# hawkn/emqx

Measured on AMD Instinct MI355X. Metric: topic matches/sec at 10M filters, higher is better.
Workload: dtype u8/u32; 1 GPU; c3: 10M mixed-wildcard filters incl. $share groups and '$SYS' exclusion; filters=10000002, topics_per_gpu_step=1000000, global_batch=1000000, parallelism=topic-sharded x1 (trie replicated), streams=3, distinct_batches=4, table_copies=1, outputs=pairs

## Files before the change

### emqx_amd/_native.py

```python
from __future__ import annotations

import ctypes as C
from pathlib import Path

import numpy as np

from .build import LIB_TMATCH

TM_OK, TM_EINVAL, TM_ENOMEM, TM_EDEVICE, TM_ECAP = 0, -1, -2, -3, -4
TM_OP_DELETE, TM_OP_INSERT = 0, 1
TM_KEY_BINARY, TM_KEY_WORDS, TM_KEY_EMPTY_LIST, TM_KEY_ESCAPED = 0, 1, 2, 4
TM_ORDER_TRAVERSAL, TM_ORDER_SORTED, TM_ORDER_UNIQUE = 0, 1, 2

EXPORTS = ("tm_create", "tm_destroy", "tm_apply_deltas", "tm_sync", "tm_match_batch",
           "tm_match_batch_dev", "tm_first_batch", "tm_stats", "tm_profile_enable", "tm_profile_read",
           "tm_last_error", "tm_abi_version", "tm_merge_shards", "tm_host_alloc", "tm_host_free",
           "tm_stream_release", "tm_match_batch_ex", "tm_match_batch_dev_ex", "tm_sort_segments",
           "tm_matches_filter", "tm_apply_deltas_ex", "tm_read_begin", "tm_read_end", "tm_epoch",
           "tm_create_replicas", "tm_replica_stats", "tm_debug_set", "tm_debug_get", "tm_match_batch32_ex",
           "tm_match_batch32_dev", "tm_matches_filter_ex", "tm_host_alloc_ex", "tm_commit",
           "tm_match_batch32_pairs", "tm_match_batch_dev_pairs", "tm_set_dests", "tm_fanout_dev", "tm_route_batch",
           "tm_fanout_dev_pairs", "tm_route_batch32", "tm_set_route_filters", "tm_aggre_dev", "tm_route_batch_ex",
           "tm_route_batch32_ex")
TM_ALLOC_VRAM = 1
TM_ROUTE_AGGRE = 1
NO_FILTER = 0xFFFFFFFF
TM_DEBUG_LB_SPINS, TM_DEBUG_LB_FAIL_BLOCK, TM_DEBUG_LB_LAUNCHES, TM_DEBUG_PHASES = 1, 2, 3, 4
TM_DEBUG_FAILED_BATCHES, TM_DEBUG_RETRIED_BATCHES = 5, 6
TM_DEBUG_PATH_PHASES, TM_DEBUG_PATH_SMALL, TM_DEBUG_PATH_LANE = 7, 8, 9
TM_DEBUG_SMALL_KERNEL = 10
SMALL_AUTO, SMALL_WAVE, SMALL_WAVE8 = 0, 1, 3
TM_DEBUG_COMBINE, TM_DEBUG_COMBINED_LAUNCHES, TM_DEBUG_COMBINED_BATCHES = 12, 13, 14
TM_DEBUG_WIDE_NODES, TM_DEBUG_DENSE_WIDE = 15, 16
TM_DEBUG_CMB_GATHER, TM_DEBUG_CMB_LAND = 17, 18
TM_DEBUG_COMMITS, TM_DEBUG_COMMIT_WAITS, TM_DEBUG_COMMIT_FORCED = 19, 20, 21
TM_DEBUG_SMALL_TICKET = 22
TM_DEBUG_CMB_SPIN = 23
TM_DEBUG_PATCH_ZC = 24
TM_DEBUG_FANOUT_GRID = 25
TM_DEBUG_ROUTE_ONE, TM_DEBUG_ROUTE_GRID = 26, 27
MAX_DESTS = 65536


class NativeUnavailable(RuntimeError):
    pass


class TmError(RuntimeError):
    def __init__(self, code, msg):
        super().__init__(f"tmatch error {code}: {msg}")
        self.code = code


class DeviceError(TmError):
    """TM_EDEVICE: the GPU failed the call (e.g. a batch whose look-back wait
    expired twice, include/tmatch.h err flag 4).  Never a client error: the
    reference raises badarg only for a '+'/'#' topic level
    (emqx_trie_search.erl:374-375)."""


class tm_options(C.Structure):
    _fields_ = [("device", C.c_int32), ("copies", C.c_uint32), ("hint_keys", C.c_uint64)]


class tm_stats_t(C.Structure):
    _fields_ = [(n, C.c_uint64) for n in ("n_keys", "n_wild_keys", "n_exact_keys", "n_dead_keys",
                                          "n_nodes", "n_edges", "n_words", "device_bytes",
                                          "uploads", "patch_bytes")]


_lib = None


def load_library(path: Path | None = None):
    global _lib
    if _lib is not None and path is None:
        return _lib
    import os
    p = Path(path) if path else Path(os.environ.get("TM_LIB", LIB_TMATCH))
    if not p.exists():
        raise NativeUnavailable(f"{p} is not built (run emqx_amd.build.build_all())")
    lib = C.CDLL(str(p))
    vp, u64, u32, i32 = C.c_void_p, C.c_uint64, C.c_uint32, C.c_int
    sig = {
        "tm_create": (i32, [C.POINTER(tm_options), C.POINTER(vp)]),
        "tm_destroy": (i32, [vp]),
        "tm_apply_deltas": (i32, [vp, u64, vp, vp, vp, vp, vp]),
        "tm_sync": (i32, [vp, vp]),
        "tm_match_batch": (i32, [vp, u64, vp, vp, vp, vp, u64, vp]),
        "tm_match_batch_dev": (i32, [vp, u64, vp, vp, vp, vp, u64, vp, vp]),
        "tm_first_batch": (i32, [vp, u64, vp, vp, vp, vp]),
        "tm_matches_filter": (i32, [vp, u64, vp, vp, vp, vp, u64, vp]),
        "tm_matches_filter_ex": (i32, [vp, u64, vp, vp, vp, vp, vp, u64, vp]),
        "tm_stats": (i32, [vp, C.POINTER(tm_stats_t)]),
        "tm_profile_enable": (i32, [vp, i32]),
        "tm_profile_read": (i32, [vp, C.POINTER(C.c_double), C.POINTER(C.c_double), C.POINTER(u64), i32]),
        "tm_last_error": (C.c_char_p, [vp]),
        "tm_abi_version": (u32, []),
        "tm_merge_shards": (i32, [u32, u64, vp, vp, u64, vp, vp, u64, vp]),
        "tm_host_alloc": (i32, [vp, u64, C.POINTER(vp)]),
        "tm_host_free": (i32, [vp, vp]),
        "tm_host_alloc_ex": (i32, [vp, u64, u32, C.POINTER(vp)]),
        "tm_stream_release": (i32, [vp, vp]),
        "tm_match_batch_ex": (i32, [vp, u64, vp, vp, vp, vp, u64, vp, u32, vp]),
        "tm_match_batch_dev_ex": (i32, [vp, u64, vp, vp, vp, vp, u64, vp, u32, vp, vp]),
        "tm_match_batch_dev_pairs": (i32, [vp, u64, vp, vp, vp, vp, u64, vp, vp]),
        "tm_sort_segments": (i32, [vp, u64, vp, vp, u64, u32, vp, vp]),
        "tm_apply_deltas_ex": (i32, [vp, u64, vp, vp, vp, vp, vp, C.POINTER(u64)]),
        "tm_commit": (i32, [vp, u64, vp, vp, vp, vp, vp, C.POINTER(u64)]),
        "tm_read_begin": (i32, [vp, C.POINTER(u64)]),
        "tm_read_end": (i32, [vp, u64]),
        "tm_epoch": (i32, [vp, C.POINTER(u64), C.POINTER(u64)]),
        "tm_create_replicas": (i32, [C.POINTER(tm_options), C.POINTER(C.c_int32), u32, C.POINTER(vp)]),
        "tm_replica_stats": (i32, [vp, u32, C.POINTER(u64), C.POINTER(C.c_int32)]),
        "tm_match_batch32_ex": (i32, [vp, u64, vp, vp, vp, vp, u64, vp, u32, vp]),
        "tm_match_batch32_dev": (i32, [vp, u64, vp, vp, vp, vp, u64, vp, vp]),
        "tm_match_batch32_pairs": (i32, [vp, u64, vp, vp, vp, vp, u64, vp]),
        "tm_set_dests": (i32, [vp, u64, vp, vp]),
        "tm_fanout_dev": (i32, [vp, u64, vp, vp, u64, vp, u64, u32, vp, vp, vp, vp]),
        "tm_fanout_dev_pairs": (i32, [vp, u64, vp, vp, u64, vp, u64, u32, vp, vp, vp, vp]),
        "tm_route_batch": (i32, [vp, u64, vp, vp, u32, vp, vp, vp, u64, vp]),
        "tm_route_batch32": (i32, [vp, u64, vp, vp, u32, vp, vp, vp, u64, vp]),
        "tm_set_route_filters": (i32, [vp, u64, vp, vp]),
        "tm_aggre_dev": (i32, [vp, u32, vp, vp, vp, u64, vp, u64, vp, vp, vp, vp]),
        "tm_route_batch_ex": (i32, [vp, u64, vp, vp, u32, vp, vp, vp, u64, vp, u32]),
        "tm_route_batch32_ex": (i32, [vp, u64, vp, vp, u32, vp, vp, vp, u64, vp, u32]),
        "tm_debug_set": (i32, [vp, u32, u64]),
        "tm_debug_get": (i32, [vp, u32, C.POINTER(u64)]),
    }
    for name, (res, args) in sig.items():
        try:
            f = getattr(lib, name)
        except AttributeError:
            if p == LIB_TMATCH:
                raise
            continue
        f.restype, f.argtypes = res, args
    if path is None:
        _lib = lib
    return lib


def _ptr(a: np.ndarray | None):
    return None if a is None else a.ctypes.data_as(C.c_void_p)


def _gpu_present() -> bool:
    try:
        import torch
        return torch.cuda.is_available()
    except Exception:
        return False


def merge_shards(world: int, n: int, d_shard_hit: int, d_shard_vals: int, stride: int, d_out_hit: int,
                 d_out_vals: int, cap: int, stream: int | None = None):
    if not _gpu_present():
        raise NativeUnavailable("no HIP device visible: the shard merge runs on the GPU only")
    lib = load_library()
    rc = lib.tm_merge_shards(world, n, d_shard_hit, d_shard_vals, stride, d_out_hit, d_out_vals, cap, stream)
    if rc != TM_OK:
        raise TmError(rc, lib.tm_last_error(None).decode())


def pack_strings(items) -> tuple[np.ndarray, np.ndarray]:
    items = [bytes(x) for x in items]
    offs = np.zeros(len(items) + 1, dtype=np.uint64)
    if items:
        offs[1:] = np.cumsum([len(x) for x in items], dtype=np.uint64)
    blob = np.frombuffer(b"".join(items) + b"\0" * 16, dtype=np.uint8)
    return blob, offs


class Index:

    def __init__(self, device: int = -1, hint_keys: int = 0, devices=None, copies: int = 1):
        if not _gpu_present():
            raise NativeUnavailable("no HIP device visible: the topic index runs on the GPU only")
        self._lib = load_library()
        opts = tm_options(device, copies, hint_keys)
        h = C.c_void_p()
        if devices is not None:
            devs = (C.c_int32 * len(devices))(*devices)
            rc = self._lib.tm_create_replicas(C.byref(opts), devs, len(devices), C.byref(h))
        else:
            rc = self._lib.tm_create(C.byref(opts), C.byref(h))
        if rc != TM_OK:
            raise TmError(rc, self._lib.tm_last_error(None).decode())
        self._h = h

    def _check(self, rc):
        if rc != TM_OK:
            cls = DeviceError if rc == TM_EDEVICE else TmError
# ... 260 lines not shown
```

### emqx_amd/csrc/tm_dev.h

```cpp
#pragma once
#include <stdint.h>
#include <hip/hip_runtime.h>
#include "tm_layout.h"

namespace tmx {

struct DevIndex {
    const VocabEntry *vocab; uint32_t vmask;
    const uint8_t *wpool;
    const Node *nodes;
    const CSlot *ctab;
    const uint32_t *vals;
    const ExactEntry *exact; uint32_t xmask;
    const uint16_t *xfp;
    const uint32_t *wseq;
    const uint32_t *wbits; uint32_t wcap;
    uint32_t depth, xlen_max;
    uint64_t xlen_mask;
    uint32_t hdesc;
};

constexpr int FAST_L = 8;

__host__ __device__ __forceinline__ uint32_t need_levels(const DevIndex &ix, uint32_t L) {
    const bool exact = L < 64 ? ((ix.xlen_mask >> L) & 1u) != 0 : L <= ix.xlen_max;
    return exact || L < ix.depth ? L : ix.depth;
}
constexpr int MID_L = 32;
constexpr int MAX_LEVELS = 65536;
constexpr int RCAP = 8;
constexpr int DEEP_LANES = 64;

enum { L_MID = 0, L_DEEP = 1, L_OVF_MID = 2, L_OVF_DEEP = 3, L_COUNT = 4 };

enum : uint32_t { LB_AGG = 1, LB_INCL = 2, LB_FAIL = 3 };
constexpr uint32_t LB_TAG_BITS = 19, LB_TAG_MASK = (1u << LB_TAG_BITS) - 1;
constexpr uint64_t LB_VAL_MASK = (1ull << 42) - 1;
__host__ __device__ constexpr uint64_t lb_word(uint32_t tag, uint32_t st, uint64_t v) {
    return (uint64_t)tag << 45 | (uint64_t)st << 42 | (v & LB_VAL_MASK);
}
__host__ __device__ constexpr uint32_t lb_tag(uint64_t w) { return (uint32_t)(w >> 45); }
__host__ __device__ constexpr uint32_t lb_state(uint64_t w) { return (uint32_t)(w >> 42) & 7u; }

constexpr uint32_t LB_SPINS = 1u << 22;
constexpr uint32_t LB_SLEEP = 1;
constexpr uint32_t LB_STRIDE = 1;
struct LbCtl {
    uint32_t spins;
    uint32_t fail_block;
    uint32_t ticket;
};

constexpr int SMALL_SEGS = 16;

struct Workspace {
    uint32_t *cnt;
    uint32_t *nr;
    uint2 *rng;
    uint32_t *lists;
    uint32_t *list_n;
    uint64_t *blk;
    uint64_t *sup;
    uint32_t *deep_wid;
    uint2 *deep_stk;
    uint8_t *deep_plus;
    uint64_t *look;
    uint32_t *pairs;
    uint64_t *vres;
    uint32_t *hint_h, *hint_d;
    uint64_t cap_n;
};

constexpr int TILE = 256;
constexpr int SUP = 64;
constexpr int SM_TICK = L_COUNT + 4;
constexpr int LIST_SLOTS = SM_TICK + SMALL_SEGS;
constexpr int HINT_FAIL = L_COUNT + 1;
constexpr int HINT_WORDS = L_COUNT + 2;
constexpr int VRES_K = 64;
constexpr int VRES_STRIDE = 16;
constexpr int VRES_POOL = VRES_K * VRES_STRIDE;
constexpr int VRES_WORDS = VRES_POOL + VRES_STRIDE;
constexpr int SM_TOPICS = 16;
constexpr int SM_TB = 256;
constexpr int SM_VSTAGE = 1024;


hipError_t launch_match_phase1(const DevIndex &ix, const Workspace &ws, uint64_t n, const uint8_t *bytes,
                               const uint64_t *offs, uint64_t *hit_offs, uint8_t *err, hipStream_t s,
                               hipEvent_t ev_walk0 = nullptr, hipEvent_t ev_walk1 = nullptr);
hipError_t launch_match_phase2(const DevIndex &ix, const Workspace &ws, uint64_t n, const uint8_t *bytes,
                               const uint64_t *offs, uint64_t *hit_offs, uint32_t *out, uint64_t cap,
                               hipStream_t s);
hipError_t launch_match_pairs(const DevIndex &ix, const Workspace &ws, uint64_t n, const uint8_t *bytes,
                              const uint64_t *offs, uint8_t *err, uint32_t *pairs, uint32_t *out, uint64_t cap,
                              hipStream_t s, hipEvent_t ev_walk0 = nullptr, hipEvent_t ev_walk1 = nullptr);
bool small_path_ok(const DevIndex &ix, uint64_t n);
bool one_launch_ok(const DevIndex &ix);
bool lite_path_ok(const DevIndex &ix);
enum { SMALL_AUTO = 0, SMALL_WAVE = 1, SMALL_WAVE8 = 3 };
enum { PATH_PHASES = 0, PATH_SMALL = 1, PATH_LANE = 2, PATH_COUNT = 3 };
hipError_t launch_match(const DevIndex &ix, const Workspace &ws, uint64_t n, const uint8_t *bytes,
                        const uint64_t *offs, uint64_t *hit_offs, uint8_t *err, uint32_t *out, uint64_t cap,
                        uint32_t tag, LbCtl lb, bool phases, int small_kind, hipStream_t s,
                        hipEvent_t ev_walk0 = nullptr, hipEvent_t ev_walk1 = nullptr, int *path = nullptr);
struct SmallSeg {
    const uint8_t *blob; const void *offs; void *hit; uint8_t *err; uint32_t *out;
    uint64_t cap; uint32_t n, block0;
};
struct SmallSegs { uint32_t count, pairs; SmallSeg s[SMALL_SEGS]; };
hipError_t launch_small_segs(const DevIndex &ix, const Workspace &ws, const SmallSegs &sg, bool u32, uint32_t tag,
                             LbCtl lb, int small_kind, hipStream_t s, int *path = nullptr);
hipError_t launch_match32(const DevIndex &ix, const Workspace &ws, uint64_t n, const uint8_t *bytes,
                          const uint32_t *offs, uint32_t *hit_offs, uint8_t *err, uint32_t *out, uint64_t cap,
                          uint32_t tag, LbCtl lb, int small_kind, hipStream_t s, int *path = nullptr);
hipError_t launch_offs_widen(const uint32_t *in, uint64_t *out, uint64_t m, hipStream_t s);
hipError_t launch_offs_narrow(const uint64_t *in, uint32_t *out, uint64_t m, hipStream_t s);
hipError_t launch_first(const DevIndex &ix, const Workspace &ws, uint64_t n, const uint8_t *bytes,
                        const uint64_t *offs, uint32_t *out_value, uint8_t *out_found, hipStream_t s);
hipError_t launch_merge_shards(uint32_t world, uint64_t n, const uint64_t *shard_hit, const uint32_t *shard_vals,
                               uint64_t stride, uint64_t *out_hit, uint32_t *out, uint64_t cap, hipStream_t s);
hipError_t launch_sort_segments(const Workspace &ws, uint64_t n, const uint64_t *hit_offs, uint32_t *out, uint64_t cap,
                                int unique, uint32_t *ucnt, hipStream_t s);
hipError_t launch_copy_values(const uint64_t *hit_offs, uint64_t n, const uint32_t *src, uint32_t *dst, uint64_t cap,
                              hipStream_t s);
constexpr int FO_GRID = 4096;
constexpr int FO_MAX_BITS = 9;
constexpr int FO_BINS = 1 << FO_MAX_BITS;
constexpr uint32_t FO_MAX_DESTS = 65536;
struct FanoutScratch {
    uint32_t *tab;
    uint32_t *tot;
    uint32_t *t, *v, *b;
    uint64_t cap;
    uint64_t *voff;
    uint64_t voff_cap;
    uint64_t *sums;
    uint32_t *b2;
    uint64_t *ag_bits;
    uint32_t *ag_pre, *ag_cnt;
    uint64_t ag_cap;
};
constexpr uint32_t FP_TILES = 1024;
bool fanout_two_pass(uint32_t n_dests);
hipError_t launch_fanout(const FanoutScratch &fs, uint64_t n, const uint64_t *hit, const uint32_t *values,
                         uint64_t cap, const uint32_t *dest_of, uint64_t dest_len, uint32_t n_dests,
                         uint64_t *dest_offsets, uint32_t *out_topic, uint32_t *out_value, hipStream_t s);
hipError_t launch_fanout_pairs(const FanoutScratch &fs, uint64_t n, const uint32_t *pairs, const uint32_t *values,
                               uint64_t cap, const uint32_t *dest_of, uint64_t dest_len, uint32_t n_dests,
                               uint64_t *dest_offsets, uint32_t *out_topic, uint32_t *out_value, hipStream_t s);
constexpr uint32_t FO1_TOPICS = 8192;
constexpr uint32_t FO1_ENTRIES = 16384;
constexpr uint32_t FO1_BLOCK = 1024;
constexpr uint32_t FO1_MAX_DESTS = 255;
enum { FO1_ST_STATE = 0, FO1_ST_TOTAL = 1, FO1_ST_WORDS = 2 };
enum : uint32_t { FO1_DONE = 1, FO1_TOO_LARGE = 2 };
hipError_t launch_fanout_one(uint64_t n, const uint32_t *pairs, const uint32_t *values, uint64_t vcap,
                             const uint32_t *dest_of, uint64_t dest_len, uint32_t n_dests, uint32_t *dest_offsets,
                             uint32_t *out_topic, uint32_t *out_value, uint64_t cap, uint32_t *status, hipStream_t s);
hipError_t launch_aggre(const FanoutScratch &fs, uint32_t n_dests, const uint64_t *dest_offsets, const uint32_t *in_topic,
                        const uint32_t *in_value, uint64_t cap, const uint32_t *filter_of, uint64_t filter_len,
                        uint64_t *out_dest_offsets, uint32_t *out_topic, uint32_t *out_value, hipStream_t s);
hipError_t launch_aggre_one(const uint32_t *status_in, const uint32_t *dest_offsets, uint32_t n_dests,
                            const uint32_t *in_topic, const uint32_t *in_value, const uint32_t *filter_of,
                            uint64_t filter_len, uint32_t *out_dest_offsets, uint32_t *out_topic, uint32_t *out_value,
                            uint64_t cap, uint32_t *status, hipStream_t s);
constexpr int N_TABLES = 9;
constexpr uint64_t PATCH_OFF = (1ull << 48) - 1;
struct PatchRun { uint64_t dst; uint32_t src, n; };
struct PatchBases { uint64_t b[N_TABLES]; };
hipError_t launch_patch(const PatchRun *d_runs, const uint32_t *d_data, uint64_t n_runs, PatchBases bases,
                        hipStream_t s);
// ... 7 lines not shown
```

### emqx_amd/csrc/tm_host.cpp

```cpp
#include <hip/hip_runtime.h>

#include <algorithm>
#include <atomic>
#include <chrono>
#include <cstdlib>
#include <cstdio>
#include <cstring>
#include <condition_variable>
#include <deque>
#include <memory>
#include <mutex>
#include <string>
#include <thread>
#include <map>
#include <unordered_map>
#include <unordered_set>
#include <set>
#include <vector>

#include "../../include/tmatch.h"
#include "tm_dev.h"
#include "tm_layout.h"

using namespace tmx;

namespace {

thread_local std::string g_last_error;


struct Dirty {
    std::vector<std::pair<uint64_t, uint64_t>> r;
    bool all = true;
    void add(uint64_t lo, uint64_t hi) {
        if (all || lo >= hi) return;
        if (!r.empty() && lo >= r.back().first && lo <= r.back().second) {
            r.back().second = std::max(r.back().second, hi);
            return;
        }
        r.push_back({lo, hi});
    }
    void set_all() { all = true; r.clear(); }
    void clear() { all = false; r.clear(); }
};

constexpr int MAX_REPLICAS = 16;

template <class T>
struct Mirror {
    std::vector<T> h;
    T *d[MAX_REPLICAS] = {};
    uint64_t dcap = 0;
    Dirty dirty;
    void touch(uint64_t i, uint64_t n = 1) {
        uint64_t lo = i * sizeof(T), hi = (i + n) * sizeof(T);
        dirty.add(lo / 4, (hi + 3) / 4);
    }
    uint64_t bytes() const { return h.size() * sizeof(T); }
};

struct NodeAux {
    uint32_t parent = NONE, wid = NONE, hash_cap = 0, exact_cap = 0;
    uint32_t depth = 0;
    uint32_t hash_roff = 0, exact_roff = 0;
    uint8_t is_plus = 0;
    uint32_t bm = NONE;
    uint32_t hdesc = 0;
};

struct WordRef { const uint8_t *p; uint32_t n; int kind; };

inline uint32_t nlit_of(const Node &n) { return n.nlit & NLIT_MASK; }

}

struct Lane {
    int r = 0;
    hipStream_t s = nullptr;
    bool owned = false;
    bool busy = false;
    bool used = false;
    bool drained = false;
    hipEvent_t done = nullptr;
    uint64_t tick = 0;
    uint32_t tag = 0;
    uint64_t waited = 0;
    Workspace w{};
    uint8_t *pin_in = nullptr, *pin_in_dev = nullptr; uint64_t pin_in_cap = 0;
    uint8_t *pin_out = nullptr, *pin_out_dev = nullptr; uint64_t pin_out_cap = 0;
    uint8_t *d_in = nullptr; uint64_t d_in_cap = 0;
    uint8_t *d_res = nullptr; uint64_t d_res_cap = 0;
    uint32_t *pin_vals = nullptr, *pin_vals_dev = nullptr; uint64_t pin_vals_cap = 0;
    uint32_t *d_vals = nullptr; uint64_t d_vals_cap = 0;
    uint64_t *d_o64 = nullptr, *d_h64 = nullptr; uint64_t d_o64_cap = 0, d_h64_cap = 0;
    FanoutScratch f{};
    uint32_t *d_ft = nullptr, *d_fv = nullptr; uint64_t d_ft_cap = 0, d_fv_cap = 0;
    uint64_t *d_fo = nullptr; uint64_t d_fo_cap = 0;
    uint32_t *d_pr = nullptr; uint64_t d_pr_cap = 0;
    uint32_t *fo1_h = nullptr, *fo1_d = nullptr;
    uint32_t *d_at = nullptr, *d_av = nullptr; uint64_t d_at_cap = 0, d_av_cap = 0;
    uint64_t *d_ao = nullptr; uint64_t d_ao_cap = 0;
    uint32_t *fo1_s = nullptr;
};

constexpr int PATCH_RING = 128;
constexpr uint64_t PATCH_ZC_MAX = 64 << 10;
struct PatchSlot {
    uint8_t *pin = nullptr; uint64_t pin_cap = 0;
    uint8_t *pin_dev = nullptr;
    uint64_t bytes = 0, nr = 0, seq = 0;
};

struct Replica {
    int device = 0, group = 0;
    hipStream_t ps = nullptr;
    hipEvent_t last_patch = nullptr;
    uint8_t *pdev[PATCH_RING] = {}; uint64_t pdev_cap[PATCH_RING] = {};
    hipEvent_t pdone[PATCH_RING] = {}; bool ppending[PATCH_RING] = {};
    uint64_t applied = 0;
    uint64_t last_use = 0;
    uint64_t batches = 0;
};


constexpr int MAX_HOST_LANES = 16;
constexpr int MAX_DEV_LANES = 16;

constexpr int CMB_LEADERS = 4;

struct tm_index {
    std::mutex mu;
    std::mutex img;
    std::atomic<bool> img_dirty{true};
    bool view_ok = false;
    std::condition_variable cv;
    int nrep = 1, ngroups = 1;
    Replica rep[MAX_REPLICAS];
    uint64_t rr = 0;

    Mirror<VocabEntry> vocab; uint64_t vcount = 0; uint32_t wid_next = 0;
    std::vector<uint32_t> wref, wslot, free_wids;
    Mirror<uint8_t> wpool; uint64_t wpool_dead = 0;
    Mirror<Node> nodes; std::vector<NodeAux> aux; std::vector<uint32_t> free_nodes; uint64_t live_nodes = 0;
    Mirror<CSlot> ctab; std::vector<uint32_t> free_ctab[33]; uint64_t nlinks = 0, ntables = 0;
    Mirror<uint32_t> vals; std::vector<uint32_t> free_blocks[33];
    Mirror<ExactEntry> exact; std::vector<uint32_t> xcap, xroff; uint64_t xcount = 0;
    Mirror<uint16_t> xfp;
    Mirror<uint32_t> wseq; uint64_t wseq_dead = 0;
    Mirror<uint32_t> wbits; uint32_t wb_words = 0;
    std::vector<uint32_t> free_wbits; std::set<uint32_t> wide;
    std::unordered_map<uint64_t, uint32_t> lvl_edges;
    std::vector<uint32_t> lvl_distinct;
    bool dense_dirty = false;

    std::vector<uint64_t> depth_cnt, xlen_cnt;

    std::unordered_set<std::string> dead;
    struct MfState {
        std::mutex mu;
        bool log_on = false, log_lost = false;
        std::vector<std::pair<bool, std::string>> log;
        std::unordered_set<std::string> keys;
        bool have_keys = false, dev_stale = true;
        std::atomic<size_t> nkeys{0};
        std::vector<std::string> words;
        uint32_t *pool = nullptr, *val = nullptr; uint64_t *koff = nullptr, K = 0;
        uint64_t pcap = 0, vcap = 0, kcap = 0;
        uint32_t *q = nullptr; uint64_t qcap = 0;
        uint8_t *err = nullptr; uint64_t *hit = nullptr; uint32_t *out = nullptr;
        uint64_t ecap = 0, ocap = 0, hcap = 0;
        hipStream_t s = nullptr;
        uint64_t snapshots = 0, slices = 0;
    } mf;
    uint64_t n_wild = 0, n_exact = 0;
    uint64_t n_hdesc_keys = 0;
    uint64_t uploads = 0, patch_bytes = 0;

    PatchSlot patch[PATCH_RING]; uint64_t patch_seq = 0;
    uint64_t pub_seq = 0;
    int serving[MAX_REPLICAS];
    std::atomic<int> img_hold{0};
    std::atomic<uint64_t> commits{0}, commit_waits{0}, commit_forced{0};
    DevIndex view[MAX_REPLICAS];

    std::vector<std::unique_ptr<Lane>> lanes;
    uint64_t tick = 0;

    std::mutex dst_mu;
    std::vector<uint32_t> dest_h;
    struct DestDev {
        uint32_t *d = nullptr; uint64_t cap = 0, len = 0;
        uint64_t lo = 0, hi = 0;
        uint32_t *pin = nullptr; uint64_t pin_cap = 0;
        hipEvent_t ev = nullptr; bool ev_set = false;
        hipStream_t ev_s = nullptr;
    } dest[MAX_REPLICAS];
    std::vector<uint32_t> filt_h;
    DestDev filt[MAX_REPLICAS];

    struct Pinned { uint8_t *host, *dev; uint64_t size; bool vram; };
    std::vector<Pinned> pinned;

    std::atomic<uint64_t> epoch{1};
    std::mutex ep_mu;
    uint64_t next_ticket = 1;
    std::map<uint64_t, uint64_t> readers;
    std::multiset<uint64_t> reader_epochs;

    bool prof = false;
    struct ProfEv { hipEvent_t b0, w0, w1, b1; int device; };
    std::vector<ProfEv> prof_pending, prof_free;
    double prof_walk_ms = 0, prof_batch_ms = 0;
    uint64_t prof_batches = 0;

    LbCtl dbg_lb{LB_SPINS, NONE, 0};
    uint32_t small_ticket = 1;
    bool patch_zc = true;
    uint64_t dbg_lb_launches = 0;
    bool dbg_phases = false;
    int small_kind = SMALL_AUTO;
    std::atomic<uint64_t> failed_batches{0}, retried_batches{0};
    std::atomic<uint64_t> path_batches[PATH_COUNT] = {};
    std::atomic<uint64_t> route_one{0}, route_grid{0};
    std::mutex cmb_mu;
    std::condition_variable cmb_gcv;
    std::deque<struct SmallReq *> cmb_q;
    int cmb_running = 0;
    int cmb_inflight = 0;
    int cmb_gathering = 0;
    int cmb_hw = 0;
    uint64_t cmb_hw_ns = 0;
    std::atomic<int> cmb_leaders{CMB_LEADERS};
    std::atomic<int> cmb_gather_us{0};
    std::atomic<int> cmb_spin_us{0};
    std::atomic<uint64_t> cmb_launches{0}, cmb_batches{0};
};

namespace {

int fail(tm_index *, int code, const std::string &msg) {
    g_last_error = msg;
    return code;
}

#define HIPCHK(h, x)                                                                    \
    do {                                                                                \
        hipError_t e_ = (x);                                                            \
        if (e_ != hipSuccess)                                                           \
            return fail(h, TM_EDEVICE, std::string(#x ": ") + hipGetErrorString(e_));   \
    } while (0)


void pack8(const uint8_t *p, uint32_t n, uint32_t &b0, uint32_t &b1);

uint64_t word_hash(const uint8_t *p, uint32_t n) {
    if (n <= VINL) {
        uint32_t b0, b1;
        pack8(p, n, b0, b1);
        return word_hash_short(b0, b1, n);
    }
    uint64_t x = FNV_OFF;
    for (uint32_t i = 0; i < n; i++) x = (x ^ p[i]) * FNV_PRIME;
    return word_hash_finish(x, n);
}

uint32_t pow2_at_least(uint64_t x) {
    uint64_t c = 16;
    while (c < x) c <<= 1;
    return (uint32_t)c;
}


void pack8(const uint8_t *p, uint32_t n, uint32_t &b0, uint32_t &b1) {
    b0 = b1 = 0;
    for (uint32_t i = 0; i < n && i < 8; i++) (i < 4 ? b0 : b1) |= (uint32_t)p[i] << (8 * (i % 4));
}

bool vocab_eq(tm_index *ix, const VocabEntry &e, uint64_t h, const uint8_t *p, uint32_t n) {
    if (e.tag != vocab_tag(h, n)) return false;
    if (n <= VINL) {
        uint32_t b0, b1;
        pack8(p, n, b0, b1);
        return e.b0 == b0 && e.b1 == b1;
    }
    return e.b1 == n && !memcmp(ix->wpool.h.data() + e.b0, p, n);
}

uint32_t vocab_find(tm_index *ix, const uint8_t *p, uint32_t n) {
    const uint64_t h = word_hash(p, n);
    const uint32_t mask = (uint32_t)ix->vocab.h.size() - 1;
    for (uint32_t s = (uint32_t)h & mask;; s = (s + 1) & mask) {
        const VocabEntry &e = ix->vocab.h[s];
        if (e.wid == NONE) return NONE;
        if (vocab_eq(ix, e, h, p, n)) return e.wid;
    }
}

VocabEntry empty_vocab() { VocabEntry e; memset(&e, 0, sizeof e); e.wid = NONE; return e; }

void vocab_bytes(tm_index *ix, const VocabEntry &e, std::string &out) {
    uint32_t n = e.tag & 0xFF;
    if (n < VINL + 1) {
        out.resize(n);
        for (uint32_t i = 0; i < n; i++) out[i] = (char)(((i < 4 ? e.b0 : e.b1) >> (8 * (i % 4))) & 0xFF);
    } else {
        out.assign(reinterpret_cast<const char *>(ix->wpool.h.data() + e.b0), e.b1);
    }
}

constexpr uint32_t VOCAB_LOAD_SHIFT = 2;
uint64_t vocab_entry_hash(tm_index *ix, const VocabEntry &e) {
    std::string w;
    vocab_bytes(ix, e, w);
    return word_hash(reinterpret_cast<const uint8_t *>(w.data()), (uint32_t)w.size());
}

void vocab_rehash(tm_index *ix, uint64_t cap) {
    std::vector<VocabEntry> nt(cap, empty_vocab());
    const uint32_t mask = (uint32_t)nt.size() - 1;
    for (const VocabEntry &e : ix->vocab.h) {
        if (e.wid == NONE) continue;
        const uint64_t h = vocab_entry_hash(ix, e);
        for (uint32_t s = (uint32_t)h & mask;; s = (s + 1) & mask)
            if (nt[s].wid == NONE) { nt[s] = e; ix->wslot[e.wid] = s; break; }
    }
    ix->vocab.h.swap(nt);
    ix->vocab.dirty.set_all();
}

void wide_cover(tm_index *ix);

void vocab_grow(tm_index *ix, uint64_t need) {
    if ((need << VOCAB_LOAD_SHIFT) <= ix->vocab.h.size()) return;
    vocab_rehash(ix, pow2_at_least(need << VOCAB_LOAD_SHIFT));
}

uint32_t vocab_intern(tm_index *ix, const uint8_t *p, uint32_t n) {
    uint32_t w = vocab_find(ix, p, n);
    if (w != NONE) return w;
    vocab_grow(ix, ix->vcount + 1);
    VocabEntry e = empty_vocab();
    const uint64_t h = word_hash(p, n);
    e.tag = vocab_tag(h, n);
    if (!ix->free_wids.empty()) { e.wid = ix->free_wids.back(); ix->free_wids.pop_back(); }
    else {
        e.wid = ix->wid_next++;
        ix->wref.push_back(0);
        ix->wslot.push_back(NONE);
        wide_cover(ix);
    }
    if (n <= VINL) {
        pack8(p, n, e.b0, e.b1);
    } else {
        uint64_t off = ix->wpool.h.size();
        ix->wpool.h.resize(off + ((n + 3) & ~3u), 0);
        memcpy(ix->wpool.h.data() + off, p, n);
        ix->wpool.touch(off, (n + 3) & ~3u);
        e.b0 = (uint32_t)off;
        e.b1 = n;
    }
    const uint32_t mask = (uint32_t)ix->vocab.h.size() - 1;
    for (uint32_t s = (uint32_t)h & mask;; s = (s + 1) & mask)
        if (ix->vocab.h[s].wid == NONE) { ix->vocab.h[s] = e; ix->vocab.touch(s); ix->wslot[e.wid] = s; break; }
    ix->vcount++;
    return e.wid;
}

void vocab_erase(tm_index *ix, uint32_t wid) {
    auto &t = ix->vocab.h;
    const uint32_t mask = (uint32_t)t.size() - 1;
    uint32_t i = ix->wslot[wid];
    if (t[i].wid != wid) return;
    if ((t[i].tag & 0xFF) > VINL) ix->wpool_dead += (t[i].b1 + 3) & ~3u;
    for (uint32_t j = (i + 1) & mask; t[j].wid != NONE; j = (j + 1) & mask) {
        const uint32_t k = (uint32_t)vocab_entry_hash(ix, t[j]) & mask;
        const bool stays = (i <= j) ? (i < k && k <= j) : (i < k || k <= j);
        if (!stays) { t[i] = t[j]; ix->wslot[t[i].wid] = i; ix->vocab.touch(i); i = j; }
    }
    t[i] = empty_vocab();
    ix->vocab.touch(i);
    ix->wslot[wid] = NONE;
    ix->free_wids.push_back(wid);
    ix->vcount--;
}

void word_ref(tm_index *ix, uint32_t wid) { ix->wref[wid]++; }
void word_unref(tm_index *ix, uint32_t wid) {
    if (--ix->wref[wid] == 0) vocab_erase(ix, wid);
}


uint32_t cls_of(uint32_t cap);

uint32_t ctab_alloc(tm_index *ix, uint32_t cap) {
    auto &fl = ix->free_ctab[cls_of(cap)];
    uint32_t o;
    if (!fl.empty()) { o = fl.back(); fl.pop_back(); }
    else { o = (uint32_t)ix->ctab.h.size(); ix->ctab.h.resize(o + cap); }
    for (uint32_t i = 0; i < cap; i++) ix->ctab.h[o + i] = CSlot{NONE, NONE, 0, 0};
    ix->ctab.touch(o, cap);
    ix->ntables++;
    return o;
}

void ctab_free(tm_index *ix, uint32_t off, uint32_t cap) {
    ix->free_ctab[cls_of(cap)].push_back(off);
    ix->ntables--;
}

void ctab_put(tm_index *ix, uint32_t off, uint32_t mask, uint32_t wid, uint32_t child, uint64_t sum) {
    for (uint32_t s = child_hash(wid) & mask;; s = (s + 1) & mask)
        if (ix->ctab.h[off + s].wid == NONE) {
            ix->ctab.h[off + s] = CSlot{wid, child, (uint32_t)sum, (uint32_t)(sum >> 32)};
            ix->ctab.touch(off + s);
            return;
        }
}

uint32_t ctab_find(tm_index *ix, uint32_t off, uint32_t mask, uint32_t wid) {
    for (uint32_t s = child_hash(wid) & mask;; s = (s + 1) & mask) {
        const CSlot &c = ix->ctab.h[off + s];
        if (c.wid == NONE) return NONE;
        if (c.wid == wid) return s;
    }
}

void ctab_erase(tm_index *ix, uint32_t off, uint32_t mask, uint32_t wid) {
    uint32_t i = ctab_find(ix, off, mask, wid);
    if (i == NONE) return;
    CSlot *t = ix->ctab.h.data() + off;
    for (uint32_t j = (i + 1) & mask; t[j].wid != NONE; j = (j + 1) & mask) {
        uint32_t k = child_hash(t[j].wid) & mask;
        bool stays = (i <= j) ? (i < k && k <= j) : (i < k || k <= j);
        if (!stays) { t[i] = t[j]; ix->ctab.touch(off + i); i = j; }
    }
    t[i] = CSlot{NONE, NONE, 0, 0};
    ix->ctab.touch(off + i);
}


uint32_t cls_of(uint32_t cap) { uint32_t c = 0; while ((1u << c) < cap) c++; return c; }

uint32_t val_alloc(tm_index *ix, uint32_t cap) {
    auto &fl = ix->free_blocks[cls_of(cap)];
    if (!fl.empty()) { uint32_t o = fl.back(); fl.pop_back(); return o; }
    uint64_t o = ix->vals.h.size();
    ix->vals.h.resize(o + cap, 0);
    return (uint32_t)o;
}

void val_free(tm_index *ix, uint32_t off, uint32_t cap) {
    if (cap) ix->free_blocks[cls_of(cap)].push_back(off);
}

bool run_insert(tm_index *ix, uint32_t &off, uint32_t &cnt, uint32_t &cap, uint32_t v) {
    uint32_t *b = ix->vals.h.data() + off;
    uint32_t pos = (uint32_t)(std::lower_bound(b, b + cnt, v) - b);
    if (pos < cnt && b[pos] == v) return false;
    if (cnt == cap) {
        uint32_t ncap = cap ? cap * 2 : 1;
        uint32_t noff = val_alloc(ix, ncap);
        memmove(ix->vals.h.data() + noff, ix->vals.h.data() + off, sizeof(uint32_t) * cnt);
        val_free(ix, off, cap);
        off = noff; cap = ncap;
        ix->vals.touch(off, cnt);
    }
    uint32_t *r = ix->vals.h.data() + off;
    memmove(r + pos + 1, r + pos, sizeof(uint32_t) * (cnt - pos));
    r[pos] = v;
    cnt++;
    ix->vals.touch(off + pos, cnt - pos);
    return true;
}

bool run_erase(tm_index *ix, uint32_t &off, uint32_t &cnt, uint32_t &cap, uint32_t v) {
    uint32_t *b = ix->vals.h.data() + off;
    uint32_t pos = (uint32_t)(std::lower_bound(b, b + cnt, v) - b);
    if (pos >= cnt || b[pos] != v) return false;
    memmove(b + pos, b + pos + 1, sizeof(uint32_t) * (cnt - pos - 1));
    cnt--;
    if (pos < cnt) ix->vals.touch(off + pos, cnt - pos);
    if (!cnt) { val_free(ix, off, cap); off = 0; cap = 0; }
    return true;
}

bool run_op(tm_index *ix, bool ins, uint32_t &roff, uint32_t &cap, uint32_t &doff, uint32_t &dcnt, uint32_t v) {
    uint32_t off = roff, cnt = dcnt & RUN_CNT;
    const bool changed = ins ? run_insert(ix, off, cnt, cap, v) : run_erase(ix, off, cnt, cap, v);
    roff = off;
    if (cnt == 1) { doff = ix->vals.h[off]; dcnt = 1u | RUN_INLINE; }
    else { doff = off; dcnt = cnt; }
    return changed;
}


uint32_t node_new(tm_index *ix, uint32_t parent, uint32_t wid, bool is_plus) {
    uint32_t id;
    if (!ix->free_nodes.empty()) { id = ix->free_nodes.back(); ix->free_nodes.pop_back(); }
    else { id = (uint32_t)ix->nodes.h.size(); ix->nodes.h.emplace_back(); ix->aux.emplace_back(); }
    Node nd; memset(&nd, 0, sizeof nd); nd.plus = NONE;
    for (uint32_t k = 0; k < KINL; k++) { nd.kw[k] = NONE; nd.kc[k] = NONE; }
    ix->nodes.h[id] = nd;
    ix->nodes.touch(id);
    NodeAux a; a.parent = parent; a.wid = wid; a.is_plus = is_plus;
    a.depth = parent == NONE ? 0 : ix->aux[parent].depth + 1;
    ix->aux[id] = a;
    ix->live_nodes++;
    if (ix->depth_cnt.size() <= a.depth) ix->depth_cnt.resize(a.depth + 1, 0);
    ix->depth_cnt[a.depth]++;
    if (!is_plus && wid != NONE) word_ref(ix, wid);
    return id;
}

uint32_t child_find(tm_index *ix, uint32_t node, uint32_t wid) {
    const Node &n = ix->nodes.h[node];
    if (nlit_of(n) <= KINL) {
        for (uint32_t k = 0; k < KINL; k++) if (n.kw[k] == wid) return n.kc[k];
        return NONE;
    }
    uint32_t s = ctab_find(ix, n.kw[0], n.kw[1], wid);
    return s == NONE ? NONE : ix->ctab.h[n.kw[0] + s].child;
}

void set_bloom(Node &n, uint32_t wid) {
    const uint32_t b = child_bit(child_hash(wid));
    bloom_word(n, b >> 5) |= 1u << (b & 31);
}


void wide_bit(tm_index *ix, uint32_t node, uint32_t wid, bool on) {
    const uint32_t bm = ix->aux[node].bm;
    if (bm == NONE) return;
    uint32_t &w = ix->wbits.h[bm + (wid >> 5)];
    if (on) w |= 1u << (wid & 31); else w &= ~(1u << (wid & 31));
    ix->wbits.touch(bm + (wid >> 5));
}

void wide_fill(tm_index *ix, uint32_t node) {
    const uint32_t bm = ix->aux[node].bm;
    std::fill(ix->wbits.h.begin() + bm, ix->wbits.h.begin() + bm + ix->wb_words, 0u);
    Node &n = ix->nodes.h[node];
    for (uint32_t i = 0; i <= n.kw[1]; i++) {
        const uint32_t w = ix->ctab.h[n.kw[0] + i].wid;
        if (w != NONE) ix->wbits.h[bm + (w >> 5)] |= 1u << (w & 31);
    }
    ix->wbits.touch(bm, ix->wb_words);
    n.kw[2] = bm;
    ix->nodes.touch(node);
    ix->dense_dirty = true;
}

uint32_t wide_alloc(tm_index *ix) {
    if (!ix->free_wbits.empty()) { uint32_t o = ix->free_wbits.back(); ix->free_wbits.pop_back(); return o; }
    const uint32_t o = (uint32_t)ix->wbits.h.size();
    ix->wbits.h.resize(o + ix->wb_words, 0u);
    return o;
}

void wide_cover(tm_index *ix) {
    if (ix->wide.empty() || (uint64_t)ix->wb_words * 32 >= ix->wid_next) return;
    uint32_t words = std::max<uint32_t>(ix->wb_words, 1024);
    while ((uint64_t)words * 32 < ix->wid_next) words *= 2;
    ix->wb_words = words;
    ix->wbits.h.clear();
    ix->free_wbits.clear();
    for (uint32_t node : ix->wide) {
        ix->aux[node].bm = wide_alloc(ix);
        wide_fill(ix, node);
    }
    ix->wbits.dirty.set_all();
}

void to_wide(tm_index *ix, uint32_t node) {
    if (ix->wide.empty()) ix->wb_words = 0;
    ix->wide.insert(node);
    if ((uint64_t)ix->wb_words * 32 < ix->wid_next) {
        ix->aux[node].bm = NONE;
        wide_cover(ix);
        return;
    }
    ix->aux[node].bm = wide_alloc(ix);
    wide_fill(ix, node);
}

void from_wide(tm_index *ix, uint32_t node) {
    ix->free_wbits.push_back(ix->aux[node].bm);
    ix->aux[node].bm = NONE;
    ix->wide.erase(node);
    Node &n = ix->nodes.h[node];
    for (uint32_t j = 0; j < 6; j++) bloom_word(n, j) = 0;
    for (uint32_t i = 0; i <= n.kw[1]; i++) {
        const uint32_t w = ix->ctab.h[n.kw[0] + i].wid;
        if (w != NONE) set_bloom(n, w);
    }
    ix->nodes.touch(node);
}

uint64_t lit_bloom(tm_index *ix, uint32_t q) {
    const Node &n = ix->nodes.h[q];
    uint64_t m = 0;
    auto add = [&](uint32_t wid) { m |= 1ull << psum_bit(child_hash(wid)); };
    if (nlit_of(n) <= KINL) {
        for (uint32_t k = 0; k < KINL; k++) if (n.kw[k] != NONE) add(n.kw[k]);
    } else if (nlit_of(n) > PSUM_BLOOM) {
        m = (1ull << PSUM_BLOOM) - 1;
    } else {
        for (uint32_t i = 0; i <= n.kw[1]; i++) if (ix->ctab.h[n.kw[0] + i].wid != NONE) add(ix->ctab.h[n.kw[0] + i].wid);
    }
    return m;
}

uint64_t node_flags(const Node &n) {
    return (n.hash_cnt ? PSUM_HASH : 0) | (n.exact_cnt ? PSUM_EXACT : 0) | (n.plus != NONE ? PSUM_PLUS : 0) |
           ((n.nlit & NLIT_HDESC) ? PSUM_HDESC : 0);
}

uint64_t node_psum(tm_index *ix, uint32_t q) {
    const Node &n = ix->nodes.h[q];
    uint64_t m = node_flags(n) | lit_bloom(ix, q) << PSUM_BQ;
    if (n.plus != NONE) m |= node_flags(ix->nodes.h[n.plus]) << PSUM_QQ | lit_bloom(ix, n.plus) << PSUM_BQQ;
    return m;
}

void summary_refresh1(tm_index *ix, uint32_t x);
void summary_refresh(tm_index *ix, uint32_t x) {
    summary_refresh1(ix, x);
    if (x != ROOT && ix->aux[x].is_plus) summary_refresh1(ix, ix->aux[x].parent);
}

void summary_refresh1(tm_index *ix, uint32_t x) {
    if (x == ROOT) return;
    const NodeAux &a = ix->aux[x];
    const uint32_t p = a.parent;
    Node &pn = ix->nodes.h[p];
    if (a.is_plus) {
        if (pn.plus != x) return;
        const uint64_t m = node_psum(ix, x);
        if (pn.psum_lo != (uint32_t)m || pn.psum_hi != (uint32_t)(m >> 32)) {
            pn.psum_lo = (uint32_t)m; pn.psum_hi = (uint32_t)(m >> 32);
            ix->nodes.touch(p);
        }
        return;
    }
    if (nlit_of(pn) <= KINL) return;
    const uint32_t sl = ctab_find(ix, pn.kw[0], pn.kw[1], a.wid);
    if (sl == NONE) return;
    CSlot &c = ix->ctab.h[pn.kw[0] + sl];
    if (c.child != x) return;
    const uint64_t m = node_psum(ix, x);
    if (c.sum_lo != (uint32_t)m || c.sum_hi != (uint32_t)(m >> 32)) {
        c.sum_lo = (uint32_t)m; c.sum_hi = (uint32_t)(m >> 32);
        ix->ctab.touch(pn.kw[0] + sl);
    }
}

void to_table(tm_index *ix, uint32_t node, uint32_t cap) {
    Node &n = ix->nodes.h[node];
    std::vector<CSlot> kids;
    if (nlit_of(n) <= KINL) {
        for (uint32_t k = 0; k < KINL; k++)
            if (n.kw[k] != NONE) {
                const uint64_t m = node_psum(ix, n.kc[k]);
                kids.push_back({n.kw[k], n.kc[k], (uint32_t)m, (uint32_t)(m >> 32)});
            }
    } else {
        for (uint32_t i = 0; i <= n.kw[1]; i++) if (ix->ctab.h[n.kw[0] + i].wid != NONE) kids.push_back(ix->ctab.h[n.kw[0] + i]);
        ctab_free(ix, n.kw[0], n.kw[1] + 1);
    }
    uint32_t off = ctab_alloc(ix, cap);
    Node &m = ix->nodes.h[node];
    for (uint32_t j = 0; j < 6; j++) bloom_word(m, j) = 0;
    for (auto &c : kids) {
        ctab_put(ix, off, cap - 1, c.wid, c.child, (uint64_t)c.sum_hi << 32 | c.sum_lo);
        set_bloom(m, c.wid);
    }
    m.kw[0] = off; m.kw[1] = cap - 1;
    if (ix->aux[node].bm != NONE) {
        m.kw[2] = ix->aux[node].bm;
        ix->dense_dirty = true;
    }
}

void lvl_edge(tm_index *ix, uint32_t lvl, uint32_t wid, bool add) {
    const uint64_t k = (uint64_t)lvl << 32 | wid;
    if (ix->lvl_distinct.size() <= lvl) ix->lvl_distinct.resize(lvl + 1, 0);
    if (add) {
        if (ix->lvl_edges[k]++ == 0) { ix->lvl_distinct[lvl]++; ix->dense_dirty |= !ix->wide.empty(); }
    } else {
        auto it = ix->lvl_edges.find(k);
        if (it != ix->lvl_edges.end() && --it->second == 0) {
            ix->lvl_edges.erase(it);
            ix->lvl_distinct[lvl]--;
            ix->dense_dirty |= !ix->wide.empty();
        }
    }
}

constexpr uint64_t DENSE_NUM = 3, DENSE_DEN = 5;
void wide_dense(tm_index *ix) {
    if (!ix->dense_dirty) return;
    ix->dense_dirty = false;
    for (uint32_t node : ix->wide) {
        Node &n = ix->nodes.h[node];
        const uint32_t lvl = ix->aux[node].depth;
        const uint64_t distinct = lvl < ix->lvl_distinct.size() ? ix->lvl_distinct[lvl] : 0;
        const bool dense = (uint64_t)nlit_of(n) * DENSE_DEN >= distinct * DENSE_NUM;
        const uint32_t want = dense ? NONE : ix->aux[node].bm;
        if (n.kw[2] != want) { n.kw[2] = want; ix->nodes.touch(node); }
    }
}

void child_add(tm_index *ix, uint32_t node, uint32_t wid, uint32_t child) {
    ix->nlinks++;
    lvl_edge(ix, ix->aux[node].depth, wid, true);
    if (ix->aux[node].bm != NONE) ix->dense_dirty = true;
    Node *n = &ix->nodes.h[node];
    if (nlit_of(*n) < KINL) {
        for (uint32_t k = 0; k < KINL; k++)
            if (n->kw[k] == NONE) { n->kw[k] = wid; n->kc[k] = child; break; }
    } else {
        if (nlit_of(*n) == KINL) to_table(ix, node, 16);
        else if ((nlit_of(*n) + 1) * 2 > n->kw[1] + 1) to_table(ix, node, (n->kw[1] + 1) * 2);
        n = &ix->nodes.h[node];
        ctab_put(ix, n->kw[0], n->kw[1], wid, child, node_psum(ix, child));
        if (ix->aux[node].bm != NONE) wide_bit(ix, node, wid, true);
        else set_bloom(*n, wid);
    }
    n->nlit++;
    if (nlit_of(*n) == WIDE_LIT && ix->aux[node].bm == NONE) { to_wide(ix, node); n = &ix->nodes.h[node]; }
    ix->nodes.touch(node);
    summary_refresh(ix, node);
}

void child_remove(tm_index *ix, uint32_t node, uint32_t wid) {
    ix->nlinks--;
    lvl_edge(ix, ix->aux[node].depth, wid, false);
    if (ix->aux[node].bm != NONE) ix->dense_dirty = true;
    Node &n = ix->nodes.h[node];
    if (nlit_of(n) <= KINL) {
        for (uint32_t k = 0; k < KINL; k++)
            if (n.kw[k] == wid) { n.kw[k] = NONE; n.kc[k] = NONE; break; }
        n.nlit--;
    } else {
        ctab_erase(ix, n.kw[0], n.kw[1], wid);
        wide_bit(ix, node, wid, false);
        n.nlit--;
        if (ix->aux[node].bm != NONE && nlit_of(n) < WIDE_LIT) from_wide(ix, node);
        if (nlit_of(n) == KINL) {
            std::vector<CSlot> kids;
            for (uint32_t i = 0; i <= n.kw[1]; i++) if (ix->ctab.h[n.kw[0] + i].wid != NONE) kids.push_back(ix->ctab.h[n.kw[0] + i]);
            ctab_free(ix, n.kw[0], n.kw[1] + 1);
            for (uint32_t k = 0; k < KINL; k++) { n.kw[k] = kids[k].wid; n.kc[k] = kids[k].child; }
        }
    }
    ix->nodes.touch(node);
    summary_refresh(ix, node);
}

bool node_empty(tm_index *ix, uint32_t id) {
    const Node &n = ix->nodes.h[id];
    return n.plus == NONE && n.nlit == 0 && n.hash_cnt == 0 && n.exact_cnt == 0 && ix->aux[id].hdesc == 0;
}

void node_prune(tm_index *ix, uint32_t id) {
    while (id != ROOT && node_empty(ix, id)) {
        NodeAux a = ix->aux[id];
        if (a.is_plus) {
            Node &pn = ix->nodes.h[a.parent];
            pn.plus = NONE; pn.psum_lo = pn.psum_hi = 0;
            ix->nodes.touch(a.parent);
            summary_refresh(ix, a.parent);
        } else {
            child_remove(ix, a.parent, a.wid);
            word_unref(ix, a.wid);
        }
        ix->free_nodes.push_back(id);
        ix->live_nodes--;
        ix->depth_cnt[a.depth]--;
        id = a.parent;
    }
}


ExactEntry empty_exact() { ExactEntry e; memset(&e, 0, sizeof e); e.nlev = NONE; return e; }

uint64_t seq_hash(const std::vector<uint32_t> &w) {
    uint64_t x = FNV_OFF;
    for (uint32_t v : w) x = seq_hash_step(x, v);
    return seq_hash_finish(x, (uint32_t)w.size());
}

bool exact_eq(tm_index *ix, const ExactEntry &e, uint64_t h, const std::vector<uint32_t> &w) {
    if (e.h_lo != (uint32_t)h || e.h_hi != (uint32_t)(h >> 32) || e.nlev != w.size()) return false;
    const uint32_t *s = w.size() <= XINL ? e.wids : ix->wseq.h.data() + e.seq_off;
    return !memcmp(s, w.data(), sizeof(uint32_t) * w.size());
}

uint32_t exact_find_slot(tm_index *ix, uint64_t h, const std::vector<uint32_t> &w) {
    const uint32_t mask = (uint32_t)ix->exact.h.size() - 1;
    for (uint32_t s = (uint32_t)h & mask;; s = (s + 1) & mask) {
        const ExactEntry &e = ix->exact.h[s];
        if (e.nlev == NONE) return NONE;
        if (exact_eq(ix, e, h, w)) return s;
    }
}

void exact_rehash(tm_index *ix, uint32_t ncap);
void exact_grow(tm_index *ix, uint64_t need) {
    if (need * 2 <= ix->exact.h.size()) return;
    exact_rehash(ix, pow2_at_least(need * 2));
}

void exact_rehash(tm_index *ix, uint32_t ncap) {
    std::vector<ExactEntry> nt(ncap, empty_exact());
    std::vector<uint32_t> nc(ncap, 0), nr(ncap, 0);
    std::vector<uint16_t> nf(ncap, 0);
    const uint32_t mask = ncap - 1;
    for (size_t i = 0; i < ix->exact.h.size(); i++) {
        const ExactEntry &e = ix->exact.h[i];
        if (e.nlev == NONE) continue;
        for (uint32_t s = e.h_lo & mask;; s = (s + 1) & mask)
            if (nt[s].nlev == NONE) { nt[s] = e; nc[s] = ix->xcap[i]; nr[s] = ix->xroff[i]; nf[s] = ix->xfp.h[i]; break; }
    }
    ix->exact.h.swap(nt);
    ix->xcap.swap(nc);
    ix->xroff.swap(nr);
    ix->xfp.h.swap(nf);
    ix->exact.dirty.set_all();
    ix->xfp.dirty.set_all();
}

void exact_erase_slot(tm_index *ix, uint32_t i) {
    auto &t = ix->exact.h;
    const uint32_t mask = (uint32_t)t.size() - 1;
    {
        const uint32_t nl = t[i].nlev;
        const uint32_t *ws = nl <= XINL ? t[i].wids : ix->wseq.h.data() + t[i].seq_off;
        std::vector<uint32_t> used(ws, ws + nl);
        if (nl > XINL) ix->wseq_dead += nl;
        for (uint32_t w : used) word_unref(ix, w);
        ix->xlen_cnt[nl]--;
    }
    for (uint32_t j = (i + 1) & mask; t[j].nlev != NONE; j = (j + 1) & mask) {
        uint32_t k = t[j].h_lo & mask;
        bool stays = (i <= j) ? (i < k && k <= j) : (i < k || k <= j);
        if (!stays) {
            t[i] = t[j]; ix->xcap[i] = ix->xcap[j]; ix->xroff[i] = ix->xroff[j]; ix->xfp.h[i] = ix->xfp.h[j];
            ix->exact.touch(i); ix->xfp.touch(i);
            i = j;
        }
    }
    t[i] = empty_exact();
    ix->xcap[i] = 0;
    ix->xroff[i] = 0;
    ix->xfp.h[i] = 0;
    ix->exact.touch(i);
    ix->xfp.touch(i);
    ix->xcount--;
}

void reclaim(tm_index *ix) {
    if (ix->wpool_dead * 2 > ix->wpool.h.size() && ix->wpool.h.size() >= (64u << 10)) {
        std::vector<uint8_t> np;
        np.reserve(ix->wpool.h.size() - ix->wpool_dead);
        for (VocabEntry &e : ix->vocab.h) {
            if (e.wid == NONE || (e.tag & 0xFF) <= VINL) continue;
            const uint64_t off = np.size(), padded = (e.b1 + 3) & ~3u;
            np.insert(np.end(), ix->wpool.h.begin() + e.b0, ix->wpool.h.begin() + e.b0 + padded);
            e.b0 = (uint32_t)off;
        }
        ix->wpool.h.swap(np);
        ix->wpool_dead = 0;
        ix->wpool.dirty.set_all();
        ix->vocab.dirty.set_all();
    }
    if (ix->wseq_dead * 2 > ix->wseq.h.size() && ix->wseq.h.size() >= (16u << 10)) {
        std::vector<uint32_t> nq;
        nq.reserve(ix->wseq.h.size() - ix->wseq_dead);
        for (ExactEntry &e : ix->exact.h) {
            if (e.nlev == NONE || e.nlev <= XINL) continue;
            const uint64_t off = nq.size();
            nq.insert(nq.end(), ix->wseq.h.begin() + e.seq_off, ix->wseq.h.begin() + e.seq_off + e.nlev);
            e.seq_off = (uint32_t)off;
        }
        ix->wseq.h.swap(nq);
        ix->wseq_dead = 0;
        ix->wseq.dirty.set_all();
        ix->exact.dirty.set_all();
    }
    const uint64_t vmin = 1024;
    if (ix->vocab.h.size() > vmin && (ix->vcount << (VOCAB_LOAD_SHIFT + 2)) < ix->vocab.h.size())
        vocab_rehash(ix, std::max<uint64_t>(vmin, pow2_at_least(std::max<uint64_t>(ix->vcount, 1) << VOCAB_LOAD_SHIFT)));
    if (ix->exact.h.size() > 1024 && ix->xcount * 8 < ix->exact.h.size())
        exact_rehash(ix, std::max<uint32_t>(1024, pow2_at_least(ix->xcount * 2)));
}


void split_words(const uint8_t *f, uint32_t len, std::vector<WordRef> &out) {
    out.clear();
    uint32_t s = 0;
    for (uint32_t i = 0; i <= len; i++) {
        if (i == len || f[i] == '/') {
            uint32_t n = i - s;
            int kind = (n == 1 && f[s] == '+') ? 1 : (n == 1 && f[s] == '#') ? 2 : 0;
            out.push_back({f + s, n, kind});
            s = i + 1;
        }
    }
}

std::string dead_key(const uint8_t *f, uint32_t len, uint32_t v, uint8_t flags) {
    std::string k;
    k.reserve(len + 5);
    k.push_back((char)flags);
// ... 34 lines not shown
std::string esc_join(const std::vector<std::pair<std::string, bool>> &w) {
    std::string o;
    for (size_t i = 0; i < w.size(); i++) {
        if (i) o.push_back('/');
        if (w[i].second) { o += w[i].first; continue; }
        if (w[i].first == "+" || w[i].first == "#") { o.push_back('\\'); o += w[i].first; continue; }
        for (char c : w[i].first) {
            if (c == '/' || c == '\\') o.push_back('\\');
            o.push_back(c);
        }
    }
    return o;
}

bool word_never(const std::pair<std::string, bool> &w) {
    return !w.second && (w.first == "+" || w.first == "#" || w.first.find('/') != std::string::npos);
}

void word_key_op(tm_index *ix, bool ins, const std::vector<WordRef> &w, uint32_t v, const std::string &dk,
                 bool dead_done);

void key_op(tm_index *ix, bool ins, const uint8_t *f, uint32_t len, uint32_t v, uint8_t flags,
            std::vector<WordRef> &w, std::vector<uint32_t> &wids) {
    if ((flags & TM_KEY_ESCAPED) && !(flags & TM_KEY_EMPTY_LIST)) {
        std::vector<std::pair<std::string, bool>> ew;
        esc_words(f, len, ew);
        bool never = false;
        for (auto &x : ew) never |= word_never(x);
        if (!never) {
            std::string plain;
            for (size_t i = 0; i < ew.size(); i++) { if (i) plain.push_back('/'); plain += ew[i].first; }
            key_op(ix, ins, reinterpret_cast<const uint8_t *>(plain.data()), (uint32_t)plain.size(), v,
                   TM_KEY_WORDS, w, wids);
            return;
        }
        const std::string canon = esc_join(ew);
        const std::string dk = dead_key(reinterpret_cast<const uint8_t *>(canon.data()), (uint32_t)canon.size(), v,
                                        TM_KEY_WORDS | TM_KEY_ESCAPED);
        if (ix->mf.log_on) mf_log(ix, ins, dk);
        if (ins ? !ix->dead.insert(dk).second : !ix->dead.erase(dk)) return;
        size_t hpos = ew.size();
        for (size_t i = 0; i + 1 < ew.size(); i++)
            if (ew[i].second && ew[i].first == "#") { hpos = i; break; }
        bool plain_prefix = hpos < ew.size();
        for (size_t i = 0; i < hpos && plain_prefix; i++) plain_prefix = !word_never(ew[i]);
        if (!plain_prefix) return;
        std::vector<WordRef> pw;
        for (size_t i = 0; i <= hpos; i++)
            pw.push_back({reinterpret_cast<const uint8_t *>(ew[i].first.data()), (uint32_t)ew[i].first.size(),
                          ew[i].second ? (ew[i].first == "+" ? 1 : 2) : 0});
        pw.push_back({nullptr, 0, 0});
        word_key_op(ix, ins, pw, v, dk, true);
        return;
    }
    if (flags & TM_KEY_EMPTY_LIST) {
        auto k = dead_key(nullptr, 0, v, TM_KEY_EMPTY_LIST);
        if (ins) ix->dead.insert(k); else ix->dead.erase(k);
        mf_log(ix, ins, k);
        return;
    }
    split_words(f, len, w);
    bool wild = false;
    for (auto &x : w) wild |= x.kind != 0;
    if (!wild && !(flags & TM_KEY_WORDS)) {
        wids.clear();
        if (ins) {
            for (auto &x : w) wids.push_back(vocab_intern(ix, x.p, x.n));
            exact_grow(ix, ix->xcount + 1);
        } else {
            for (auto &x : w) {
                uint32_t id = vocab_find(ix, x.p, x.n);
                if (id == NONE) return;
                wids.push_back(id);
            }
        }
        const uint64_t h = seq_hash(wids);
        uint32_t s = exact_find_slot(ix, h, wids);
        if (s == NONE) {
            if (!ins) return;
            ExactEntry e = empty_exact();
            e.h_lo = (uint32_t)h; e.h_hi = (uint32_t)(h >> 32); e.nlev = (uint32_t)wids.size();
            if (wids.size() <= XINL) {
                std::copy(wids.begin(), wids.end(), e.wids);
            } else {
                e.seq_off = (uint32_t)ix->wseq.h.size();
                ix->wseq.h.insert(ix->wseq.h.end(), wids.begin(), wids.end());
                ix->wseq.touch(e.seq_off, wids.size());
            }
            const uint32_t mask = (uint32_t)ix->exact.h.size() - 1;
            for (s = (uint32_t)h & mask; ix->exact.h[s].nlev != NONE; s = (s + 1) & mask) {}
            ix->exact.h[s] = e;
            ix->xcap[s] = 0;
            ix->xroff[s] = 0;
            ix->xfp.h[s] = exact_fp(h);
            ix->xfp.touch(s);
            ix->xcount++;
            for (uint32_t wd : wids) word_ref(ix, wd);
            if (ix->xlen_cnt.size() <= wids.size()) ix->xlen_cnt.resize(wids.size() + 1, 0);
            ix->xlen_cnt[wids.size()]++;
        }
        ExactEntry &e = ix->exact.h[s];
        if (ins) { if (run_op(ix, true, ix->xroff[s], ix->xcap[s], e.val_off, e.val_cnt, v)) ix->n_exact++; }
        else if (run_op(ix, false, ix->xroff[s], ix->xcap[s], e.val_off, e.val_cnt, v)) {
            ix->n_exact--;
            if (!(e.val_cnt & RUN_CNT)) { exact_erase_slot(ix, s); return; }
        }
        ix->exact.touch(s);
        return;
    }
    word_key_op(ix, ins, w, v, dead_key(f, len, v, TM_KEY_WORDS), false);
}

void word_key_op(tm_index *ix, bool ins, const std::vector<WordRef> &w, uint32_t v, const std::string &dk,
                 bool dead_done) {
    if (ix->mf.log_on && !dead_done) mf_log(ix, ins, dk);
    size_t hpos = w.size();
    for (size_t i = 0; i + 1 < w.size(); i++)
        if (w[i].kind == 2) { hpos = i; break; }
    if (hpos < w.size() && !dead_done) {
        if (ins ? !ix->dead.insert(dk).second : !ix->dead.erase(dk)) return;
    }
    const bool hash_term = hpos == w.size() && w.back().kind == 2;
    const size_t end = hpos < w.size() ? hpos : hash_term ? w.size() - 1 : w.size();
    uint32_t node = ROOT;
    for (size_t i = 0; i < end; i++) {
        if (w[i].kind == 1) {
            uint32_t c = ix->nodes.h[node].plus;
            if (c == NONE) {
                if (!ins) return;
                c = node_new(ix, node, NONE, true);
                ix->nodes.h[node].plus = c;
                ix->nodes.touch(node);
                summary_refresh(ix, node);
                summary_refresh(ix, c);
            }
            node = c;
        } else {
            uint32_t wid = ins ? vocab_intern(ix, w[i].p, w[i].n) : vocab_find(ix, w[i].p, w[i].n);
            if (wid == NONE) return;
            uint32_t c = child_find(ix, node, wid);
            if (c == NONE) {
                if (!ins) return;
                c = node_new(ix, node, wid, false);
                child_add(ix, node, wid, c);
            }
            node = c;
        }
    }
    Node &nd = ix->nodes.h[node];
    NodeAux &a = ix->aux[node];
    if (hpos < w.size()) {
        a.hdesc += ins ? 1 : -1;
        ix->n_hdesc_keys += ins ? 1 : -1;
        nd.nlit = nlit_of(nd) | (a.hdesc ? NLIT_HDESC : 0);
        ix->nodes.touch(node);
        summary_refresh(ix, node);
        if (!ins) node_prune(ix, node);
        return;
    }
    bool changed;
    changed = hash_term ? run_op(ix, ins, a.hash_roff, a.hash_cap, nd.hash_off, nd.hash_cnt, v)
                        : run_op(ix, ins, a.exact_roff, a.exact_cap, nd.exact_off, nd.exact_cnt, v);
    if (!changed) return;
    ix->nodes.touch(node);
    summary_refresh(ix, node);
    if (ins) ix->n_wild++;
    else { ix->n_wild--; node_prune(ix, node); }
}


constexpr uint64_t DEV_GUARD = 16;

int bring_up(tm_index *ix, int r, uint64_t upto, hipStream_t st, bool idle = false);
int collect_patch_locked(tm_index *ix);

template <class T>
int upload_full(tm_index *ix, Mirror<T> &m) {
    for (int r = 0; r < ix->nrep; r++)
        if (int rc = bring_up(ix, r, ix->patch_seq, ix->rep[r].ps)) return rc;
    uint64_t need = std::max<uint64_t>(m.h.size(), 1);
    const bool grow = need > m.dcap;
    const uint64_t cap = grow ? need + need / 2 + DEV_GUARD : m.dcap;
    auto ship = [&]() -> int {
        for (int r = 0; r < ix->nrep; r++) {
            HIPCHK(ix, hipSetDevice(ix->rep[r].device));
            HIPCHK(ix, hipDeviceSynchronize());
            if (grow) {
                if (m.d[r]) HIPCHK(ix, hipFree(m.d[r]));
                m.d[r] = nullptr;
                HIPCHK(ix, hipMalloc(&m.d[r], cap * sizeof(T)));
            }
            if (m.bytes()) HIPCHK(ix, hipMemcpy(m.d[r], m.h.data(), m.bytes(), hipMemcpyHostToDevice));
        }
        return TM_OK;
    };
    if (int rc = ship()) {
        m.dcap = 0;
        return rc;
    }
    m.dcap = cap;
    if (getenv("TM_DEBUG_UPLOADS"))
        fprintf(stderr, "tm upload_full: %zu-byte elements x %zu (%.1f MB), dcap %lu, %d replicas\n", sizeof(T),
                m.h.size(), m.bytes() / 1e6, (unsigned long)m.dcap, ix->nrep);
    m.dirty.clear();
    ix->uploads++;
    return TM_OK;
}

constexpr uint32_t PATCH_RUN = 64;

template <class T>
int collect(tm_index *ix, Mirror<T> &m, uint32_t table, std::vector<PatchRun> &runs, std::vector<uint32_t> &data) {
    if (m.h.size() + DEV_GUARD > m.dcap) m.dirty.set_all();
    if (!m.dirty.all) {
        uint64_t words = 0;
        for (auto &r : m.dirty.r) words += r.second - r.first;
        if (words * 4 > m.bytes() / 2) m.dirty.set_all();
    }
    if (m.dirty.all) return upload_full(ix, m);
    const uint8_t *src = reinterpret_cast<const uint8_t *>(m.h.data());
    const uint64_t limit = (m.bytes() + 3) / 4;
    for (auto &r : m.dirty.r) {
        const uint64_t hi = std::min<uint64_t>(r.second, limit);
        for (uint64_t lo = r.first; lo < hi; lo += PATCH_RUN) {
            const uint32_t n = (uint32_t)std::min<uint64_t>(PATCH_RUN, hi - lo);
            const uint64_t at = data.size();
            runs.push_back(PatchRun{(uint64_t)table << 48 | lo, (uint32_t)at, n});
            data.resize(at + n, 0);
            memcpy(data.data() + at, src + 4 * lo, std::min<uint64_t>(4ull * n, m.bytes() - 4 * lo));
        }
    }
    m.dirty.clear();
    return TM_OK;
}

PatchBases patch_bases(tm_index *ix, int r) {
    PatchBases b;
    const void *t[N_TABLES] = {ix->vocab.d[r], ix->wpool.d[r], ix->nodes.d[r], ix->ctab.d[r], ix->vals.d[r],
                               ix->exact.d[r], ix->xfp.d[r], ix->wseq.d[r], ix->wbits.d[r]};
    for (int i = 0; i < N_TABLES; i++) b.b[i] = reinterpret_cast<uint64_t>(t[i]);
    return b;
}

int next_tag(tm_index *ix, Lane &ln, hipStream_t s, uint32_t &tag) {
    ln.tag = (ln.tag + 1) & LB_TAG_MASK;
    if (!ln.tag) {
        ln.tag = 1;
        HIPCHK(ix, hipMemsetAsync(ln.w.look, 0, (ln.w.cap_n / SM_TOPICS + 4) * 8 * LB_STRIDE, s));
    }
    tag = ln.tag;
    return TM_OK;
}

LbCtl next_lb(tm_index *ix) {
    LbCtl c{LB_SPINS, NONE, 0};
    if (ix->dbg_lb_launches) {
        ix->dbg_lb_launches--;
        c = ix->dbg_lb;
    }
    c.ticket = ix->small_ticket;
    return c;
}

bool batch_failed(tm_index *ix, Lane &ln) {
    volatile uint32_t *f = ln.w.hint_h + HINT_FAIL;
    if (!*f) return false;
    *f = 0;
    ix->failed_batches++;
    return true;
}

int batch_done(tm_index *ix, Lane &ln) {
    HIPCHK(ix, hipEventRecord(ln.done, ln.s));
    ln.used = true;
    ln.drained = false;
    return TM_OK;
}

bool lane_busy(Lane &l) {
    if (!l.used || l.drained) return false;
    if (hipEventQuery(l.done) == hipErrorNotReady) return true;
    l.drained = true;
    return false;
}

int apply_patch(tm_index *ix, int r, uint64_t q, hipStream_t st, bool wait_readers = true) {
    Replica &R = ix->rep[r];
    const uint32_t k = (uint32_t)((q - 1) % PATCH_RING);
    const PatchSlot &p = ix->patch[k];
    HIPCHK(ix, hipSetDevice(R.device));
    const bool zc = ix->patch_zc && p.pin_dev && p.bytes <= PATCH_ZC_MAX;
    if (!zc && (p.bytes > R.pdev_cap[k] || !R.pdev[k])) {
        if (R.ppending[k]) { HIPCHK(ix, hipEventSynchronize(R.pdone[k])); R.ppending[k] = false; }
        if (R.pdev[k]) HIPCHK(ix, hipFree(R.pdev[k]));
        R.pdev[k] = nullptr;
        R.pdev_cap[k] = 0;
        const uint64_t want = std::max<uint64_t>(p.bytes * 2, 1u << 20);
        uint8_t *np = nullptr;
        HIPCHK(ix, hipMalloc(&np, want));
        R.pdev[k] = np;
        R.pdev_cap[k] = want;
    }
    if (wait_readers)
        for (auto &l : ix->lanes)
            if (l->r == r && l->s != st && lane_busy(*l)) HIPCHK(ix, hipStreamWaitEvent(st, l->done, 0));
    if (R.last_patch) HIPCHK(ix, hipStreamWaitEvent(st, R.last_patch, 0));
    const uint8_t *src = R.pdev[k];
// ... 25 lines not shown
    if (ix->view_ok && !commit &&
        (!ix->img_dirty.load(std::memory_order_acquire) || ix->img_hold.load(std::memory_order_acquire) > 0))
        return TM_OK;
    std::lock_guard<std::mutex> gi(ix->img);
    ix->img_dirty.store(false, std::memory_order_relaxed);
    int rc = collect_patch_locked(ix);
    for (int r = 0; r < ix->nrep; r++) ix->view[r] = dev_view_build(ix, r);
    ix->view_ok = rc == TM_OK;
    if (!commit) ix->pub_seq = ix->patch_seq;
    return rc;
}

int collect_patch_locked2(tm_index *ix);

int collect_patch_locked(tm_index *ix) {
    const int rc = collect_patch_locked2(ix);
    if (rc) {
        ix->vocab.dirty.set_all(); ix->wpool.dirty.set_all(); ix->nodes.dirty.set_all();
        ix->ctab.dirty.set_all(); ix->vals.dirty.set_all(); ix->exact.dirty.set_all();
        ix->xfp.dirty.set_all(); ix->wseq.dirty.set_all(); ix->wbits.dirty.set_all();
    }
    return rc;
}

std::atomic<uint64_t> g_col_n{0}, g_col_runs_ns{0}, g_col_slot_ns{0}, g_col_copy_ns{0};
const bool g_col_timing = getenv("TM_HOST_TIMING") != nullptr;
uint64_t col_now() {
    return (uint64_t)std::chrono::duration_cast<std::chrono::nanoseconds>(
        std::chrono::steady_clock::now().time_since_epoch()).count();
}

int collect_patch_locked2(tm_index *ix) {
    const uint64_t t0 = g_col_timing ? col_now() : 0;
    std::vector<PatchRun> runs;
    std::vector<uint32_t> data;
    int rc;
    if ((rc = collect(ix, ix->vocab, 0, runs, data))) return rc;
    if ((rc = collect(ix, ix->wpool, 1, runs, data))) return rc;
    if ((rc = collect(ix, ix->nodes, 2, runs, data))) return rc;
    if ((rc = collect(ix, ix->ctab, 3, runs, data))) return rc;
    if ((rc = collect(ix, ix->vals, 4, runs, data))) return rc;
    if ((rc = collect(ix, ix->exact, 5, runs, data))) return rc;
    if ((rc = collect(ix, ix->xfp, 6, runs, data))) return rc;
    if ((rc = collect(ix, ix->wseq, 7, runs, data))) return rc;
    if ((rc = collect(ix, ix->wbits, 8, runs, data))) return rc;
    const uint64_t nr = runs.size(), nw = data.size();
    if (!nr) return TM_OK;
    const uint64_t t1 = g_col_timing ? col_now() : 0;
    const uint64_t q = ix->patch_seq + 1;
    const uint32_t k = (uint32_t)((q - 1) % PATCH_RING);
    PatchSlot &p = ix->patch[k];
    if (p.seq) {
        for (int r = 0; r < ix->nrep; r++) {
            Replica &R = ix->rep[r];
            if (R.applied < p.seq && (rc = bring_up(ix, r, p.seq, R.ps))) return rc;
            if (R.ppending[k]) {
                HIPCHK(ix, hipSetDevice(R.device));
                HIPCHK(ix, hipEventSynchronize(R.pdone[k]));
                R.ppending[k] = false;
            }
        }
    }
    const uint64_t t2 = g_col_timing ? col_now() : 0;
    const uint64_t bytes = nr * sizeof(PatchRun) + nw * 4;
    if (bytes > p.pin_cap || !p.pin) {
        if (p.pin) HIPCHK(ix, hipHostFree(p.pin));
        p.pin = nullptr;
        p.pin_cap = 0;
        const uint64_t want = std::max<uint64_t>(bytes * 2, 64u << 10);
        uint8_t *np = nullptr;
        HIPCHK(ix, hipHostMalloc(&np, want, hipHostMallocPortable | hipHostMallocMapped));
        p.pin = np;
        p.pin_cap = want;
        void *dp = nullptr;
        p.pin_dev = hipHostGetDevicePointer(&dp, np, 0) == hipSuccess ? static_cast<uint8_t *>(dp) : nullptr;
    }
    memcpy(p.pin, runs.data(), nr * sizeof(PatchRun));
    memcpy(p.pin + nr * sizeof(PatchRun), data.data(), nw * 4);
    p.bytes = bytes; p.nr = nr; p.seq = q;
    if (g_col_timing) {
        g_col_n++;
        g_col_runs_ns += t1 - t0; g_col_slot_ns += t2 - t1; g_col_copy_ns += col_now() - t2;
    }
    ix->patch_seq = q;
    ix->patch_bytes += nw * 4;
    ix->uploads++;
    return TM_OK;
}

int sync_locked(tm_index *ix, int r0, hipStream_t s) {
    int rc;
    if ((rc = collect_patch(ix))) return rc;
    if ((rc = bring_up(ix, r0, ix->pub_seq, s))) return rc;
    HIPCHK(ix, hipSetDevice(ix->rep[r0].device));
    return TM_OK;
}

int pick_copy(tm_index *ix, int g, const int *busy, hipStream_t s = nullptr, bool by_stream = false) {
    auto ok = [&](int r) { return ix->rep[r].group == g && (!busy || busy[r] < MAX_HOST_LANES); };
    const int sv = ix->serving[g];
    if (sv >= 0 && ok(sv) && ix->rep[sv].applied >= ix->pub_seq) return sv;
    for (int r = 0; r < ix->nrep; r++)
        if (ok(r) && ix->rep[r].applied >= ix->pub_seq) return r;
    if (by_stream) {
        int pick = -1;
        uint64_t pick_tick = 0;
        for (int r = 0; r < ix->nrep; r++) {
            if (!ok(r)) continue;
            bool free_here = true;
            uint64_t mine = 0;
            for (auto &l : ix->lanes) {
                if (l->r != r || !l->used) continue;
                if (l->s == s) { mine = std::max<uint64_t>(mine, l->tick); continue; }
                if (lane_busy(*l)) { free_here = false; break; }
            }
            if (free_here && (pick < 0 || mine > pick_tick)) { pick = r; pick_tick = mine; }
        }
        if (pick >= 0) return pick;
    }
    for (int r = 0; r < ix->nrep; r++) {
        if (!ok(r)) continue;
        bool idle = true;
        for (auto &l : ix->lanes)
            if (l->r == r && lane_busy(*l)) { idle = false; break; }
        if (idle) return r;
    }
    int best = -1;
    for (int r = 0; r < ix->nrep; r++)
        if (ok(r) && (best < 0 || ix->rep[r].last_use < ix->rep[best].last_use)) best = r;
    return best;
}

DevIndex dev_view(tm_index *ix, int r) { return ix->view[r]; }

DevIndex dev_view_build(tm_index *ix, int r) {
    DevIndex d;
    d.vocab = ix->vocab.d[r]; d.vmask = (uint32_t)ix->vocab.h.size() - 1;
    d.wpool = ix->wpool.d[r];
    d.nodes = ix->nodes.d[r];
    d.ctab = ix->ctab.d[r];
    d.vals = ix->vals.d[r];
    d.exact = ix->exact.d[r]; d.xmask = (uint32_t)ix->exact.h.size() - 1;
    d.xfp = ix->xfp.d[r];
    d.wseq = ix->wseq.d[r];
    d.wbits = ix->wbits.d[r]; d.wcap = ix->wide.empty() ? 0 : ix->wb_words * 32;
    auto &dc = ix->depth_cnt, &xc = ix->xlen_cnt;
    while (dc.size() > 1 && dc.back() == 0) dc.pop_back();
    while (!xc.empty() && xc.back() == 0) xc.pop_back();
    d.depth = dc.empty() ? 0 : (uint32_t)dc.size() - 1;
    d.xlen_max = xc.empty() ? 0 : (uint32_t)xc.size() - 1;
    d.xlen_mask = 0;
    for (size_t k = 0; k < xc.size() && k < 64; k++) if (xc[k]) d.xlen_mask |= 1ull << k;
    d.hdesc = ix->n_hdesc_keys != 0;
    return d;
}


void free_workspace(Workspace &w) {
    void *wb[] = {w.cnt, w.nr, w.rng, w.lists, w.list_n, w.blk, w.deep_wid, w.deep_stk, w.deep_plus, w.look, w.pairs,
                  w.vres};
    for (void *p : wb) if (p) (void)hipFree(p);
    if (w.hint_h) (void)hipHostFree(w.hint_h);
    w = Workspace{};
}

void free_lane(Lane &l) {
    free_workspace(l.w);
    void *dv[] = {l.d_in, l.d_res, l.d_vals, l.d_o64, l.d_h64, l.f.tab, l.f.tot, l.f.t, l.f.v, l.f.b, l.f.voff, l.f.sums, l.f.b2,
                  l.d_ft, l.d_fv, l.d_fo, l.d_pr, l.f.ag_bits, l.f.ag_pre, l.f.ag_cnt, l.d_at, l.d_av, l.d_ao, l.fo1_s};
    for (void *p : dv) if (p) (void)hipFree(p);
    void *pins[] = {l.pin_in, l.pin_out, l.pin_vals, l.fo1_h};
    for (void *p : pins) if (p) (void)hipHostFree(p);
    if (l.done) (void)hipEventDestroy(l.done);
    if (l.owned && l.s) (void)hipStreamDestroy(l.s);
}

int make_lane(tm_index *ix, int r, hipStream_t s, bool owned, Lane *&out) {
    auto l = std::make_unique<Lane>();
    l->r = r;
    l->owned = owned;
    if (owned) HIPCHK(ix, hipStreamCreateWithFlags(&l->s, hipStreamNonBlocking));
    else l->s = s;
    HIPCHK(ix, hipEventCreateWithFlags(&l->done, hipEventDisableTiming));
    out = l.get();
    ix->lanes.push_back(std::move(l));
    return TM_OK;
}

int host_lane(tm_index *ix, std::unique_lock<std::mutex> &g, Lane *&out) {
    for (;;) {
        if (int rc = collect_patch(ix)) return rc;
        int busy[MAX_REPLICAS] = {}, gbusy[MAX_REPLICAS] = {};
        bool gfree[MAX_REPLICAS] = {};
        for (auto &l : ix->lanes)
            if (l->owned) busy[l->r] += l->busy;
        for (int r = 0; r < ix->nrep; r++) {
            gbusy[ix->rep[r].group] += busy[r];
            gfree[ix->rep[r].group] |= busy[r] < MAX_HOST_LANES;
        }
        int bg = -1;
        for (int k = 0; k < ix->ngroups; k++) {
            const int gi = (int)((ix->rr + k) % ix->ngroups);
            if (gfree[gi] && (bg < 0 || gbusy[gi] < gbusy[bg])) bg = gi;
        }
        if (bg >= 0) {
            ix->rr++;
            const int best = pick_copy(ix, bg, busy);
            ix->rep[best].last_use = ++ix->tick;
            HIPCHK(ix, hipSetDevice(ix->rep[best].device));
            for (auto &l : ix->lanes)
                if (l->owned && l->r == best && !l->busy) { l->busy = true; out = l.get(); return TM_OK; }
            int rc = make_lane(ix, best, nullptr, true, out);
            if (rc) return rc;
            out->busy = true;
            return TM_OK;
        }
        ix->cv.wait(g);
    }
}

struct LaneLease {
    tm_index *ix;
    std::unique_lock<std::mutex> &g;
    Lane *ln = nullptr;
    ~LaneLease() {
        if (!ln) return;
        if (!g.owns_lock()) g.lock();
        ln->busy = false;
        ix->cv.notify_one();
    }
};

int dev_group(tm_index *ix, int &g) {
    int dev = 0;
    HIPCHK(ix, hipGetDevice(&dev));
    for (int r = 0; r < ix->nrep; r++)
        if (ix->rep[r].device == dev) { g = ix->rep[r].group; return TM_OK; }
    return fail(ix, TM_EINVAL, "device API: the current HIP device holds no replica of this index");
}

int dev_lane(tm_index *ix, hipStream_t s, int r, Lane *&out) {
    int n = 0;
    size_t lru = SIZE_MAX;
    for (size_t i = 0; i < ix->lanes.size(); i++) {
        Lane &l = *ix->lanes[i];
        if (l.owned) continue;
        if (l.s == s && l.r == r) { l.tick = ++ix->tick; out = &l; return TM_OK; }
        n++;
        if (lru == SIZE_MAX || l.tick < ix->lanes[lru]->tick) lru = i;
    }
    if (n >= MAX_DEV_LANES && lru != SIZE_MAX) {
        Lane &l = *ix->lanes[lru];
        HIPCHK(ix, hipSetDevice(ix->rep[l.r].device));
        if (l.used) HIPCHK(ix, hipEventSynchronize(l.done));
        free_lane(l);
        ix->lanes.erase(ix->lanes.begin() + lru);
    }
    HIPCHK(ix, hipSetDevice(ix->rep[r].device));
    int rc = make_lane(ix, r, s, false, out);
    if (rc) return rc;
    out->tick = ++ix->tick;
    return TM_OK;
}

template <class T>
int grow_dev(tm_index *ix, hipStream_t s, T *&p, uint64_t &cap, uint64_t need) {
    if (need <= cap && p) return TM_OK;
    HIPCHK(ix, hipStreamSynchronize(s));
    if (p) HIPCHK(ix, hipFree(p));
    p = nullptr;
    cap = std::max<uint64_t>(need + need / 4, 64);
    HIPCHK(ix, hipMalloc(&p, cap * sizeof(T)));
    return TM_OK;
}

int ensure_ws(tm_index *ix, uint64_t n, Lane &ln) {
    Workspace &w = ln.w;
    if (!w.deep_wid) {
        HIPCHK(ix, hipMalloc(&w.deep_wid, (uint64_t)DEEP_LANES * MAX_LEVELS * 4));
        HIPCHK(ix, hipMalloc(&w.deep_stk, (uint64_t)DEEP_LANES * (MAX_LEVELS + 1) * 8));
        HIPCHK(ix, hipMalloc(&w.deep_plus, (uint64_t)DEEP_LANES * MAX_LEVELS));
        HIPCHK(ix, hipMalloc(&w.list_n, LIST_SLOTS * 4));
        HIPCHK(ix, hipMemsetAsync(w.list_n, 0, LIST_SLOTS * 4, ln.s));
        HIPCHK(ix, hipMalloc(&w.pairs, 2 * SMALL_SEGS * 4));
        HIPCHK(ix, hipMemsetAsync(w.pairs, 0, 2 * SMALL_SEGS * 4, ln.s));
        HIPCHK(ix, hipMalloc(&w.vres, VRES_WORDS * 8));
        HIPCHK(ix, hipMemsetAsync(w.vres, 0, VRES_WORDS * 8, ln.s));
        HIPCHK(ix, hipHostMalloc(&w.hint_h, HINT_WORDS * 4, hipHostMallocMapped));
        std::memset(w.hint_h, 0, HINT_WORDS * 4);
        HIPCHK(ix, hipHostGetDevicePointer(reinterpret_cast<void **>(&w.hint_d), w.hint_h, 0));
    }
    if (ix->rep[ln.r].last_patch && ln.waited != ix->rep[ln.r].applied) {
        HIPCHK(ix, hipStreamWaitEvent(ln.s, ix->rep[ln.r].last_patch, 0));
        ln.waited = ix->rep[ln.r].applied;
    }
    if (n <= w.cap_n && w.cnt) return TM_OK;
    HIPCHK(ix, hipStreamSynchronize(ln.s));
    if (w.cnt) {
        void *old[] = {w.cnt, w.nr, w.rng, w.lists, w.blk, w.look};
        for (void *p : old) (void)hipFree(p);
    }
    uint64_t c = std::max<uint64_t>(n + n / 4, 1024);
    HIPCHK(ix, hipMalloc(&w.cnt, c * 4));
    HIPCHK(ix, hipMalloc(&w.nr, c * 4));
    HIPCHK(ix, hipMalloc(&w.rng, c * RCAP * 8));
    HIPCHK(ix, hipMalloc(&w.lists, c * (L_COUNT + 1) * 4));
    const uint64_t nblk = c / TILE + 4, nsup = c / ((uint64_t)TILE * SUP) + 4;
    HIPCHK(ix, hipMalloc(&w.blk, (nblk + nsup) * 8));
    HIPCHK(ix, hipMemsetAsync(w.blk, 0, (nblk + nsup) * 8, ln.s));
    w.sup = w.blk + nblk;
    HIPCHK(ix, hipMalloc(&w.look, (c / SM_TOPICS + 4) * 8 * LB_STRIDE));
    HIPCHK(ix, hipMemsetAsync(w.look, 0, (c / SM_TOPICS + 4) * 8 * LB_STRIDE, ln.s));
    w.cap_n = c;
    return TM_OK;
}

void init_tables(tm_index *ix, uint64_t hint) {
    ix->vocab.h.assign(1024, empty_vocab());
    ix->exact.h.assign(1024, empty_exact());
    ix->xfp.h.assign(1024, 0);
    ix->xcap.assign(ix->exact.h.size(), 0);
    ix->xroff.assign(ix->exact.h.size(), 0);
    ix->nodes.h.reserve(hint / 2 + 1);
    ix->aux.reserve(hint / 2 + 1);
    node_new(ix, NONE, NONE, false);
    ix->vals.h.reserve(hint + 16);
    ix->vals.h.assign(4, 0);
}

hipStream_t pick_stream(tm_index *, void *s) { return reinterpret_cast<hipStream_t>(s); }

int prof_begin(tm_index *ix, tm_index::ProfEv &ev, hipStream_t s) {
    ev = {nullptr, nullptr, nullptr, nullptr, 0};
    if (!ix->prof) return TM_OK;
    int dev = 0;
    HIPCHK(ix, hipGetDevice(&dev));
    for (size_t i = 0; i < ix->prof_free.size(); i++)
        if (ix->prof_free[i].device == dev) {
            ev = ix->prof_free[i];
            ix->prof_free.erase(ix->prof_free.begin() + i);
            break;
        }
    if (!ev.b0) {
        HIPCHK(ix, hipEventCreate(&ev.b0)); HIPCHK(ix, hipEventCreate(&ev.w0));
        HIPCHK(ix, hipEventCreate(&ev.w1)); HIPCHK(ix, hipEventCreate(&ev.b1));
        ev.device = dev;
    }
    HIPCHK(ix, hipEventRecord(ev.b0, s));
    return TM_OK;
}

int prof_end(tm_index *ix, tm_index::ProfEv &ev, hipStream_t s) {
    if (!ev.b0) return TM_OK;
    HIPCHK(ix, hipEventRecord(ev.b1, s));
    ix->prof_pending.push_back(ev);
    return TM_OK;
}

int drain_lanes(tm_index *ix) {
    for (auto &l : ix->lanes)
        if (l->used) {
            HIPCHK(ix, hipSetDevice(ix->rep[l->r].device));
            HIPCHK(ix, hipEventSynchronize(l->done));
        }
    return TM_OK;
}

}


extern "C" {

uint32_t tm_abi_version(void) { return (1u << 16) | 14u; }

const char *tm_last_error(tm_index *) { return g_last_error.c_str(); }

int tm_create_replicas(const tm_options *opts, const int32_t *devices, uint32_t n, tm_index **out) {
    if (!out) return fail(nullptr, TM_EINVAL, "tm_create: out is NULL");
    *out = nullptr;
    const uint32_t copies = opts && opts->copies ? opts->copies : 1;
    if (!devices || n == 0 || n > 8 || copies > 4 || n * copies > (uint32_t)MAX_REPLICAS)
        return fail(nullptr, TM_EINVAL, "tm_create_replicas: 1 to 8 devices, 1 to 4 copies, at most 16 replicas");
    tm_index *ix = new (std::nothrow) tm_index();
    if (!ix) return fail(nullptr, TM_ENOMEM, "tm_create: out of host memory");
    ix->nrep = (int)(n * copies);
    for (int g = 0; g < MAX_REPLICAS; g++) ix->serving[g] = -1;
    ix->ngroups = (int)n;
    hipError_t e = hipSuccess;
    for (uint32_t r = 0; r < n * copies && e == hipSuccess; r++) {
        Replica &R = ix->rep[r];
        R.device = devices[r / copies];
        R.group = (int)(r / copies);
        e = hipSetDevice(R.device);
        if (e == hipSuccess) e = hipStreamCreateWithFlags(&R.ps, hipStreamNonBlocking);
        for (int i = 0; i < PATCH_RING && e == hipSuccess; i++)
            e = hipEventCreateWithFlags(&R.pdone[i], hipEventDisableTiming);
    }
    if (e != hipSuccess) {
        std::string m = std::string("tm_create: ") + hipGetErrorString(e);
        tm_destroy(ix);
        return fail(nullptr, TM_EDEVICE, m);
    }
    (void)hipSetDevice(ix->rep[0].device);
    init_tables(ix, opts ? opts->hint_keys : 0);
    *out = ix;
    return TM_OK;
}

int tm_create(const tm_options *opts, tm_index **out) {
    int32_t dev = opts ? opts->device : -1;
    if (dev < 0) {
        int d = 0;
        if (hipGetDevice(&d) != hipSuccess) d = 0;
        dev = d;
    }
    return tm_create_replicas(opts, &dev, 1, out);
}

int tm_replica_stats(tm_index *ix, uint32_t r, uint64_t *batches, int32_t *device) {
    if (!ix) return fail(nullptr, TM_EINVAL, "tm_replica_stats: null handle");
    std::lock_guard<std::mutex> g(ix->mu);
    if (r >= (uint32_t)ix->nrep) return fail(ix, TM_EINVAL, "tm_replica_stats: no such replica");
    if (batches) *batches = ix->rep[r].batches;
    if (device) *device = ix->rep[r].device;
    return TM_OK;
}

namespace { void mf_free_keys(tm_index::MfState &m); }

struct CmbTiming {
    std::atomic<uint64_t> groups{0}, reqs{0};
    std::atomic<uint64_t> lock_ns{0}, setup_ns{0}, launch_ns{0}, sync_ns{0}, release_ns{0}, done_ns{0}, req_ns{0};
};
static CmbTiming g_cmbt;
struct CommitTiming {
    std::atomic<uint64_t> n{0}, apply_ns{0}, lock_ns{0}, collect_ns{0}, idle_ns{0}, ship_ns{0};
};
static CommitTiming g_cmt;
static const bool g_cmb_timing = getenv("TM_HOST_TIMING") != nullptr;
static inline uint64_t ns_now() {
    return (uint64_t)std::chrono::duration_cast<std::chrono::nanoseconds>(
        std::chrono::steady_clock::now().time_since_epoch()).count();
}

int tm_destroy(tm_index *ix) {
    if (!ix) return TM_EINVAL;
    if (g_cmb_timing && g_cmbt.groups) {
        const double g = (double)g_cmbt.groups, us = 1e-3;
        fprintf(stderr, "tm combiner: %lu launches, %lu requests (%.2f per launch); per launch us: lock %.1f "
                        "setup %.1f launch %.1f sync %.1f lane-release %.1f mark-done %.1f; per request %.1f us\n",
                (unsigned long)g_cmbt.groups.load(), (unsigned long)g_cmbt.reqs.load(), g_cmbt.reqs / g,
                g_cmbt.lock_ns * us / g, g_cmbt.setup_ns * us / g, g_cmbt.launch_ns * us / g, g_cmbt.sync_ns * us / g,
                g_cmbt.release_ns * us / g, g_cmbt.done_ns * us / g,
                g_cmbt.req_ns * us / std::max<double>(1.0, (double)g_cmbt.reqs));
    }
    if (g_cmb_timing && g_col_n) {
        const double c = (double)g_col_n, us = 1e-3;
        fprintf(stderr, "tm collect: %lu patches; per patch us: runs %.1f slot-reuse %.1f pinned-copy %.1f\n",
                (unsigned long)g_col_n.load(), g_col_runs_ns * us / c, g_col_slot_ns * us / c, g_col_copy_ns * us / c);
    }
    if (g_cmb_timing && g_cmt.n) {
        const double c = (double)g_cmt.n, us = 1e-3;
        fprintf(stderr, "tm commit: %lu commits; per commit us: image %.1f lock %.1f collect %.1f wait-idle %.1f "
                        "ship %.1f\n", (unsigned long)g_cmt.n.load(), g_cmt.apply_ns * us / c, g_cmt.lock_ns * us / c,
                g_cmt.collect_ns * us / c, g_cmt.idle_ns * us / c, g_cmt.ship_ns * us / c);
    }
    for (int r = 0; r < ix->nrep; r++) {
        (void)hipSetDevice(ix->rep[r].device);
        (void)hipDeviceSynchronize();
    }
    for (auto &l : ix->lanes) {
        (void)hipSetDevice(ix->rep[l->r].device);
        free_lane(*l);
    }
    for (int r = 0; r < ix->nrep; r++) {
        Replica &R = ix->rep[r];
        (void)hipSetDevice(R.device);
        void *bufs[] = {ix->vocab.d[r], ix->wpool.d[r], ix->nodes.d[r], ix->ctab.d[r], ix->vals.d[r], ix->exact.d[r],
                        ix->xfp.d[r], ix->wseq.d[r], ix->wbits.d[r]};
        for (void *p : bufs) if (p) (void)hipFree(p);
        for (int i = 0; i < PATCH_RING; i++) {
            if (R.pdev[i]) (void)hipFree(R.pdev[i]);
            if (R.pdone[i]) (void)hipEventDestroy(R.pdone[i]);
        }
        if (R.ps) (void)hipStreamDestroy(R.ps);
    }
    for (int g = 0; g < ix->ngroups; g++) {
        for (int r = 0; r < ix->nrep; r++)
            if (ix->rep[r].group == g) { (void)hipSetDevice(ix->rep[r].device); break; }
        for (auto *D : {&ix->dest[g], &ix->filt[g]}) {
            if (D->d) (void)hipFree(D->d);
            if (D->pin) (void)hipHostFree(D->pin);
            if (D->ev) (void)hipEventDestroy(D->ev);
        }
    }
    (void)hipSetDevice(ix->rep[0].device);
    mf_free_keys(ix->mf);
    for (void *p : {(void *)ix->mf.q, (void *)ix->mf.err, (void *)ix->mf.hit, (void *)ix->mf.out}) if (p) (void)hipFree(p);
    if (ix->mf.s) (void)hipStreamDestroy(ix->mf.s);
    for (auto &p : ix->patch) if (p.pin) (void)hipHostFree(p.pin);
    for (auto &b : ix->pinned) (void)(b.vram ? hipFree(b.host) : hipHostFree(b.host));
    for (auto *v : {&ix->prof_pending, &ix->prof_free})
        for (auto &ev : *v) {
            (void)hipSetDevice(ev.device);
            for (hipEvent_t x : {ev.b0, ev.w0, ev.w1, ev.b1}) (void)hipEventDestroy(x);
        }
    delete ix;
    return TM_OK;
}

int tm_apply_deltas_ex(tm_index *ix, uint64_t n, const uint8_t *ops, const uint8_t *fb, const uint64_t *fo,
                       const uint32_t *values, const uint8_t *key_flags, uint64_t *out_epoch) {
    if (!ix) return fail(nullptr, TM_EINVAL, "tm_apply_deltas: null handle");
    if (n && (!ops || !fo || !values || (!fb && fo[n] != fo[0])))
        return fail(ix, TM_EINVAL, "tm_apply_deltas: null buffer");
    for (uint64_t i = 0; i < n; i++)
        if (ops[i] > TM_OP_INSERT || fo[i + 1] < fo[i] || fo[i + 1] - fo[i] > 0xFFFFFFFFull)
            return fail(ix, TM_EINVAL, "tm_apply_deltas: bad op or offsets at " + std::to_string(i));
    std::lock_guard<std::mutex> g(ix->img);
    std::vector<WordRef> w;
    std::vector<uint32_t> wids;
    try {
        for (uint64_t i = 0; i < n; i++)
            key_op(ix, ops[i] == TM_OP_INSERT, fb + fo[i], (uint32_t)(fo[i + 1] - fo[i]), values[i],
                   key_flags ? key_flags[i] : 0, w, wids);
        reclaim(ix);
        wide_dense(ix);
    } catch (const std::bad_alloc &) {
        return fail(ix, TM_ENOMEM, "tm_apply_deltas: out of host memory");
    }
    if (n) ix->img_dirty.store(true, std::memory_order_release);
    const uint64_t e = n ? ix->epoch.fetch_add(1, std::memory_order_acq_rel) + 1 : ix->epoch.load();
    if (out_epoch) *out_epoch = e;
    return TM_OK;
}

int tm_apply_deltas(tm_index *ix, uint64_t n, const uint8_t *ops, const uint8_t *fb, const uint64_t *fo,
                    const uint32_t *values, const uint8_t *key_flags) {
    return tm_apply_deltas_ex(ix, n, ops, fb, fo, values, key_flags, nullptr);
}

constexpr auto COMMIT_WAIT = std::chrono::milliseconds(20);

static_assert(sizeof(DevIndex) == 120, "DevIndex changed: compare the new field in same_view");
static bool same_view(const DevIndex &a, const DevIndex &b) {
    return a.vocab == b.vocab && a.vmask == b.vmask && a.wpool == b.wpool && a.nodes == b.nodes && a.ctab == b.ctab &&
           a.vals == b.vals && a.exact == b.exact && a.xmask == b.xmask && a.xfp == b.xfp && a.wseq == b.wseq &&
           a.wbits == b.wbits && a.wcap == b.wcap && a.depth == b.depth && a.xlen_max == b.xlen_max &&
           a.xlen_mask == b.xlen_mask && a.hdesc == b.hdesc;
}

int tm_commit(tm_index *ix, uint64_t n, const uint8_t *ops, const uint8_t *fb, const uint64_t *fo,
              const uint32_t *values, const uint8_t *key_flags, uint64_t *out_epoch) {
    if (!ix) return fail(nullptr, TM_EINVAL, "tm_commit: null handle");
    ix->img_hold.fetch_add(1, std::memory_order_acq_rel);
    struct Unhold {
        tm_index *ix;
        ~Unhold() { ix->img_hold.fetch_sub(1, std::memory_order_acq_rel); }
    } unhold{ix};
    const uint64_t ta = g_cmb_timing ? ns_now() : 0;
    int rc = tm_apply_deltas_ex(ix, n, ops, fb, fo, values, key_flags, out_epoch);
    if (rc || !n) return rc;
    const uint64_t tb = g_cmb_timing ? ns_now() : 0;
    std::unique_lock<std::mutex> g(ix->mu);
    const uint64_t tc = g_cmb_timing ? ns_now() : 0;
    const bool had_view = ix->view_ok;
    const uint64_t uploads0 = ix->uploads;
    DevIndex view0[MAX_REPLICAS];
    for (int r = 0; r < ix->nrep; r++) view0[r] = ix->view[r];
    if ((rc = collect_patch(ix, true))) return rc;
    const uint64_t q = ix->patch_seq;
    if (ix->pub_seq >= q) return TM_OK;
    ix->commits++;
    bool no_wait = !had_view || ix->uploads - uploads0 > 1;
    for (int r = 0; r < ix->nrep && !no_wait; r++) no_wait = !same_view(view0[r], ix->view[r]);
    const uint64_t td = g_cmb_timing ? ns_now() : 0;
    uint64_t t_idle = 0, t_ship = 0;
    const auto t0 = std::chrono::steady_clock::now();
    bool done[MAX_REPLICAS] = {}, waited = false;
    int left = ix->ngroups;
    for (;;) {
        const bool late = no_wait || std::chrono::steady_clock::now() - t0 > COMMIT_WAIT;
        bool busy[MAX_REPLICAS] = {};
        for (auto &l : ix->lanes)
            if (!busy[l->r] && lane_busy(*l)) busy[l->r] = true;
        for (int gi = 0; gi < ix->ngroups; gi++) {
            if (done[gi]) continue;
            int pick = -1, copies = 0;
            for (int r = 0; r < ix->nrep; r++) {
                if (ix->rep[r].group != gi) continue;
                copies++;
                if (!busy[r] && (pick < 0 || ix->rep[r].applied < ix->rep[pick].applied)) pick = r;
            }
            if (pick < 0 && copies > 1 && !late) continue;
            if (pick >= 0 && copies > 1) {
                const uint64_t t0s = g_cmb_timing ? ns_now() : 0;
                if ((rc = bring_up(ix, pick, q, ix->rep[pick].ps, true))) return rc;
                if (g_cmb_timing) t_ship += ns_now() - t0s;
                ix->serving[gi] = pick;
            } else {
                ix->commit_forced++;
            }
            done[gi] = true;
            left--;
        }
        if (!left) break;
        waited = true;
        const uint64_t tw = g_cmb_timing ? ns_now() : 0;
        g.unlock();
        std::this_thread::sleep_for(std::chrono::microseconds(2));
        g.lock();
        if (g_cmb_timing) t_idle += ns_now() - tw;
    }
    if (waited) ix->commit_waits++;
    if (ix->pub_seq < q) ix->pub_seq = q;
    if (g_cmb_timing) {
        g_cmt.n++;
        g_cmt.apply_ns += tb - ta; g_cmt.lock_ns += tc - tb; g_cmt.collect_ns += td - tc;
        g_cmt.idle_ns += t_idle; g_cmt.ship_ns += t_ship;
    }
    return TM_OK;
}

int tm_read_begin(tm_index *ix, uint64_t *ticket) {
    if (!ix || !ticket) return fail(ix, TM_EINVAL, "tm_read_begin: null argument");
    std::lock_guard<std::mutex> g(ix->ep_mu);
    const uint64_t e = ix->epoch.load(std::memory_order_acquire);
    *ticket = ix->next_ticket++;
    ix->readers.emplace(*ticket, e);
    ix->reader_epochs.insert(e);
    return TM_OK;
}

int tm_read_end(tm_index *ix, uint64_t ticket) {
    if (!ix) return fail(nullptr, TM_EINVAL, "tm_read_end: null handle");
    std::lock_guard<std::mutex> g(ix->ep_mu);
    auto it = ix->readers.find(ticket);
    if (it == ix->readers.end()) return fail(ix, TM_EINVAL, "tm_read_end: unknown ticket");
    ix->reader_epochs.erase(ix->reader_epochs.find(it->second));
    ix->readers.erase(it);
    return TM_OK;
}

int tm_epoch(tm_index *ix, uint64_t *current, uint64_t *safe) {
    if (!ix) return fail(nullptr, TM_EINVAL, "tm_epoch: null handle");
    std::lock_guard<std::mutex> g(ix->ep_mu);
    const uint64_t e = ix->epoch.load(std::memory_order_acquire);
    if (current) *current = e;
    if (safe) *safe = ix->reader_epochs.empty() ? e : *ix->reader_epochs.begin();
    return TM_OK;
}

int tm_sync(tm_index *ix, void *stream) {
    if (!ix) return fail(nullptr, TM_EINVAL, "tm_sync: null handle");
    std::lock_guard<std::mutex> g(ix->mu);
    int dev = 0, r0 = 0;
    HIPCHK(ix, hipGetDevice(&dev));
    hipStream_t s = pick_stream(ix, stream);
    bool found = false;
    for (int r = 0; r < ix->nrep && !found; r++) if (ix->rep[r].device == dev) { r0 = r; found = true; }
    if (!found) s = ix->rep[0].ps;
    return sync_locked(ix, r0, s);
}

int tm_match_batch_dev_ex(tm_index *ix, uint64_t n, const uint8_t *bytes, const uint64_t *offs, uint64_t *hit_offs,
                          uint32_t *out, uint64_t cap, uint8_t *err, uint32_t order, uint32_t *ucnt, void *stream) {
    if (!ix) return fail(nullptr, TM_EINVAL, "tm_match_batch_dev: null handle");
    if (!hit_offs || (n && (!offs || !bytes || !err))) return fail(ix, TM_EINVAL, "tm_match_batch_dev: null buffer");
    if (n >= 0xFFFFFFFFull) return fail(ix, TM_EINVAL, "tm_match_batch_dev: batch too large");
    if (order > TM_ORDER_UNIQUE) return fail(ix, TM_EINVAL, "tm_match_batch_dev: bad order");
    std::lock_guard<std::mutex> g(ix->mu);
    hipStream_t s = pick_stream(ix, stream);
    int rc, grp = 0;
    Lane *ln;
    if ((rc = dev_group(ix, grp))) return rc;
    if ((rc = collect_patch(ix))) return rc;
    const int r = pick_copy(ix, grp, nullptr, s, true);
    ix->rep[r].last_use = ++ix->tick;
    ix->rep[r].batches++;
    if ((rc = dev_lane(ix, s, r, ln))) return rc;
    if ((rc = sync_locked(ix, ln->r, s))) return rc;
    if ((rc = ensure_ws(ix, n, *ln))) return rc;
    const DevIndex d = dev_view(ix, ln->r);
    tm_index::ProfEv ev;
    if ((rc = prof_begin(ix, ev, s))) return rc;
    uint32_t tag;
    if ((rc = next_tag(ix, *ln, s, tag))) return rc;
    int path = PATH_PHASES;
    HIPCHK(ix, launch_match(d, ln->w, n, bytes, offs, hit_offs, err, out, out ? cap : 0, tag, next_lb(ix),
                            ix->dbg_phases, ix->small_kind, s, ev.w0, ev.w1, &path));
    ix->path_batches[path]++;
    if (order != TM_ORDER_TRAVERSAL && out)
        HIPCHK(ix, launch_sort_segments(ln->w, n, hit_offs, out, cap, order == TM_ORDER_UNIQUE, ucnt, s));
    if ((rc = batch_done(ix, *ln))) return rc;
    return prof_end(ix, ev, s);
}

int tm_match_batch_dev_pairs(tm_index *ix, uint64_t n, const uint8_t *bytes, const uint64_t *offs, uint32_t *pairs,
                             uint32_t *out, uint64_t cap, uint8_t *err, void *stream) {
    if (!ix) return fail(nullptr, TM_EINVAL, "tm_match_batch_dev_pairs: null handle");
    if (!pairs || (n && (!offs || !bytes || !err))) return fail(ix, TM_EINVAL, "tm_match_batch_dev_pairs: null buffer");
    if (reinterpret_cast<uintptr_t>(pairs) & 7) return fail(ix, TM_EINVAL, "tm_match_batch_dev_pairs: pairs not 8-byte aligned");
// ... 1208 lines not shown
        if (ev.w1) HIPCHK(ix, hipEventRecord(ev.w1, s));
        ix->path_batches[path]++;
    } else {
        if ((rc = grow_dev(ix, s, ln->d_o64, ln->d_o64_cap, n + 1))) return rc;
        if ((rc = grow_dev(ix, s, ln->d_h64, ln->d_h64_cap, n + 1))) return rc;
        HIPCHK(ix, launch_offs_widen(offs, ln->d_o64, n + 1, s));
        int path = PATH_PHASES;
        HIPCHK(ix, launch_match(d, ln->w, n, bytes, ln->d_o64, ln->d_h64, err, out, out ? cap : 0, tag, next_lb(ix),
                                ix->dbg_phases, ix->small_kind, s, ev.w0, ev.w1, &path));
        ix->path_batches[path]++;
        HIPCHK(ix, launch_offs_narrow(ln->d_h64, hit_offs, n + 1, s));
    }
    if ((rc = batch_done(ix, *ln))) return rc;
    return prof_end(ix, ev, s);
}

int tm_first_batch(tm_index *ix, uint64_t n, const uint8_t *tb, const uint64_t *to, uint32_t *out_value,
                   uint8_t *out_found) {
    if (!ix) return fail(nullptr, TM_EINVAL, "tm_first_batch: null handle");
    if (!to || !out_value || !out_found || (n && !tb && to[n] != to[0]))
        return fail(ix, TM_EINVAL, "tm_first_batch: null buffer");
    if (n >= 0xFFFFFFFFull) return fail(ix, TM_EINVAL, "tm_first_batch: batch too large");
    std::unique_lock<std::mutex> g(ix->mu);
    LaneLease lease{ix, g};
    int rc;
    if ((rc = host_lane(ix, g, lease.ln))) return rc;
    Lane &ln = *lease.ln;
    const hipStream_t s = ln.s;
    if ((rc = sync_locked(ix, ln.r, s))) return rc;
    if ((rc = ensure_ws(ix, n, ln))) return rc;
    ix->rep[ln.r].batches++;
    if (n && n <= ZC_TOPICS) {
        const uint64_t nbytes = to[n];
        uint8_t *db = nbytes ? pinned_dev(ix, tb, nbytes) : nullptr;
        uint8_t *dof = pinned_dev(ix, to, (n + 1) * 8);
        uint8_t *dv = pinned_dev(ix, out_value, n * 4), *df = pinned_dev(ix, out_found, n);
        if ((db || !nbytes) && ((uintptr_t)tb & 15) == 0 && dof && dv && df) {
            HIPCHK(ix, launch_first(dev_view(ix, ln.r), ln.w, n, db ? db : dof, reinterpret_cast<const uint64_t *>(dof),
                                    reinterpret_cast<uint32_t *>(dv), df, s));
            if ((rc = batch_done(ix, ln))) return rc;
            g.unlock();
            HIPCHK(ix, hipStreamSynchronize(s));
            return TM_OK;
        }
    }
    const uint8_t *dbytes;
    const uint64_t *doffs;
    if ((rc = stage_in(ix, ln, n, tb, to, nullptr, dbytes, doffs))) return rc;
    const uint64_t rbytes = n * 5;
    uint8_t *dres;
    if ((rc = stage_out(ix, ln, n, rbytes, dres))) return rc;
    HIPCHK(ix, launch_first(dev_view(ix, ln.r), ln.w, n, dbytes, doffs, reinterpret_cast<uint32_t *>(dres), dres + n * 4, s));
    if ((rc = fetch_out(ix, ln, n, rbytes))) return rc;
    if ((rc = batch_done(ix, ln))) return rc;
    g.unlock();
    HIPCHK(ix, hipStreamSynchronize(s));
    if (n) {
        memcpy(out_value, ln.pin_out, n * 4);
        memcpy(out_found, ln.pin_out + n * 4, n);
    }
    return TM_OK;
}

int tm_merge_shards(uint32_t world, uint64_t n, const uint64_t *shard_hit, const uint32_t *shard_vals,
                    uint64_t stride, uint64_t *out_hit, uint32_t *out, uint64_t cap, void *stream) {
    if (!world || !shard_hit || !out_hit || (cap && !out) || (n && !shard_vals))
        return fail(nullptr, TM_EINVAL, "tm_merge_shards: bad argument");
    hipError_t e = launch_merge_shards(world, n, shard_hit, shard_vals, stride, out_hit, out, cap,
                                       reinterpret_cast<hipStream_t>(stream));
    if (e != hipSuccess) return fail(nullptr, TM_EDEVICE, std::string("tm_merge_shards: ") + hipGetErrorString(e));
    return TM_OK;
}

int tm_profile_enable(tm_index *ix, int enable) {
    if (!ix) return fail(nullptr, TM_EINVAL, "tm_profile_enable: null handle");
    std::lock_guard<std::mutex> g(ix->mu);
    ix->prof = enable != 0;
    return TM_OK;
}

int tm_profile_read(tm_index *ix, double *walk_ms, double *batch_ms, uint64_t *batches, int reset) {
    if (!ix) return fail(nullptr, TM_EINVAL, "tm_profile_read: null handle");
    std::lock_guard<std::mutex> g(ix->mu);
    for (auto &ev : ix->prof_pending) {
        HIPCHK(ix, hipEventSynchronize(ev.b1));
        float w = 0, b = 0;
        if (ev.w0) { HIPCHK(ix, hipEventElapsedTime(&w, ev.w0, ev.w1)); }
        HIPCHK(ix, hipEventElapsedTime(&b, ev.b0, ev.b1));
        ix->prof_walk_ms += w; ix->prof_batch_ms += b; ix->prof_batches++;
        ix->prof_free.push_back(ev);
    }
    ix->prof_pending.clear();
    if (walk_ms) *walk_ms = ix->prof_walk_ms;
    if (batch_ms) *batch_ms = ix->prof_batch_ms;
    if (batches) *batches = ix->prof_batches;
    if (reset) { ix->prof_walk_ms = ix->prof_batch_ms = 0; ix->prof_batches = 0; }
    return TM_OK;
}

int tm_debug_set(tm_index *ix, uint32_t key, uint64_t value) {
    if (!ix) return fail(nullptr, TM_EINVAL, "tm_debug_set: null handle");
    std::lock_guard<std::mutex> g(ix->mu);
    switch (key) {
    case TM_DEBUG_LB_SPINS: ix->dbg_lb.spins = value > 0xFFFFFFFFull ? 0xFFFFFFFFu : (uint32_t)value; break;
    case TM_DEBUG_LB_FAIL_BLOCK: ix->dbg_lb.fail_block = value > 0xFFFFFFFFull ? NONE : (uint32_t)value; break;
    case TM_DEBUG_LB_LAUNCHES: ix->dbg_lb_launches = value; break;
    case TM_DEBUG_PHASES: ix->dbg_phases = value != 0; break;
    case TM_DEBUG_COMBINE: ix->cmb_leaders = value > 16 ? 16 : (int)value; break;
    case TM_DEBUG_CMB_GATHER: ix->cmb_gather_us = value > 1000 ? 1000 : (int)value; break;
    case TM_DEBUG_CMB_LAND: if (value) return fail(ix, TM_EINVAL, "tm_debug_set: TM_DEBUG_CMB_LAND was removed"); break;
    case TM_DEBUG_CMB_SPIN: ix->cmb_spin_us = value > 1000 ? 1000 : (int)value; break;
    case TM_DEBUG_SMALL_TICKET: ix->small_ticket = value != 0; break;
    case TM_DEBUG_PATCH_ZC: ix->patch_zc = value != 0; break;
    case TM_DEBUG_SMALL_KERNEL:
        if (value != SMALL_AUTO && value != SMALL_WAVE && value != SMALL_WAVE8)
            return fail(ix, TM_EINVAL, "tm_debug_set: TM_DEBUG_SMALL_KERNEL is 0, 1 or 3 (2, the lane kernel, was removed)");
        ix->small_kind = (int)value;
        break;
    default: return fail(ix, TM_EINVAL, "tm_debug_set: unknown key");
    }
    return TM_OK;
}

int tm_debug_get(tm_index *ix, uint32_t key, uint64_t *value) {
    if (!ix || !value) return fail(ix, TM_EINVAL, "tm_debug_get: null argument");
    switch (key) {
    case TM_DEBUG_FAILED_BATCHES: *value = ix->failed_batches.load(); break;
    case TM_DEBUG_RETRIED_BATCHES: *value = ix->retried_batches.load(); break;
    case TM_DEBUG_PATH_PHASES: *value = ix->path_batches[PATH_PHASES].load(); break;
    case TM_DEBUG_PATH_SMALL: *value = ix->path_batches[PATH_SMALL].load(); break;
    case TM_DEBUG_PATH_LANE: *value = ix->path_batches[PATH_LANE].load(); break;
    case TM_DEBUG_COMBINE: *value = (uint64_t)ix->cmb_leaders.load(); break;
    case TM_DEBUG_CMB_GATHER: *value = (uint64_t)ix->cmb_gather_us.load(); break;
    case TM_DEBUG_CMB_LAND: *value = 0; break;
    case TM_DEBUG_CMB_SPIN: *value = (uint64_t)ix->cmb_spin_us.load(); break;
    case TM_DEBUG_COMMITS: *value = ix->commits.load(); break;
    case TM_DEBUG_SMALL_TICKET: *value = ix->small_ticket; break;
    case TM_DEBUG_PATCH_ZC: *value = ix->patch_zc; break;
    case TM_DEBUG_FANOUT_GRID: *value = FO_GRID; break;
    case TM_DEBUG_ROUTE_ONE: *value = ix->route_one.load(); break;
    case TM_DEBUG_ROUTE_GRID: *value = ix->route_grid.load(); break;
    case TM_DEBUG_COMMIT_WAITS: *value = ix->commit_waits.load(); break;
    case TM_DEBUG_COMMIT_FORCED: *value = ix->commit_forced.load(); break;
    case TM_DEBUG_COMBINED_LAUNCHES: *value = ix->cmb_launches.load(); break;
    case TM_DEBUG_COMBINED_BATCHES: *value = ix->cmb_batches.load(); break;
    case TM_DEBUG_WIDE_NODES:
    case TM_DEBUG_DENSE_WIDE: {
        std::lock_guard<std::mutex> g(ix->img);
        uint64_t v = 0;
        for (uint32_t node : ix->wide) v += key == TM_DEBUG_WIDE_NODES || ix->nodes.h[node].kw[2] == NONE;
        *value = v;
        break;
    }
    default: return fail(ix, TM_EINVAL, "tm_debug_get: unknown key");
    }
    return TM_OK;
}


}

namespace {

void mf_words_of(const uint8_t *p, uint32_t n, std::vector<std::string> &out) {
    out.clear();
    uint32_t s0 = 0;
    for (uint32_t i = 0; i <= n; i++)
        if (i == n || p[i] == '/') { out.emplace_back(reinterpret_cast<const char *>(p) + s0, i - s0); s0 = i + 1; }
}

uint32_t mf_rank(const std::vector<std::string> &words, const std::string &w, bool wild) {
    if (wild) return w == "#" ? 0 : 1;
    const auto it = std::lower_bound(words.begin(), words.end(), w);
    const uint32_t i = (uint32_t)(it - words.begin());
    return it != words.end() && *it == w ? 3 + 2 * i : 2 + 2 * i;
}

void mf_key_words(const uint8_t *p, uint32_t n, uint8_t flags, std::vector<std::pair<std::string, bool>> &out) {
    if (flags & TM_KEY_ESCAPED) { esc_words(p, n, out); return; }
    std::vector<std::string> ws;
    mf_words_of(p, n, ws);
    out.clear();
    for (auto &x : ws) out.emplace_back(x, x == "+" || x == "#");
}

void mf_free_keys(tm_index::MfState &m) {
    for (void *p : {(void *)m.pool, (void *)m.koff, (void *)m.val}) if (p) (void)hipFree(p);
    m.pool = nullptr; m.koff = nullptr; m.val = nullptr; m.K = 0; m.pcap = m.kcap = m.vcap = 0;
}

void mf_path(tm_index *ix, uint32_t node, std::string &out) {
    std::vector<uint32_t> up;
    for (uint32_t x = node; x != ROOT; x = ix->aux[x].parent) up.push_back(x);
    out.clear();
    std::string w;
    for (size_t i = up.size(); i-- > 0;) {
        const NodeAux &a = ix->aux[up[i]];
        if (a.is_plus) w = "+";
        else vocab_bytes(ix, ix->vocab.h[ix->wslot[a.wid]], w);
        if (i + 1 != up.size()) out.push_back('/');
        out += w;
    }
}

constexpr double MF_SLICE_US = 100.0;

void mf_snapshot(tm_index *ix) {
    auto &m = ix->mf;
    m.keys.clear();
    {
        std::lock_guard<std::mutex> g(ix->img);
        m.log.clear();
        m.log_on = true;
        m.log_lost = false;
        for (const std::string &k : ix->dead) m.keys.insert(k);
    }
    std::string path, key;
    for (uint64_t cur = 0;;) {
        std::lock_guard<std::mutex> g(ix->img);
        const auto t0 = std::chrono::steady_clock::now();
        uint64_t end = ix->nodes.h.size(), x = cur;
        for (; x < end; x++) {
            if ((x & 63) == 63 &&
                std::chrono::duration<double, std::micro>(std::chrono::steady_clock::now() - t0).count() > MF_SLICE_US) {
                end = x;
                break;
            }
            const Node &n = ix->nodes.h[x];
            if (!(n.exact_cnt & RUN_CNT) && !(n.hash_cnt & RUN_CNT)) continue;
            mf_path(ix, (uint32_t)x, path);
            const NodeAux &a = ix->aux[x];
            auto add = [&](uint32_t roff, uint32_t cnt, bool hash) {
                for (uint32_t i = 0; i < cnt; i++) {
                    const uint32_t v = ix->vals.h[roff + i];
                    std::string f = hash ? (x == ROOT ? std::string("#") : path + "/#") : path;
                    m.keys.insert(dead_key(reinterpret_cast<const uint8_t *>(f.data()), (uint32_t)f.size(), v,
                                           TM_KEY_WORDS));
                }
            };
            add(a.exact_roff, n.exact_cnt & RUN_CNT, false);
            add(a.hash_roff, n.hash_cnt & RUN_CNT, true);
        }
        m.slices++;
        cur = end;
        if (cur >= ix->nodes.h.size()) break;
    }
    m.snapshots++;
    m.have_keys = true;
}

int mf_upload(tm_index *ix) {
    auto &m = ix->mf;
    std::vector<std::pair<std::string, bool>> dw;
    std::vector<std::string> sorted;
    std::unordered_set<std::string> distinct;
    for (const std::string &k : m.keys) {
        if ((uint8_t)k[0] & TM_KEY_EMPTY_LIST) continue;
        mf_key_words(reinterpret_cast<const uint8_t *>(k.data()) + 5, (uint32_t)k.size() - 5, (uint8_t)k[0], dw);
        for (auto &x : dw) if (!x.second) distinct.insert(x.first);
    }
    sorted.assign(distinct.begin(), distinct.end());
    std::sort(sorted.begin(), sorted.end());
    std::vector<uint32_t> pool;
    struct K { uint64_t off; uint32_t len, val; };
    std::vector<K> keys;
    keys.reserve(m.keys.size());
    for (const std::string &k : m.keys) {
        uint32_t v;
        memcpy(&v, k.data() + 1, 4);
        const uint64_t off = pool.size();
        if (!((uint8_t)k[0] & TM_KEY_EMPTY_LIST)) {
            mf_key_words(reinterpret_cast<const uint8_t *>(k.data()) + 5, (uint32_t)k.size() - 5, (uint8_t)k[0], dw);
            for (auto &x : dw) pool.push_back(mf_rank(sorted, x.first, x.second));
        }
        keys.push_back(K{off, (uint32_t)(pool.size() - off), v});
    }
    std::sort(keys.begin(), keys.end(), [&](const K &x, const K &y) {
        const uint32_t m2 = std::min(x.len, y.len);
        for (uint32_t i = 0; i < m2; i++)
            if (pool[x.off + i] != pool[y.off + i]) return pool[x.off + i] < pool[y.off + i];
        if (x.len != y.len) return x.len < y.len;
        return x.val < y.val;
    });
    std::vector<uint32_t> spool;
    spool.reserve(pool.size());
    std::vector<uint64_t> koff(keys.size() + 1, 0);
    std::vector<uint32_t> kval(keys.size());
    for (size_t i = 0; i < keys.size(); i++) {
        koff[i] = spool.size();
        spool.insert(spool.end(), pool.begin() + keys[i].off, pool.begin() + keys[i].off + keys[i].len);
        kval[i] = keys[i].val;
    }
    koff[keys.size()] = spool.size();
    auto grow = [&](auto *&p, uint64_t &cap, uint64_t need, size_t elt) -> int {
        if (need <= cap && p) return TM_OK;
        if (p) { HIPCHK(ix, hipStreamSynchronize(m.s)); HIPCHK(ix, hipFree(p)); }
        p = nullptr;
        cap = need + need / 4 + 1024;
        HIPCHK(ix, hipMalloc(reinterpret_cast<void **>(&p), cap * elt));
        return TM_OK;
    };
    int rc;
    if ((rc = grow(m.pool, m.pcap, spool.size(), 4))) return rc;
    if ((rc = grow(m.koff, m.kcap, koff.size(), 8))) return rc;
    if ((rc = grow(m.val, m.vcap, kval.size(), 4))) return rc;
    if (!spool.empty()) HIPCHK(ix, hipMemcpyAsync(m.pool, spool.data(), spool.size() * 4, hipMemcpyHostToDevice, m.s));
// ... 123 lines not shown
```

### emqx_amd/csrc/tm_kernels.hip

```cpp
#include "tm_dev.h"
#include "tm_scan.h"

#if defined(__HIP_DEVICE_COMPILE__) && !defined(__gfx950__)
#error "tm_kernels.hip: the tail tickets' ordering is argued for gfx950 only (see above)"
#endif

namespace tmx {


__device__ __forceinline__ uint4 ld4(const void *p) { return *reinterpret_cast<const uint4 *>(p); }
__device__ __forceinline__ uint4 ld4_once(const void *p) {
    typedef unsigned int u32x4 __attribute__((ext_vector_type(4)));
    const u32x4 v = __builtin_nontemporal_load(reinterpret_cast<const u32x4 *>(p));
    return make_uint4(v.x, v.y, v.z, v.w);
}

__device__ __forceinline__ uint32_t bloom_bit(const uint4 &n2, const uint4 &n3, uint32_t b) {
    const uint32_t j = b >> 5;
    const uint32_t w = j == 0 ? n2.z : j == 1 ? n2.w : j == 2 ? n3.x : j == 3 ? n3.y : j == 4 ? n3.z : n3.w;
    return (w >> (b & 31)) & 1u;
}

__device__ __forceinline__ uint32_t child_maybe(const DevIndex &ix, const uint4 &n1, const uint4 &n2, const uint4 &n3,
                                                uint32_t w, uint32_t h) {
    if ((n1.y & NLIT_MASK) >= WIDE_LIT)
        return n2.z == NONE ? 1u : w < ix.wcap ? (ix.wbits[n2.z + (w >> 5)] >> (w & 31)) & 1u : 0u;
    return bloom_bit(n2, n3, child_bit(h));
}

__device__ __forceinline__ bool child_alive(uint32_t lo, uint32_t hi, uint32_t lq, uint32_t L, uint32_t wq,
                                            uint32_t wq2) {
    const uint64_t m = (uint64_t)hi << 32 | lo;
    constexpr uint32_t AT_END = PSUM_HASH | PSUM_EXACT | PSUM_HDESC;
    if (lq == L) return (m & AT_END) != 0;
    if (m & PSUM_HASH) return true;
    if (wq != NONE && ((m >> (PSUM_BQ + psum_bit(child_hash(wq)))) & 1u)) return true;
    if (!(m & PSUM_PLUS)) return false;
    const uint32_t qq = (uint32_t)(m >> PSUM_QQ) & 15u;
    if (lq + 1 == L) return (qq & AT_END) != 0;
    if (qq & (PSUM_HASH | PSUM_PLUS)) return true;
    return wq2 != NONE && ((m >> (PSUM_BQQ + psum_bit(child_hash(wq2)))) & 1u);
}

__device__ __forceinline__ void pin(uint32_t &v) { asm volatile("" : "+v"(v)); }
__device__ __forceinline__ void pin(uint2 &v) { pin(v.x); pin(v.y); }
__device__ __forceinline__ void pin(uint4 &v) { pin(v.x); pin(v.y); pin(v.z); pin(v.w); }

struct WordAcc {
    uint32_t len, b0, b1;
    uint64_t start;
    __device__ __forceinline__ void reset(uint64_t s) {
        len = 0; b0 = b1 = 0; start = s;
    }
    __device__ __forceinline__ void push(uint32_t c) {
        uint32_t v = c << ((len & 3) * 8);
        if (len < 4) b0 |= v; else if (len < 8) b1 |= v;
        len++;
    }
};

struct GlobalSrc {
    const uint8_t *g;
    __device__ __forceinline__ uint4 ld16(uint64_t p) const { return ld4_once(g + p); }
    __device__ __forceinline__ uint32_t byte(uint64_t p) const { return g[p]; }
};
struct StagedSrc {
    const uint8_t *g;
    const uint4 *lds;
    uint64_t b0;
    bool staged;
    __device__ __forceinline__ uint4 ld16(uint64_t p) const {
        return staged ? lds[(uint32_t)(p - b0) >> 4] : ld4_once(g + p);
    }
    __device__ __forceinline__ uint32_t byte(uint64_t p) const {
        return staged ? reinterpret_cast<const uint8_t *>(lds)[(uint32_t)(p - b0)] : g[p];
    }
};

template <class Src>
__device__ bool bytes_eq(const uint8_t *a, const Src &src, uint64_t b, uint32_t n) {
    for (uint32_t i = 0; i < n; i++) if (a[i] != src.byte(b + i)) return false;
    return true;
}

template <class Src>
__device__ __forceinline__ uint64_t word_hash_dev(const WordAcc &w, const Src &src) {
    if (w.len <= VINL) return word_hash_short(w.b0, w.b1, w.len);
    uint64_t h = FNV_OFF;
    for (uint32_t i = 0; i < w.len; i++) h = (h ^ src.byte(w.start + i)) * FNV_PRIME;
    return word_hash_finish(h, w.len);
}

template <class Src>
__device__ uint32_t vocab_probe(const DevIndex &ix, uint32_t slot, uint32_t tag, uint32_t len, uint32_t b0,
                                uint32_t b1, const Src &src, uint64_t start) {
    for (;;) {
        const uint4 e = ld4(ix.vocab + slot);
        if (e.y == NONE) return NONE;
        if (e.x == tag) {
            if (len <= VINL) {
                if (e.z == b0 && e.w == b1) return e.y;
            } else if (e.w == len && bytes_eq(ix.wpool + e.z, src, start, len)) {
                return e.y;
            }
        }
        slot = (slot + 1) & ix.vmask;
    }
}

__device__ uint32_t vocab_probe_short(const DevIndex &ix, uint32_t slot, uint32_t tag, uint32_t b0, uint32_t b1) {
    for (;;) {
        const uint4 e = ld4(ix.vocab + slot);
        if (e.y == NONE) return NONE;
        if (e.x == tag && e.z == b0 && e.w == b1) return e.y;
        slot = (slot + 1) & ix.vmask;
    }
}

template <class Src>
__device__ uint32_t vocab_find(const DevIndex &ix, const WordAcc &w, const Src &src) {
    const uint64_t h = word_hash_dev(w, src);
    return vocab_probe(ix, (uint32_t)h & ix.vmask, vocab_tag(h, w.len), w.len, w.b0, w.b1, src, w.start);
}

__device__ __forceinline__ uint32_t ctab_find(const DevIndex &ix, uint32_t off, uint32_t mask, uint32_t wid,
                                              uint32_t h, uint32_t &slo, uint32_t &shi) {
    for (uint32_t s = h & mask;; s = (s + 1) & mask) {
        uint4 e = ld4(ix.ctab + off + s);
        pin(e);
        if (e.x == wid) { slo = e.z; shi = e.w; return e.y; }
        if (e.x == NONE) return NONE;
    }
}


template <int ML, bool LITE = false>
struct LdsStore {
    static constexpr uint32_t maxl = ML;
    static constexpr bool deferred = true;
    static constexpr bool cuts = ML > FAST_L;
    static constexpr bool need = ML > FAST_L || LITE;
    uint32_t *wid, *pend;
    uint8_t *len8;
    uint32_t stride;
    uint64_t mask;
    uint32_t pm;
    __device__ __forceinline__ void down(uint32_t l, bool via_plus) {
        if constexpr (cuts) pm = via_plus ? pm | (1u << l) : pm & ~(1u << l);
    }
    __device__ __forceinline__ void popped(uint32_t l) {
        if constexpr (cuts) pm &= (1u << (l - 1)) - 1u;
    }
    __device__ __forceinline__ void cut(uint32_t) {
        if constexpr (cuts) mask &= pm ? (1ull << (33u - __clz(pm))) - 1ull : 0ull;
    }
    __device__ __forceinline__ uint32_t get_wid(uint32_t l) const { return wid[l * stride]; }
    __device__ __forceinline__ void set_wid(uint32_t l, uint32_t w) { wid[l * stride] = w; }
    __device__ __forceinline__ void reset() { mask = 0; pm = 0; }
    __device__ __forceinline__ void put_word(uint32_t l, uint32_t b0, uint32_t b1, uint32_t len) {
        wid[l * stride] = b0; pend[l * stride] = b1; len8[l * stride] = (uint8_t)len;
    }
    __device__ __forceinline__ uint32_t word_b0(uint32_t l) const { return wid[l * stride]; }
    __device__ __forceinline__ uint32_t word_b1(uint32_t l) const { return pend[l * stride]; }
    __device__ __forceinline__ uint32_t word_len(uint32_t l) const { return len8[l * stride]; }
    __device__ __forceinline__ void push(uint32_t l, uint32_t node) {
        pend[l * stride] = node; mask |= 1ull << l;
    }
    __device__ __forceinline__ bool pop(uint32_t &l, uint32_t &node) {
        if (!mask) return false;
        l = 63u - (uint32_t)__clzll(mask);
        mask &= ~(1ull << l);
        node = pend[l * stride];
        return true;
    }
};

struct GlobalStore {
    static constexpr uint32_t maxl = MAX_LEVELS;
    static constexpr bool deferred = false;
    static constexpr bool cuts = true;
    static constexpr bool need = true;
    uint32_t *wid;
    uint2 *stk;
    uint8_t *plus_at;
    uint32_t top;
    __device__ __forceinline__ uint32_t get_wid(uint32_t l) const { return wid[l]; }
    __device__ __forceinline__ void set_wid(uint32_t l, uint32_t w) { wid[l] = w; }
    __device__ __forceinline__ void reset() { top = 0; }
    __device__ __forceinline__ void down(uint32_t l, bool via_plus) { plus_at[l] = via_plus; }
    __device__ __forceinline__ void popped(uint32_t l) { plus_at[l - 1] = 0; }
    __device__ void cut(uint32_t L) {
        int64_t q = (int64_t)L - 1;
        while (q >= 0 && !plus_at[q]) q--;
        while (top && (int64_t)stk[top - 1].x > q + 1) top--;
    }
    __device__ __forceinline__ void push(uint32_t l, uint32_t node) { stk[top++] = make_uint2(l, node); }
    __device__ __forceinline__ bool pop(uint32_t &l, uint32_t &node) {
        if (!top) return false;
        uint2 e = stk[--top]; l = e.x; node = e.y;
        return true;
    }
};


enum { RC_OK = 0, RC_BADARG = 1, RC_DEEP = 2 };

constexpr uint32_t VGROUP = 6;

template <class Src>
__device__ __noinline__ uint32_t count_slashes(const Src src, uint64_t p, uint64_t end) {
    uint32_t n = 0;
    for (; p < end; p += 64) {
        uint4 v[4];
#pragma unroll
        for (int c = 0; c < 4; c++) v[c] = p + 16 * c < end ? src.ld16(p + 16 * c) : make_uint4(0, 0, 0, 0);
#pragma unroll
        for (int c = 0; c < 4; c++) {
            const uint32_t w[4] = {v[c].x, v[c].y, v[c].z, v[c].w};
            const uint64_t q = p + 16 * c;
            const int k1 = q >= end ? 0 : end - q < 16 ? (int)(end - q) : 16;
#pragma unroll
            for (int j = 0; j < 4; j++) {
                const uint32_t x = w[j] ^ 0x2F2F2F2Fu;
                uint32_t nz = (((x & 0x7F7F7F7Fu) + 0x7F7F7F7Fu) | x) & 0x80808080u;
                const int valid = k1 - 4 * j;
                if (valid < 4) nz |= valid <= 0 ? 0x80808080u : 0x80808080u << (8 * valid);
                n += 4 - __popc(nz);
            }
        }
    }
    return n;
}

template <class S, class Src>
__device__ int tokenize(const DevIndex &ix, const Src &src, uint64_t beg, uint64_t end, S &st,
                        uint32_t &L, bool &dollar, uint64_t &xh, bool &all_found) {
    uint64_t longmask = 0;
    all_found = true; dollar = false; xh = FNV_OFF;
    if constexpr (S::deferred) {
        constexpr bool NEED = S::need;
        const ScanOut sc = scan_levels<NEED>(src, beg, end, st);
        const uint32_t lev = sc.lev;
        bool bad = sc.bad;
        if (sc.early) {
            const bool any = ix.xlen_max <= S::maxl && ix.depth + 2 <= (uint32_t)MID_L &&
                             end - beg < (uint64_t)MAX_LEVELS;
            L = any ? lev + 1 : lev + 1 + count_slashes(src, sc.p, end);
            return RC_DEEP;
        }
        if (lev > (NEED ? MAX_LEVELS : S::maxl)) { L = lev; return RC_DEEP; }
        L = lev;
        for (uint32_t l = 0; l < L && l < S::maxl; l++) {
            const uint32_t n = st.word_len(l), c = st.word_b0(l) & 0xFFu;
            bad |= n == 1 && (c == '+' || c == '#');
        }
        if (bad) return RC_BADARG;
        if constexpr (NEED) {
            const uint32_t Lw = need_levels(ix, L);
            if (Lw + (Lw < L ? 2 : 0) > S::maxl) return RC_DEEP;
            L |= Lw << 24;
        }
        dollar = st.word_len(0) == 255 ? src.byte(beg) == '$' : st.word_len(0) >= 1 && (st.word_b0(0) & 0xFFu) == '$';
        for (uint32_t l = 0; l < (S::need ? L >> 24 : L); l++) {
            if (st.word_len(l) != 255) continue;
            WordAcc w; w.reset(beg + st.word_b1(l)); w.len = st.word_b0(l);
            st.set_wid(l, vocab_find(ix, w, src));
            longmask |= 1ull << l;
        }
    } else {
        const uint64_t p0 = beg & ~15ull;
        const uint4 z = make_uint4(0, 0, 0, 0);
        const uint4 c0 = p0 < end ? src.ld16(p0) : z;
        const uint4 c1 = p0 + 16 < end ? src.ld16(p0 + 16) : z;
        WordAcc w; w.reset(beg);
        uint32_t lev = 0;
        auto finish = [&]() -> int {
            if (w.len == 1 && (w.b0 == '+' || w.b0 == '#')) return RC_BADARG;
            if (lev >= S::maxl) return RC_DEEP;
            if (lev == 0 && w.len >= 1 && (w.b0 & 0xFF) == '$') dollar = true;
            st.set_wid(lev, vocab_find(ix, w, src));
            lev++;
            return RC_OK;
        };
        uint32_t ci = 0;
        for (uint64_t p = p0; p < end; p += 16, ci++) {
            const uint4 v = ci == 0 ? c0 : ci == 1 ? c1 : src.ld16(p);
            const uint32_t k0 = p < beg ? (uint32_t)(beg - p) : 0;
            const uint32_t k1 = end - p < 16 ? (uint32_t)(end - p) : 16;
            for (uint32_t k = k0; k < k1; k++) {
                const uint32_t word = k < 4 ? v.x : k < 8 ? v.y : k < 12 ? v.z : v.w;
                const uint32_t c = (word >> ((k & 3) * 8)) & 0xFFu;
                if (c == '/') {
                    int rc = finish();
                    if (rc) return rc;
                    w.reset(p + k + 1);
                } else {
                    w.push(c);
                }
            }
        }
        int rc = finish();
        if (rc) return rc;
        L = lev;
    }
    if constexpr (S::deferred) {
        for (uint32_t base = 0; base < (S::need ? L >> 24 : L); base += VGROUP) {
            uint4 e[VGROUP];
            uint32_t tg[VGROUP];
            bool use[VGROUP];
#pragma unroll
            for (uint32_t k = 0; k < VGROUP; k++) {
                const uint32_t l = base + k;
                use[k] = l < (S::need ? L >> 24 : L) && !((longmask >> l) & 1);
                const uint32_t ls = use[k] ? l : 0;
                const uint32_t len = st.word_len(ls);
                const uint64_t h = word_hash_short(st.word_b0(ls), st.word_b1(ls), len);
                tg[k] = vocab_tag(h, len);
                e[k] = ld4(ix.vocab + (use[k] ? ((uint32_t)h & ix.vmask) : 0u));
            }
#pragma unroll
            for (uint32_t k = 0; k < VGROUP; k++) {
                const uint32_t l = use[k] ? base + k : 0;
                const uint32_t b0 = st.word_b0(l), b1 = st.word_b1(l);
                const bool hit = e[k].x == tg[k] && e[k].z == b0 && e[k].w == b1;
                uint32_t wid = e[k].y == NONE ? NONE : hit ? e[k].y : NONE - 1;
                pin(wid);
                if (use[k]) {
                    if (wid == NONE - 1) {
                        const uint32_t len = st.word_len(l);
                        const uint64_t h = word_hash_short(b0, b1, len);
                        wid = vocab_probe_short(ix, ((uint32_t)h + 1) & ix.vmask, tg[k], b0, b1);
                    }
                    st.set_wid(l, wid);
                }
            }
        }
    }
    if constexpr (S::deferred && S::need) {
      const uint32_t Lw = L >> 24;
      L &= 0xFFFFFFu;
      if (Lw < L) {
        st.set_wid(Lw, NONE);
        st.set_wid(Lw + 1, NONE);
        all_found = false;
        return RC_OK;
      }
    }
    for (uint32_t l = 0; l < L; l++) {
        const uint32_t wid = st.get_wid(l);
        all_found &= wid != NONE;
        xh = seq_hash_step(xh, wid);
    }
    xh = seq_hash_finish(xh, L);
    return RC_OK;
}

__device__ __forceinline__ int tail_list(const DevIndex &ix, uint32_t nl) {
    return nl <= MAX_LEVELS && need_levels(ix, nl) <= MID_L ? L_MID : L_DEEP;
}

template <class S>
__device__ void exact_find(const DevIndex &ix, uint64_t xh, uint32_t L, const S &st, uint32_t slot, uint32_t f,
                           uint32_t &off, uint32_t &cnt) {
    cnt = 0; off = 0;
    const uint32_t fp = exact_fp(xh);
    for (;;) {
        if (f == 0) return;
        if (f == fp) {
            const uint4 *e = reinterpret_cast<const uint4 *>(ix.exact + slot);
            uint4 a = e[0], b = e[1], c = e[2], d = e[3];
            pin(a); pin(b); pin(c); pin(d);
            if (a.x == (uint32_t)xh && a.y == (uint32_t)(xh >> 32) && a.z == L) {
                bool eq = true;
                if (L <= XINL) {
                    const uint32_t iw[XINL] = {b.z, b.w, c.x, c.y, c.z, c.w, d.x, d.y, d.z, d.w};
#pragma unroll
                    for (uint32_t l = 0; l < XINL; l++)
                        if (l < L) eq &= iw[l] == st.get_wid(l);
                } else {
                    for (uint32_t l = 0; l < L && eq; l++) eq = ix.wseq[b.y + l] == st.get_wid(l);
                }
                if (eq) { off = a.w; cnt = b.x; return; }
            }
        }
        slot = (slot + 1) & ix.xmask;
        f = ix.xfp[slot];
    }
}


enum { DFS_DONE = 0, DFS_STOP = 1, DFS_REROUTE = 2 };
template <class S, class EM>
__device__ int dfs(const DevIndex &ix, uint32_t L, bool dollar, S &st, EM &em) {
    uint32_t cur = ROOT, l = 0;
    for (;;) {
        const uint4 *np = reinterpret_cast<const uint4 *>(ix.nodes + cur);
        const uint4 n0 = np[0];
        const uint4 n1 = np[1];
        const uint4 n2 = np[2];
        const uint4 n3 = np[3];
        const bool droot = dollar && l == 0;
        const uint32_t w = l < L ? st.get_wid(l) : NONE;
        uint32_t inl = n2.x == w ? n3.x : n2.y == w ? n3.y : n2.z == w ? n3.z : n2.w == w ? n3.w : NONE;
        pin(inl);
        if (l == L) {
            if (!em(n0.w, n1.x)) return DFS_STOP;
            if (!droot && !em(n0.y, n0.z)) return DFS_STOP;
            if (n1.y & NLIT_HDESC) {
                if constexpr (!S::cuts) return DFS_REROUTE;
                st.cut(L);
            }
        } else {
            uint32_t lit = NONE;
            if (w != NONE) {
                if ((n1.y & NLIT_MASK) <= KINL) {
                    lit = inl;
                } else {
                    const uint32_t h = child_hash(w);
                    if (child_maybe(ix, n1, n2, n3, w, h) & 1u) {
                        uint32_t slo, shi;
                        lit = ctab_find(ix, n2.x, n2.y, w, h, slo, shi);
                        if (lit != NONE && !child_alive(slo, shi, l + 1, L, l + 1 < L ? st.get_wid(l + 1) : NONE,
                                                        l + 2 < L ? st.get_wid(l + 2) : NONE))
                            lit = NONE;
                    }
                }
            }
            if (!droot && !em(n0.y, n0.z)) return DFS_STOP;
            uint32_t plus = droot || (n1.y & NLIT_HDESC) ? NONE : n0.x;
            if (plus != NONE && !child_alive(n1.z, n1.w, l + 1, L, l + 1 < L ? st.get_wid(l + 1) : NONE,
                                             l + 2 < L ? st.get_wid(l + 2) : NONE))
                plus = NONE;
            if (plus != NONE) {
                if (lit != NONE) st.push(l + 1, lit);
                st.down(l, true);
                cur = plus; l++;
                continue;
            }
            if (lit != NONE) {
                st.down(l, false);
                cur = lit; l++;
                continue;
            }
        }
        if (!st.pop(l, cur)) return DFS_DONE;
        st.popped(l);
    }
}


struct RangeEmit {
    uint2 r[RCAP];
    uint32_t cnt, nr;
    __device__ __forceinline__ bool operator()(uint32_t off, uint32_t n) {
        if (n) {
#pragma unroll
            for (uint32_t i = 0; i < RCAP; i++)
                if (nr == i) r[i] = make_uint2(off, n);
            nr++; cnt += n & RUN_CNT;
        }
        return true;
    }
    __device__ __forceinline__ void store(uint2 *rng, uint64_t n, uint64_t t) const {
#pragma unroll
        for (uint32_t i = 0; i < RCAP; i++)
            if (i < nr) __builtin_nontemporal_store((uint64_t)r[i].x | ((uint64_t)r[i].y << 32),
                                                    reinterpret_cast<uint64_t *>(rng) + (uint64_t)i * n + t);
    }
};

struct DirectEmit {
    const uint32_t *vals;
    uint32_t *out;
    uint64_t pos, cap;
    __device__ __forceinline__ bool operator()(uint32_t off, uint32_t n) {
        const uint32_t c = n & RUN_CNT;
        for (uint32_t i = 0; i < c; i++, pos++)
            if (pos < cap) out[pos] = (n & RUN_INLINE) ? off : vals[off + i];
        return true;
    }
};

struct FirstEmit {
    const uint32_t *vals;
    uint32_t v;
    bool found;
    __device__ __forceinline__ bool operator()(uint32_t off, uint32_t n) {
        if (n) { v = (n & RUN_INLINE) ? off : vals[off]; found = true; return false; }
        return true;
    }
};

template <class S, class EM, class Src>
__device__ __forceinline__ int match_topic(const DevIndex &ix, const Src &src, uint64_t beg, uint64_t end, S &st,
                                           EM &em, uint32_t *levels = nullptr) {
    uint32_t L = 0; bool dollar, allf; uint64_t xh;
    int rc = tokenize(ix, src, beg, end, st, L, dollar, xh, allf);
    if (levels) *levels = L;
    if (rc) return rc;
    st.reset();
    const uint32_t xslot = (uint32_t)xh & ix.xmask;
    const uint32_t xf = allf ? ix.xfp[xslot] : 0;
    const int d = dfs(ix, L, dollar, st, em);
    if (d == DFS_STOP) return RC_OK;
    if (d == DFS_REROUTE) {
        if (levels) *levels = L;
        return RC_DEEP;
    }
    if (allf) {
        uint32_t xoff, xcnt;
        exact_find(ix, xh, L, st, xslot, xf, xoff, xcnt);
        em(xoff, xcnt);
    }
    return RC_OK;
}

enum { MODE_COUNT = 0, MODE_FIRST = 1 };

struct Outs {
    uint8_t *err;
    uint32_t *first_val;
    uint8_t *first_found;
};

__device__ __forceinline__ void list_push_wave(const Workspace &ws, uint64_t n, int k, uint32_t t) {
    const uint32_t lane = threadIdx.x & 63;
    for (int j = 0; j < L_COUNT; j++) {
        if (!__ballot(k >= 0)) break;
        const uint64_t m = __ballot(k == j);
        if (!m) continue;
        const uint32_t leader = (uint32_t)__ffsll((unsigned long long)m) - 1;
        uint32_t base = 0;
        if (lane == leader) base = atomicAdd(&ws.list_n[j], (uint32_t)__popcll(m));
        base = (uint32_t)__shfl((int)base, (int)leader, 64);
        if (k == j) ws.lists[(uint64_t)j * n + base + (uint32_t)__popcll(m & ((1ull << lane) - 1))] = t;
    }
}

__device__ __forceinline__ void list_push(const Workspace &ws, uint64_t n, int k, uint32_t t) {
    uint32_t i = atomicAdd(&ws.list_n[k], 1u);
    ws.lists[(uint64_t)k * n + i] = t;
}

template <int MODE, class S>
__device__ int run_topic(const DevIndex &ix, const Workspace &ws, uint64_t n, const uint8_t *blob,
                         const uint64_t *offs, uint64_t t, S &st, const Outs &o, uint32_t *hits,
                         int *ovf = nullptr) {
    const uint64_t beg = offs[t], end = offs[t + 1];
    if (MODE == MODE_COUNT) {
        RangeEmit em;
        em.cnt = 0; em.nr = 0;
        uint32_t levels;
        int rc = match_topic(ix, GlobalSrc{blob}, beg, end, st, em, &levels);
        const bool toolong = rc == RC_DEEP && S::maxl == MAX_LEVELS;
        if (rc == RC_DEEP && !toolong) { *hits = levels; return rc; }
        if (rc != RC_OK) { em.cnt = 0; em.nr = 0; }
        __builtin_nontemporal_store(em.cnt, ws.cnt + t);
        __builtin_nontemporal_store(em.nr, ws.nr + t);
        em.store(ws.rng, n, t);
        __builtin_nontemporal_store((uint8_t)(rc == RC_BADARG ? 1 : (toolong ? 2 : 0)), o.err + t);
        if (em.nr > RCAP) {
            const int k = S::maxl <= MID_L ? L_OVF_MID : L_OVF_DEEP;
            if (ovf) *ovf = k; else list_push(ws, n, k, (uint32_t)t);
        }
        *hits = em.cnt;
        return rc;
    } else {
        FirstEmit em{ix.vals, 0, false};
        uint32_t levels;
        int rc = match_topic(ix, GlobalSrc{blob}, beg, end, st, em, &levels);
        const bool toolong = rc == RC_DEEP && S::maxl == MAX_LEVELS;
        if (rc == RC_DEEP && !toolong) { *hits = levels; return rc; }
// ... 1575 lines not shown
```

### emqx_amd/csrc/tm_layout.h

```cpp
#pragma once
#include <stdint.h>

#if defined(__HIPCC__)
#define TM_HD __host__ __device__ __forceinline__
#else
#define TM_HD inline
#endif

namespace tmx {

constexpr uint32_t NONE = 0xFFFFFFFFu;
constexpr uint32_t ROOT = 0;
constexpr uint32_t VINL = 8;
constexpr uint32_t XINL = 10;

struct alignas(16) VocabEntry {
    uint32_t tag;
    uint32_t wid;
    uint32_t b0, b1;
};

struct alignas(16) CSlot {
    uint32_t wid;
    uint32_t child;
    uint32_t sum_lo, sum_hi;
};

constexpr uint32_t KINL = 4;

constexpr uint32_t WIDE_LIT = 256;

struct alignas(64) Node {
    uint32_t plus;
    uint32_t hash_off, hash_cnt;
    uint32_t exact_off, exact_cnt;
    uint32_t nlit;
    uint32_t psum_lo, psum_hi;
    uint32_t kw[KINL];
    uint32_t kc[KINL];
};

constexpr uint32_t NLIT_HDESC = 0x80000000u;
constexpr uint32_t NLIT_MASK = 0x7FFFFFFFu;

constexpr uint32_t PSUM_HASH = 1u, PSUM_EXACT = 2u, PSUM_PLUS = 4u, PSUM_HDESC = 8u;
constexpr uint32_t PSUM_QQ = 4, PSUM_BQ = 8, PSUM_BQQ = 36, PSUM_BLOOM = 28;

struct alignas(16) ExactEntry {
    uint32_t h_lo, h_hi;
    uint32_t nlev;
    uint32_t val_off, val_cnt;
    uint32_t seq_off;
    uint32_t wids[XINL];
};

constexpr uint32_t RUN_INLINE = 0x80000000u;
constexpr uint32_t RUN_CNT = 0x7FFFFFFFu;

static_assert(sizeof(VocabEntry) == 16, "vocab entry");
static_assert(sizeof(CSlot) == 16, "child slot");
static_assert(sizeof(Node) == 64, "node");
static_assert(sizeof(ExactEntry) == 64, "exact entry");


TM_HD uint64_t mix64(uint64_t x) {
    x ^= x >> 30; x *= 0xbf58476d1ce4e5b9ull;
    x ^= x >> 27; x *= 0x94d049bb133111ebull;
    x ^= x >> 31;
    return x;
}

constexpr uint64_t FNV_OFF = 0xcbf29ce484222325ull;
constexpr uint64_t FNV_PRIME = 0x100000001b3ull;

TM_HD uint64_t word_hash_short(uint32_t b0, uint32_t b1, uint32_t len) {
    return mix64((((uint64_t)b1 << 32) | b0) + 0x9e3779b97f4a7c15ull * (len + 1));
}
TM_HD uint64_t word_hash_finish(uint64_t fnv, uint32_t len) { return mix64(fnv ^ ((uint64_t)len << 56)); }

TM_HD uint32_t vocab_tag(uint64_t h, uint32_t len) {
    return ((uint32_t)(h >> 32) & 0xFFFFFF00u) | (len < 255 ? len : 255);
}

TM_HD uint32_t child_hash(uint32_t wid) {
    uint32_t x = wid + 0x9e3779b9u;
    x ^= x >> 16; x *= 0x7feb352du;
    x ^= x >> 15; x *= 0x846ca68bu;
    x ^= x >> 16;
    return x;
}
TM_HD uint32_t child_bit(uint32_t h) { return ((h >> 16) * 192u) >> 16; }
TM_HD uint32_t psum_bit(uint32_t h) { return ((h >> 16) * PSUM_BLOOM) >> 16; }
TM_HD uint32_t &bloom_word(Node &n, uint32_t j) { return j < 2 ? n.kw[2 + j] : n.kc[j - 2]; }

TM_HD uint16_t exact_fp(uint64_t h) { return (uint16_t)((h >> 48) | 1u); }

TM_HD uint64_t seq_hash_step(uint64_t h, uint32_t wid) { return (h ^ wid) * FNV_PRIME; }
TM_HD uint64_t seq_hash_finish(uint64_t h, uint32_t nlev) { return mix64(h + 0x9e3779b97f4a7c15ull * (nlev + 1)); }

}
```

### include/tmatch.h

```cpp
#ifndef TMATCH_H
#define TMATCH_H

#include <stdint.h>

#ifdef __cplusplus
extern "C" {
#endif

typedef struct tm_index tm_index;

enum {
    TM_OK = 0,
    TM_EINVAL = -1,
    TM_ENOMEM = -2,
    TM_EDEVICE = -3,
    TM_ECAP = -4
};

enum { TM_OP_DELETE = 0, TM_OP_INSERT = 1 };
enum { TM_KEY_BINARY = 0, TM_KEY_WORDS = 1, TM_KEY_EMPTY_LIST = 2, TM_KEY_ESCAPED = 4 };

typedef struct {
    int32_t device;
    uint32_t copies;
    uint64_t hint_keys;
} tm_options;

typedef struct {
    uint64_t n_keys;
    uint64_t n_wild_keys;
    uint64_t n_exact_keys;
    uint64_t n_dead_keys;
    uint64_t n_nodes, n_edges, n_words;
    uint64_t device_bytes;
    uint64_t uploads;
    uint64_t patch_bytes;
} tm_stats_t;

int tm_create(const tm_options *opts, tm_index **out);
int tm_destroy(tm_index *h);

int tm_create_replicas(const tm_options *opts, const int32_t *devices, uint32_t n, tm_index **out);

int tm_replica_stats(tm_index *h, uint32_t r, uint64_t *batches, int32_t *device);

int tm_apply_deltas(tm_index *h, uint64_t n, const uint8_t *ops, const uint8_t *filter_bytes,
                    const uint64_t *filter_offsets, const uint32_t *values, const uint8_t *key_flags);

int tm_apply_deltas_ex(tm_index *h, uint64_t n, const uint8_t *ops, const uint8_t *filter_bytes,
                       const uint64_t *filter_offsets, const uint32_t *values, const uint8_t *key_flags,
                       uint64_t *out_epoch);

int tm_commit(tm_index *h, uint64_t n, const uint8_t *ops, const uint8_t *filter_bytes, const uint64_t *filter_offsets,
              const uint32_t *values, const uint8_t *key_flags, uint64_t *out_epoch);

int tm_read_begin(tm_index *h, uint64_t *ticket);
int tm_read_end(tm_index *h, uint64_t ticket);
int tm_epoch(tm_index *h, uint64_t *current, uint64_t *safe);

int tm_sync(tm_index *h, void *stream);

int tm_match_batch(tm_index *h, uint64_t n, const uint8_t *topic_bytes, const uint64_t *topic_offsets,
                   uint64_t *out_hit_offsets, uint32_t *out_values, uint64_t cap, uint8_t *out_err);

enum { TM_ORDER_TRAVERSAL = 0, TM_ORDER_SORTED = 1, TM_ORDER_UNIQUE = 2 };

int tm_match_batch_ex(tm_index *h, uint64_t n, const uint8_t *topic_bytes, const uint64_t *topic_offsets,
                      uint64_t *out_hit_offsets, uint32_t *out_values, uint64_t cap, uint8_t *out_err,
                      uint32_t order, uint32_t *out_unique);

int tm_match_batch32_ex(tm_index *h, uint64_t n, const uint8_t *topic_bytes, const uint32_t *topic_offsets,
                        uint32_t *out_hit_offsets, uint32_t *out_values, uint64_t cap, uint8_t *out_err,
                        uint32_t order, uint32_t *out_unique);

int tm_match_batch32_pairs(tm_index *h, uint64_t n, const uint8_t *topic_bytes, const uint32_t *topic_offsets,
                           uint32_t *out_pairs, uint32_t *out_values, uint64_t cap, uint8_t *out_err);

int tm_match_batch32_dev(tm_index *h, uint64_t n, const uint8_t *d_topic_bytes, const uint32_t *d_topic_offsets,
                         uint32_t *d_out_hit_offsets, uint32_t *d_out_values, uint64_t cap, uint8_t *d_out_err,
                         void *stream);

int tm_host_alloc(tm_index *h, uint64_t bytes, void **out);
int tm_host_free(tm_index *h, void *p);

#define TM_ALLOC_VRAM 1u
int tm_host_alloc_ex(tm_index *h, uint64_t bytes, uint32_t flags, void **out);

int tm_match_batch_dev(tm_index *h, uint64_t n, const uint8_t *d_topic_bytes, const uint64_t *d_topic_offsets,
                       uint64_t *d_out_hit_offsets, uint32_t *d_out_values, uint64_t cap,
                       uint8_t *d_out_err, void *stream);

int tm_match_batch_dev_ex(tm_index *h, uint64_t n, const uint8_t *d_topic_bytes, const uint64_t *d_topic_offsets,
                          uint64_t *d_out_hit_offsets, uint32_t *d_out_values, uint64_t cap,
                          uint8_t *d_out_err, uint32_t order, uint32_t *d_out_unique, void *stream);

int tm_match_batch_dev_pairs(tm_index *h, uint64_t n, const uint8_t *d_topic_bytes, const uint64_t *d_topic_offsets,
                             uint32_t *d_out_pairs, uint32_t *d_out_values, uint64_t cap, uint8_t *d_out_err,
                             void *stream);

int tm_sort_segments(tm_index *h, uint64_t n, const uint64_t *d_hit_offsets, uint32_t *d_values, uint64_t cap,
                     uint32_t order, uint32_t *d_out_unique, void *stream);

int tm_set_dests(tm_index *h, uint64_t n, const uint32_t *values, const uint32_t *dests);
int tm_fanout_dev(tm_index *h, uint64_t n, const uint64_t *d_hit_offsets, const uint32_t *d_values, uint64_t cap,
                  const uint32_t *d_dest_of, uint64_t dest_len, uint32_t n_dests,
                  uint64_t *d_dest_offsets, uint32_t *d_out_topic, uint32_t *d_out_value, void *stream);
int tm_fanout_dev_pairs(tm_index *h, uint64_t n, const uint32_t *d_pairs, const uint32_t *d_values, uint64_t cap,
                        const uint32_t *d_dest_of, uint64_t dest_len, uint32_t n_dests,
                        uint64_t *d_dest_offsets, uint32_t *d_out_topic, uint32_t *d_out_value, void *stream);
int tm_route_batch(tm_index *h, uint64_t n, const uint8_t *topic_bytes, const uint64_t *topic_offsets,
                   uint32_t n_dests, uint64_t *out_dest_offsets, uint32_t *out_topic, uint32_t *out_values,
                   uint64_t cap, uint8_t *out_err);
int tm_route_batch32(tm_index *h, uint64_t n, const uint8_t *topic_bytes, const uint32_t *topic_offsets,
                     uint32_t n_dests, uint32_t *out_dest_offsets, uint32_t *out_topic, uint32_t *out_values,
                     uint64_t cap, uint8_t *out_err);

#define TM_ROUTE_AGGRE 1u
int tm_set_route_filters(tm_index *h, uint64_t n, const uint32_t *values, const uint32_t *filter_ids);
int tm_aggre_dev(tm_index *h, uint32_t n_dests, const uint64_t *d_dest_offsets, const uint32_t *d_topic,
                 const uint32_t *d_value, uint64_t cap, const uint32_t *d_filter_of, uint64_t filter_len,
                 uint64_t *d_out_dest_offsets, uint32_t *d_out_topic, uint32_t *d_out_value, void *stream);
int tm_route_batch_ex(tm_index *h, uint64_t n, const uint8_t *topic_bytes, const uint64_t *topic_offsets,
                      uint32_t n_dests, uint64_t *out_dest_offsets, uint32_t *out_topic, uint32_t *out_values,
                      uint64_t cap, uint8_t *out_err, uint32_t flags);
int tm_route_batch32_ex(tm_index *h, uint64_t n, const uint8_t *topic_bytes, const uint32_t *topic_offsets,
                        uint32_t n_dests, uint32_t *out_dest_offsets, uint32_t *out_topic, uint32_t *out_values,
                        uint64_t cap, uint8_t *out_err, uint32_t flags);

int tm_stream_release(tm_index *h, void *stream);

int tm_first_batch(tm_index *h, uint64_t n, const uint8_t *topic_bytes, const uint64_t *topic_offsets,
                   uint32_t *out_value, uint8_t *out_found);

int tm_matches_filter(tm_index *h, uint64_t n, const uint8_t *filter_bytes, const uint64_t *filter_offsets,
                      uint64_t *out_hit_offsets, uint32_t *out_values, uint64_t cap, uint8_t *out_err);
int tm_matches_filter_ex(tm_index *h, uint64_t n, const uint8_t *filter_bytes, const uint64_t *filter_offsets,
                         const uint8_t *filter_flags, uint64_t *out_hit_offsets, uint32_t *out_values, uint64_t cap,
                         uint8_t *out_err);

int tm_stats(tm_index *h, tm_stats_t *out);

int tm_merge_shards(uint32_t world, uint64_t n, const uint64_t *d_shard_hit_offsets, const uint32_t *d_shard_values,
                    uint64_t stride, uint64_t *d_out_hit_offsets, uint32_t *d_out_values, uint64_t cap,
                    void *stream);

int tm_profile_enable(tm_index *h, int enable);
int tm_profile_read(tm_index *h, double *walk_ms, double *batch_ms, uint64_t *batches, int reset);

enum { TM_DEBUG_LB_SPINS = 1, TM_DEBUG_LB_FAIL_BLOCK = 2, TM_DEBUG_LB_LAUNCHES = 3, TM_DEBUG_PHASES = 4,
       TM_DEBUG_FAILED_BATCHES = 5, TM_DEBUG_RETRIED_BATCHES = 6, TM_DEBUG_PATH_PHASES = 7,
       TM_DEBUG_PATH_SMALL = 8, TM_DEBUG_PATH_LANE = 9, TM_DEBUG_SMALL_KERNEL = 10,
       TM_DEBUG_COMBINE = 12, TM_DEBUG_COMBINED_LAUNCHES = 13, TM_DEBUG_COMBINED_BATCHES = 14,
       TM_DEBUG_WIDE_NODES = 15, TM_DEBUG_DENSE_WIDE = 16, TM_DEBUG_CMB_GATHER = 17, TM_DEBUG_CMB_LAND = 18,
       TM_DEBUG_COMMITS = 19, TM_DEBUG_COMMIT_WAITS = 20, TM_DEBUG_COMMIT_FORCED = 21, TM_DEBUG_SMALL_TICKET = 22,
       TM_DEBUG_CMB_SPIN = 23, TM_DEBUG_PATCH_ZC = 24, TM_DEBUG_FANOUT_GRID = 25,
       TM_DEBUG_ROUTE_ONE = 26, TM_DEBUG_ROUTE_GRID = 27 };
int tm_debug_set(tm_index *h, uint32_t key, uint64_t value);
int tm_debug_get(tm_index *h, uint32_t key, uint64_t *value);

const char *tm_last_error(tm_index *h);

uint32_t tm_abi_version(void);

#ifdef __cplusplus
}
#endif
#endif
```

Baseline: 4.549 billion topic matches/s.

## Embed per-word child summary hints for two widest trie nodes in vocab tags

For short words, the vocab tag no longer stores hash bits. It is freed to hold 12-bit child-summary hints for two designated 'annex' wide nodes, chosen as the nodes with the most literal children. During the vocab lookup the fast-path kernel parks these hints. When the walk reaches an annex node it can skip the ctab probe, or prune it outright, without loading the child slot. This is meant to remove random ctab memory loads at hot wide nodes such as a big level-1 fan-out. The cost is host bookkeeping to keep the hints in sync, plus full vocab rewrites whenever an annex node is reassigned.

```diff
diff --git a/emqx_amd/_native.py b/emqx_amd/_native.py
--- a/emqx_amd/_native.py
+++ b/emqx_amd/_native.py
@@ -39,6 +39,7 @@
 TM_DEBUG_PATCH_ZC = 24
 TM_DEBUG_FANOUT_GRID = 25
 TM_DEBUG_ROUTE_ONE, TM_DEBUG_ROUTE_GRID = 26, 27
+TM_DEBUG_ANNEX0, TM_DEBUG_ANNEX1, TM_DEBUG_HINT_AUDIT = 28, 29, 30
 MAX_DESTS = 65536
 
 
diff --git a/emqx_amd/csrc/tm_dev.h b/emqx_amd/csrc/tm_dev.h
--- a/emqx_amd/csrc/tm_dev.h
+++ b/emqx_amd/csrc/tm_dev.h
@@ -18,6 +18,7 @@
     uint32_t depth, xlen_max;
     uint64_t xlen_mask;
     uint32_t hdesc;
+    uint32_t anx_depth[ANX_SLOTS];
 };
 
 constexpr int FAST_L = 8;
diff --git a/emqx_amd/csrc/tm_host.cpp b/emqx_amd/csrc/tm_host.cpp
--- a/emqx_amd/csrc/tm_host.cpp
+++ b/emqx_amd/csrc/tm_host.cpp
@@ -149,6 +149,8 @@
     Mirror<uint32_t> wseq; uint64_t wseq_dead = 0;
     Mirror<uint32_t> wbits; uint32_t wb_words = 0;
     std::vector<uint32_t> free_wbits; std::set<uint32_t> wide;
+    uint32_t anx[ANX_SLOTS] = {NONE, NONE};
+    bool anx_dirty = false;
     std::unordered_map<uint64_t, uint32_t> lvl_edges;
     std::vector<uint32_t> lvl_distinct;
     bool dense_dirty = false;
@@ -277,13 +279,12 @@
 }
 
 bool vocab_eq(tm_index *ix, const VocabEntry &e, uint64_t h, const uint8_t *p, uint32_t n) {
-    if (e.tag != vocab_tag(h, n)) return false;
     if (n <= VINL) {
         uint32_t b0, b1;
         pack8(p, n, b0, b1);
-        return e.b0 == b0 && e.b1 == b1;
-    }
-    return e.b1 == n && !memcmp(ix->wpool.h.data() + e.b0, p, n);
+        return vocab_short_eq(e.tag, e.b0, e.b1, n, b0, b1);
+    }
+    return e.tag == vocab_tag(h, n) && e.b1 == n && !memcmp(ix->wpool.h.data() + e.b0, p, n);
 }
 
 uint32_t vocab_find(tm_index *ix, const uint8_t *p, uint32_t n) {
@@ -572,6 +573,7 @@
 }
 
 void to_wide(tm_index *ix, uint32_t node) {
+    ix->anx_dirty = true;
     if (ix->wide.empty()) ix->wb_words = 0;
     ix->wide.insert(node);
     if ((uint64_t)ix->wb_words * 32 < ix->wid_next) {
@@ -583,7 +585,12 @@
     wide_fill(ix, node);
 }
 
+void annex_set(tm_index *ix, uint32_t s, uint32_t p);
+int annex_slot(const tm_index *ix, uint32_t p);
+
 void from_wide(tm_index *ix, uint32_t node) {
+    if (const int s = annex_slot(ix, node); s >= 0) annex_set(ix, (uint32_t)s, NONE);
+    ix->anx_dirty = true;
     ix->free_wbits.push_back(ix->aux[node].bm);
     ix->aux[node].bm = NONE;
     ix->wide.erase(node);
@@ -626,6 +633,75 @@
 void summary_refresh(tm_index *ix, uint32_t x) {
     summary_refresh1(ix, x);
     if (x != ROOT && ix->aux[x].is_plus) summary_refresh1(ix, ix->aux[x].parent);
+}
+
+
+int annex_slot(const tm_index *ix, uint32_t p) {
+    for (uint32_t s = 0; s < ANX_SLOTS; s++) if (ix->anx[s] == p) return (int)s;
+    return -1;
+}
+
+void hint_put(tm_index *ix, uint32_t s, uint32_t wid, uint32_t hint) {
+    const uint32_t sl = ix->wslot[wid];
+    if (sl == NONE) return;
+    VocabEntry &e = ix->vocab.h[sl];
+    if (e.wid != wid || (e.tag & 0xFFu) > VINL) return;
+    const uint32_t sh = s ? HINT_SHIFT1 : HINT_SHIFT0;
+    const uint32_t t = (e.tag & ~(HINT_MASK << sh)) | hint << sh;
+    if (t != e.tag) { e.tag = t; ix->vocab.touch(sl); }
+}
+
+void hint_sync(tm_index *ix, uint32_t p, uint32_t wid) {
+    const int s = annex_slot(ix, p);
+    if (s < 0) return;
+    const Node &pn = ix->nodes.h[p];
+    uint32_t hint = 0;
+    if (nlit_of(pn) > KINL) {
+        const uint32_t sl = ctab_find(ix, pn.kw[0], pn.kw[1], wid);
+        if (sl != NONE) { const CSlot &c = ix->ctab.h[pn.kw[0] + sl]; hint = hint_of_sum(c.sum_lo, c.sum_hi); }
+    }
+    hint_put(ix, (uint32_t)s, wid, hint);
+}
+
+void annex_set(tm_index *ix, uint32_t s, uint32_t p) {
+    const uint32_t flag = s ? NLIT_ANX1 : NLIT_ANX0;
+    const uint32_t old = ix->anx[s];
+    if (old != NONE) { ix->nodes.h[old].nlit &= ~flag; ix->nodes.touch(old); }
+    ix->anx[s] = p;
+    if (p == NONE) return;
+    const uint32_t sh = s ? HINT_SHIFT1 : HINT_SHIFT0;
+    for (VocabEntry &e : ix->vocab.h)
+        if (e.wid != NONE && (e.tag & 0xFFu) <= VINL) e.tag &= ~(HINT_MASK << sh);
+    Node &pn = ix->nodes.h[p];
+    for (uint32_t i = 0; i <= pn.kw[1]; i++) {
+        const CSlot &c = ix->ctab.h[pn.kw[0] + i];
+        if (c.wid == NONE) continue;
+        VocabEntry &e = ix->vocab.h[ix->wslot[c.wid]];
+        if ((e.tag & 0xFFu) <= VINL) e.tag |= hint_of_sum(c.sum_lo, c.sum_hi) << sh;
+    }
+    ix->vocab.dirty.set_all();
+    pn.nlit |= flag;
+    ix->nodes.touch(p);
+}
+
+void annex_designate(tm_index *ix) {
+    if (!ix->anx_dirty) return;
+    ix->anx_dirty = false;
+    for (int round = 0; round < (int)ANX_SLOTS; round++) {
+        uint32_t best = NONE;
+        for (uint32_t node : ix->wide) {
+            if (ix->aux[node].depth < 1 || annex_slot(ix, node) >= 0) continue;
+            if (best == NONE || nlit_of(ix->nodes.h[node]) > nlit_of(ix->nodes.h[best])) best = node;
+        }
+        if (best == NONE) return;
+        uint32_t s = ANX_SLOTS;
+        for (uint32_t k = 0; k < ANX_SLOTS && s == ANX_SLOTS; k++) if (ix->anx[k] == NONE) s = k;
+        if (s == ANX_SLOTS) {
+            s = nlit_of(ix->nodes.h[ix->anx[1]]) < nlit_of(ix->nodes.h[ix->anx[0]]) ? 1 : 0;
+            if (nlit_of(ix->nodes.h[best]) < 2 * (uint64_t)nlit_of(ix->nodes.h[ix->anx[s]])) return;
+        }
+        annex_set(ix, s, best);
+    }
 }
 
 void summary_refresh1(tm_index *ix, uint32_t x) {
@@ -651,6 +727,7 @@
     if (c.sum_lo != (uint32_t)m || c.sum_hi != (uint32_t)(m >> 32)) {
         c.sum_lo = (uint32_t)m; c.sum_hi = (uint32_t)(m >> 32);
         ix->ctab.touch(pn.kw[0] + sl);
+        hint_sync(ix, p, a.wid);
     }
 }
 
@@ -713,7 +790,7 @@
 void child_add(tm_index *ix, uint32_t node, uint32_t wid, uint32_t child) {
     ix->nlinks++;
     lvl_edge(ix, ix->aux[node].depth, wid, true);
-    if (ix->aux[node].bm != NONE) ix->dense_dirty = true;
+    if (ix->aux[node].bm != NONE) { ix->dense_dirty = true; ix->anx_dirty = true; }
     Node *n = &ix->nodes.h[node];
     if (nlit_of(*n) < KINL) {
         for (uint32_t k = 0; k < KINL; k++)
@@ -725,6 +802,7 @@
         ctab_put(ix, n->kw[0], n->kw[1], wid, child, node_psum(ix, child));
         if (ix->aux[node].bm != NONE) wide_bit(ix, node, wid, true);
         else set_bloom(*n, wid);
+        hint_sync(ix, node, wid);
     }
     n->nlit++;
     if (nlit_of(*n) == WIDE_LIT && ix->aux[node].bm == NONE) { to_wide(ix, node); n = &ix->nodes.h[node]; }
@@ -735,7 +813,7 @@
 void child_remove(tm_index *ix, uint32_t node, uint32_t wid) {
     ix->nlinks--;
     lvl_edge(ix, ix->aux[node].depth, wid, false);
-    if (ix->aux[node].bm != NONE) ix->dense_dirty = true;
+    if (ix->aux[node].bm != NONE) { ix->dense_dirty = true; ix->anx_dirty = true; }
     Node &n = ix->nodes.h[node];
     if (nlit_of(n) <= KINL) {
         for (uint32_t k = 0; k < KINL; k++)
@@ -744,6 +822,7 @@
     } else {
         ctab_erase(ix, n.kw[0], n.kw[1], wid);
         wide_bit(ix, node, wid, false);
+        hint_sync(ix, node, wid);
         n.nlit--;
         if (ix->aux[node].bm != NONE && nlit_of(n) < WIDE_LIT) from_wide(ix, node);
         if (nlit_of(n) == KINL) {
@@ -759,7 +838,7 @@
 
 bool node_empty(tm_index *ix, uint32_t id) {
     const Node &n = ix->nodes.h[id];
-    return n.plus == NONE && n.nlit == 0 && n.hash_cnt == 0 && n.exact_cnt == 0 && ix->aux[id].hdesc == 0;
+    return n.plus == NONE && nlit_of(n) == 0 && n.hash_cnt == 0 && n.exact_cnt == 0 && ix->aux[id].hdesc == 0;
 }
 
 void node_prune(tm_index *ix, uint32_t id) {
@@ -1100,7 +1179,7 @@
     if (hpos < w.size()) {
         a.hdesc += ins ? 1 : -1;
         ix->n_hdesc_keys += ins ? 1 : -1;
-        nd.nlit = nlit_of(nd) | (a.hdesc ? NLIT_HDESC : 0);
+        nd.nlit = (nd.nlit & ~NLIT_HDESC) | (a.hdesc ? NLIT_HDESC : 0);
         ix->nodes.touch(node);
         summary_refresh(ix, node);
         if (!ins) node_prune(ix, node);
@@ -1432,6 +1511,7 @@
     d.xlen_mask = 0;
     for (size_t k = 0; k < xc.size() && k < 64; k++) if (xc[k]) d.xlen_mask |= 1ull << k;
     d.hdesc = ix->n_hdesc_keys != 0;
+    for (uint32_t s = 0; s < ANX_SLOTS; s++) d.anx_depth[s] = ix->anx[s] == NONE ? NONE : ix->aux[ix->anx[s]].depth;
     return d;
 }
 
@@ -1651,7 +1731,7 @@
 
 extern "C" {
 
-uint32_t tm_abi_version(void) { return (1u << 16) | 14u; }
+uint32_t tm_abi_version(void) { return (1u << 16) | 15u; }
 
 const char *tm_last_error(tm_index *) { return g_last_error.c_str(); }
 
@@ -1806,6 +1886,7 @@
                    key_flags ? key_flags[i] : 0, w, wids);
         reclaim(ix);
         wide_dense(ix);
+        annex_designate(ix);
     } catch (const std::bad_alloc &) {
         return fail(ix, TM_ENOMEM, "tm_apply_deltas: out of host memory");
     }
@@ -1822,12 +1903,13 @@
 
 constexpr auto COMMIT_WAIT = std::chrono::milliseconds(20);
 
-static_assert(sizeof(DevIndex) == 120, "DevIndex changed: compare the new field in same_view");
+static_assert(sizeof(DevIndex) == 128, "DevIndex changed: compare the new field in same_view");
 static bool same_view(const DevIndex &a, const DevIndex &b) {
     return a.vocab == b.vocab && a.vmask == b.vmask && a.wpool == b.wpool && a.nodes == b.nodes && a.ctab == b.ctab &&
            a.vals == b.vals && a.exact == b.exact && a.xmask == b.xmask && a.xfp == b.xfp && a.wseq == b.wseq &&
            a.wbits == b.wbits && a.wcap == b.wcap && a.depth == b.depth && a.xlen_max == b.xlen_max &&
-           a.xlen_mask == b.xlen_mask && a.hdesc == b.hdesc;
+           a.xlen_mask == b.xlen_mask && a.hdesc == b.hdesc && a.anx_depth[0] == b.anx_depth[0] &&
+           a.anx_depth[1] == b.anx_depth[1];
 }
 
 int tm_commit(tm_index *ix, uint64_t n, const uint8_t *ops, const uint8_t *fb, const uint64_t *fo,
@@ -3342,6 +3424,34 @@
         *value = v;
         break;
     }
+    case TM_DEBUG_ANNEX0:
+    case TM_DEBUG_ANNEX1: {
+        std::lock_guard<std::mutex> g(ix->img);
+        const uint32_t p = ix->anx[key - TM_DEBUG_ANNEX0];
+        *value = p == NONE ? ~0ull : (uint64_t)ix->aux[p].depth << 32 | nlit_of(ix->nodes.h[p]);
+        break;
+    }
+    case TM_DEBUG_HINT_AUDIT: {
+        std::lock_guard<std::mutex> g(ix->img);
+        uint64_t bad = 0;
+        for (uint32_t s = 0; s < ANX_SLOTS; s++) {
+            const uint32_t p = ix->anx[s];
+            if (p == NONE) continue;
+            const Node &pn = ix->nodes.h[p];
+            const uint32_t flag = s ? NLIT_ANX1 : NLIT_ANX0;
+            bad += (pn.nlit & (NLIT_ANX0 | NLIT_ANX1)) != flag || nlit_of(pn) < WIDE_LIT;
+            for (const VocabEntry &e : ix->vocab.h) {
+                if (e.wid == NONE || (e.tag & 0xFFu) > VINL) continue;
+                const uint32_t sl = ctab_find(ix, pn.kw[0], pn.kw[1], e.wid);
+                const CSlot *c = sl == NONE ? nullptr : &ix->ctab.h[pn.kw[0] + sl];
+                bad += ((e.tag >> (s ? HINT_SHIFT1 : HINT_SHIFT0)) & HINT_MASK) != (c ? hint_of_sum(c->sum_lo, c->sum_hi) : 0u);
+            }
+        }
+        for (uint32_t id = 0; id < ix->nodes.h.size(); id++)
+            bad += (ix->nodes.h[id].nlit & (NLIT_ANX0 | NLIT_ANX1)) && annex_slot(ix, id) < 0;
+        *value = bad;
+        break;
+    }
     default: return fail(ix, TM_EINVAL, "tm_debug_get: unknown key");
     }
     return TM_OK;
diff --git a/emqx_amd/csrc/tm_kernels.hip b/emqx_amd/csrc/tm_kernels.hip
--- a/emqx_amd/csrc/tm_kernels.hip
+++ b/emqx_amd/csrc/tm_kernels.hip
@@ -28,19 +28,6 @@
     return bloom_bit(n2, n3, child_bit(h));
 }
 
-__device__ __forceinline__ bool child_alive(uint32_t lo, uint32_t hi, uint32_t lq, uint32_t L, uint32_t wq,
-                                            uint32_t wq2) {
-    const uint64_t m = (uint64_t)hi << 32 | lo;
-    constexpr uint32_t AT_END = PSUM_HASH | PSUM_EXACT | PSUM_HDESC;
-    if (lq == L) return (m & AT_END) != 0;
-    if (m & PSUM_HASH) return true;
-    if (wq != NONE && ((m >> (PSUM_BQ + psum_bit(child_hash(wq)))) & 1u)) return true;
-    if (!(m & PSUM_PLUS)) return false;
-    const uint32_t qq = (uint32_t)(m >> PSUM_QQ) & 15u;
-    if (lq + 1 == L) return (qq & AT_END) != 0;
-    if (qq & (PSUM_HASH | PSUM_PLUS)) return true;
-    return wq2 != NONE && ((m >> (PSUM_BQQ + psum_bit(child_hash(wq2)))) & 1u);
-}
 
 __device__ __forceinline__ void pin(uint32_t &v) { asm volatile("" : "+v"(v)); }
 __device__ __forceinline__ void pin(uint2 &v) { pin(v.x); pin(v.y); }
@@ -97,22 +84,21 @@
     for (;;) {
         const uint4 e = ld4(ix.vocab + slot);
         if (e.y == NONE) return NONE;
-        if (e.x == tag) {
-            if (len <= VINL) {
-                if (e.z == b0 && e.w == b1) return e.y;
-            } else if (e.w == len && bytes_eq(ix.wpool + e.z, src, start, len)) {
-                return e.y;
-            }
+        if (len <= VINL) {
+            if (vocab_short_eq(e.x, e.z, e.w, len, b0, b1)) return e.y;
+        } else if (e.x == tag && e.w == len && bytes_eq(ix.wpool + e.z, src, start, len)) {
+            return e.y;
         }
         slot = (slot + 1) & ix.vmask;
     }
 }
 
-__device__ uint32_t vocab_probe_short(const DevIndex &ix, uint32_t slot, uint32_t tag, uint32_t b0, uint32_t b1) {
+__device__ uint32_t vocab_probe_short(const DevIndex &ix, uint32_t slot, uint32_t len, uint32_t b0, uint32_t b1,
+                                      uint32_t &tag) {
     for (;;) {
         const uint4 e = ld4(ix.vocab + slot);
         if (e.y == NONE) return NONE;
-        if (e.x == tag && e.z == b0 && e.w == b1) return e.y;
+        if (vocab_short_eq(e.x, e.z, e.w, len, b0, b1)) { tag = e.x; return e.y; }
         slot = (slot + 1) & ix.vmask;
     }
 }
@@ -140,6 +126,7 @@
     static constexpr bool deferred = true;
     static constexpr bool cuts = ML > FAST_L;
     static constexpr bool need = ML > FAST_L || LITE;
+    static constexpr bool hints = ML == FAST_L && !LITE;
     uint32_t *wid, *pend;
     uint8_t *len8;
     uint32_t stride;
@@ -163,6 +150,8 @@
     __device__ __forceinline__ uint32_t word_b0(uint32_t l) const { return wid[l * stride]; }
     __device__ __forceinline__ uint32_t word_b1(uint32_t l) const { return pend[l * stride]; }
     __device__ __forceinline__ uint32_t word_len(uint32_t l) const { return len8[l * stride]; }
+    __device__ __forceinline__ void park_hints(uint32_t v) { pend[0] = v; }
+    __device__ __forceinline__ uint32_t parked_hints() const { return pend[0]; }
     __device__ __forceinline__ void push(uint32_t l, uint32_t node) {
         pend[l * stride] = node; mask |= 1ull << l;
     }
@@ -180,6 +169,7 @@
     static constexpr bool deferred = false;
     static constexpr bool cuts = true;
     static constexpr bool need = true;
+    static constexpr bool hints = false;
     uint32_t *wid;
     uint2 *stk;
     uint8_t *plus_at;
@@ -206,6 +196,12 @@
 enum { RC_OK = 0, RC_BADARG = 1, RC_DEEP = 2 };
 
 constexpr uint32_t VGROUP = 6;
+
+constexpr uint32_t HINT_KNOWN = 0x1000u;
+__device__ __forceinline__ uint32_t hints_of_level(const DevIndex &ix, uint32_t l, uint32_t tag) {
+    return (l == ix.anx_depth[0] ? ((tag >> HINT_SHIFT0) & HINT_MASK) | HINT_KNOWN : 0u) |
+           (l == ix.anx_depth[1] ? (((tag >> HINT_SHIFT1) & HINT_MASK) | HINT_KNOWN) << 16 : 0u);
+}
 
 template <class Src>
 __device__ __noinline__ uint32_t count_slashes(const Src src, uint64_t p, uint64_t end) {
@@ -304,9 +300,9 @@
         L = lev;
     }
     if constexpr (S::deferred) {
+        uint32_t park = 0;
         for (uint32_t base = 0; base < (S::need ? L >> 24 : L); base += VGROUP) {
             uint4 e[VGROUP];
-            uint32_t tg[VGROUP];
             bool use[VGROUP];
 #pragma unroll
             for (uint32_t k = 0; k < VGROUP; k++) {
@@ -315,26 +311,28 @@
                 const uint32_t ls = use[k] ? l : 0;
                 const uint32_t len = st.word_len(ls);
                 const uint64_t h = word_hash_short(st.word_b0(ls), st.word_b1(ls), len);
-                tg[k] = vocab_tag(h, len);
                 e[k] = ld4(ix.vocab + (use[k] ? ((uint32_t)h & ix.vmask) : 0u));
             }
 #pragma unroll
             for (uint32_t k = 0; k < VGROUP; k++) {
                 const uint32_t l = use[k] ? base + k : 0;
                 const uint32_t b0 = st.word_b0(l), b1 = st.word_b1(l);
-                const bool hit = e[k].x == tg[k] && e[k].z == b0 && e[k].w == b1;
+                const uint32_t len = st.word_len(l);
+                const bool hit = vocab_short_eq(e[k].x, e[k].z, e[k].w, len, b0, b1);
                 uint32_t wid = e[k].y == NONE ? NONE : hit ? e[k].y : NONE - 1;
+                uint32_t tag = e[k].x;
                 pin(wid);
                 if (use[k]) {
                     if (wid == NONE - 1) {
-                        const uint32_t len = st.word_len(l);
                         const uint64_t h = word_hash_short(b0, b1, len);
-                        wid = vocab_probe_short(ix, ((uint32_t)h + 1) & ix.vmask, tg[k], b0, b1);
+                        wid = vocab_probe_short(ix, ((uint32_t)h + 1) & ix.vmask, len, b0, b1, tag);
                     }
                     st.set_wid(l, wid);
+                    if constexpr (S::hints) park |= hints_of_level(ix, l, tag);
                 }
             }
         }
+        if constexpr (S::hints) st.park_hints(park);
     }
     if constexpr (S::deferred && S::need) {
       const uint32_t Lw = L >> 24;
@@ -417,7 +415,16 @@
                     lit = inl;
                 } else {
                     const uint32_t h = child_hash(w);
-                    if (child_maybe(ix, n1, n2, n3, w, h) & 1u) {
+                    bool probe = true;
+                    if constexpr (S::hints) {
+                        if (n1.y & (NLIT_ANX0 | NLIT_ANX1)) {
+                            const uint32_t hk = st.parked_hints() >> ((n1.y & NLIT_ANX1) ? 16 : 0);
+                            if (hk & HINT_KNOWN)
+                                probe = (hk & HINT_CHILD) &&
+                                        hint_alive(hk & HINT_MASK, l + 1, L, l + 1 < L ? st.get_wid(l + 1) : NONE);
+                        }
+                    }
+                    if (probe && (child_maybe(ix, n1, n2, n3, w, h) & 1u)) {
                         uint32_t slo, shi;
                         lit = ctab_find(ix, n2.x, n2.y, w, h, slo, shi);
                         if (lit != NONE && !child_alive(slo, shi, l + 1, L, l + 1 < L ? st.get_wid(l + 1) : NONE,
diff --git a/emqx_amd/csrc/tm_layout.h b/emqx_amd/csrc/tm_layout.h
--- a/emqx_amd/csrc/tm_layout.h
+++ b/emqx_amd/csrc/tm_layout.h
@@ -41,10 +41,16 @@
 };
 
 constexpr uint32_t NLIT_HDESC = 0x80000000u;
-constexpr uint32_t NLIT_MASK = 0x7FFFFFFFu;
+constexpr uint32_t NLIT_ANX0 = 0x40000000u, NLIT_ANX1 = 0x20000000u;
+constexpr uint32_t NLIT_MASK = 0x1FFFFFFFu;
 
 constexpr uint32_t PSUM_HASH = 1u, PSUM_EXACT = 2u, PSUM_PLUS = 4u, PSUM_HDESC = 8u;
 constexpr uint32_t PSUM_QQ = 4, PSUM_BQ = 8, PSUM_BQQ = 36, PSUM_BLOOM = 28;
+
+constexpr uint32_t HINT_BITS = 12, HINT_MASK = 0xFFFu, HINT_SHIFT0 = 8, HINT_SHIFT1 = 20;
+constexpr uint32_t HINT_CHILD = 0x800u, HINT_HASH = 0x400u, HINT_EXACT = 0x200u, HINT_HDESC = 0x100u,
+                   HINT_PLUS = 0x80u, HINT_BLOOM = 7;
+constexpr uint32_t ANX_SLOTS = 2;
 
 struct alignas(16) ExactEntry {
     uint32_t h_lo, h_hi;
@@ -79,7 +85,11 @@
 TM_HD uint64_t word_hash_finish(uint64_t fnv, uint32_t len) { return mix64(fnv ^ ((uint64_t)len << 56)); }
 
 TM_HD uint32_t vocab_tag(uint64_t h, uint32_t len) {
+    if (len <= VINL) return len;
     return ((uint32_t)(h >> 32) & 0xFFFFFF00u) | (len < 255 ? len : 255);
+}
+TM_HD bool vocab_short_eq(uint32_t tag, uint32_t e0, uint32_t e1, uint32_t len, uint32_t b0, uint32_t b1) {
+    return (tag & 0xFFu) == len && e0 == b0 && e1 == b1;
 }
 
 TM_HD uint32_t child_hash(uint32_t wid) {
@@ -93,6 +103,33 @@
 TM_HD uint32_t psum_bit(uint32_t h) { return ((h >> 16) * PSUM_BLOOM) >> 16; }
 TM_HD uint32_t &bloom_word(Node &n, uint32_t j) { return j < 2 ? n.kw[2 + j] : n.kc[j - 2]; }
 
+TM_HD bool child_alive(uint32_t lo, uint32_t hi, uint32_t lq, uint32_t L, uint32_t wq, uint32_t wq2) {
+    const uint64_t m = (uint64_t)hi << 32 | lo;
+    constexpr uint32_t AT_END = PSUM_HASH | PSUM_EXACT | PSUM_HDESC;
+    if (lq == L) return (m & AT_END) != 0;
+    if (m & PSUM_HASH) return true;
+    if (wq != NONE && ((m >> (PSUM_BQ + psum_bit(child_hash(wq)))) & 1u)) return true;
+    if (!(m & PSUM_PLUS)) return false;
+    const uint32_t qq = (uint32_t)(m >> PSUM_QQ) & 15u;
+    if (lq + 1 == L) return (qq & AT_END) != 0;
+    if (qq & (PSUM_HASH | PSUM_PLUS)) return true;
+    return wq2 != NONE && ((m >> (PSUM_BQQ + psum_bit(child_hash(wq2)))) & 1u);
+}
+
+TM_HD uint32_t hint_bit(uint32_t h) { return psum_bit(h) >> 2; }
+TM_HD uint32_t hint_of_sum(uint32_t lo, uint32_t hi) {
+    const uint64_t m = (uint64_t)hi << 32 | lo;
+    uint32_t v = HINT_CHILD | ((m & PSUM_HASH) ? HINT_HASH : 0) | ((m & PSUM_EXACT) ? HINT_EXACT : 0) |
+                 ((m & PSUM_HDESC) ? HINT_HDESC : 0) | ((m & PSUM_PLUS) ? HINT_PLUS : 0);
+    for (uint32_t j = 0; j < HINT_BLOOM; j++) v |= ((m >> (PSUM_BQ + 4 * j)) & 15u) ? 1u << j : 0u;
+    return v;
+}
+TM_HD bool hint_alive(uint32_t h, uint32_t lq, uint32_t L, uint32_t wq) {
+    if (lq == L) return (h & (HINT_HASH | HINT_EXACT | HINT_HDESC)) != 0;
+    if (h & (HINT_HASH | HINT_PLUS)) return true;
+    return wq != NONE && ((h >> hint_bit(child_hash(wq))) & 1u);
+}
+
 TM_HD uint16_t exact_fp(uint64_t h) { return (uint16_t)((h >> 48) | 1u); }
 
 TM_HD uint64_t seq_hash_step(uint64_t h, uint32_t wid) { return (h ^ wid) * FNV_PRIME; }
diff --git a/include/tmatch.h b/include/tmatch.h
--- a/include/tmatch.h
+++ b/include/tmatch.h
@@ -154,7 +154,8 @@
        TM_DEBUG_WIDE_NODES = 15, TM_DEBUG_DENSE_WIDE = 16, TM_DEBUG_CMB_GATHER = 17, TM_DEBUG_CMB_LAND = 18,
        TM_DEBUG_COMMITS = 19, TM_DEBUG_COMMIT_WAITS = 20, TM_DEBUG_COMMIT_FORCED = 21, TM_DEBUG_SMALL_TICKET = 22,
        TM_DEBUG_CMB_SPIN = 23, TM_DEBUG_PATCH_ZC = 24, TM_DEBUG_FANOUT_GRID = 25,
-       TM_DEBUG_ROUTE_ONE = 26, TM_DEBUG_ROUTE_GRID = 27 };
+       TM_DEBUG_ROUTE_ONE = 26, TM_DEBUG_ROUTE_GRID = 27, TM_DEBUG_ANNEX0 = 28, TM_DEBUG_ANNEX1 = 29,
+       TM_DEBUG_HINT_AUDIT = 30 };
 int tm_debug_set(tm_index *h, uint32_t key, uint64_t value);
 int tm_debug_get(tm_index *h, uint32_t key, uint64_t *value);
 
```

After: 4.718 billion topic matches/s, median of 6. +3.7%, better.
